# Inuri04/pgtg

Measured on AMD Instinct MI355X. Metric: env-steps/sec (batched random-action rollout) at 1/2/4/8 MI355X, higher is better.
Workload: dtype int32; 1 GPU; configs[4]: 1048576 envs of 5x5 procedural maps split over the GPUs, random actions, auto-reset, RCCL-reduced global step counter; envs_total=1048576, envs_per_gpu=1048576, map=5x5, autoreset=True, parallelism=dp1 (env shards, no data-path collective)

## Files before the change

### include/pgtg.h

```cpp
#ifndef PGTG_H_
#define PGTG_H_

#include <stdint.h>

#ifdef __cplusplus
extern "C" {
#endif

#define PGTG_ABI_VERSION 9

#define PGTG_OK 0
#define PGTG_E_INVALID -1
#define PGTG_E_DONE -2
#define PGTG_E_DEVICE -3
#define PGTG_E_UNSUPPORTED -4
#define PGTG_E_MAP -5

#define PGTG_MAX_TILES 256
#define PGTG_MAX_CHANNELS 128
#define PGTG_MAX_RULES 8
#define PGTG_MAX_WINDOW 31

enum {
  PGTG_CH_ZERO = 0,
  PGTG_CH_WALL = 1,
  PGTG_CH_GOALS = 2,
  PGTG_CH_TRAFFIC = 3,
  PGTG_CH_TL_GREEN = 4,
  PGTG_CH_TL_YELLOW = 5,
  PGTG_CH_TL_RED = 6,
  PGTG_CH_START = 7,
  PGTG_CH_SUBGOAL = 8,
  PGTG_CH_USED_SUBGOAL = 9,
  PGTG_CH_FINAL_GOAL = 10,
  PGTG_CH_ICE = 11,
  PGTG_CH_BROKEN = 12,
  PGTG_CH_SAND = 13,
  PGTG_CH_SPAWNER = 14,
  PGTG_CH_LANE0 = 32
};

typedef struct {
  int32_t tile_exits;
  int32_t speed_sq_min;
  int32_t speed_sq_max;
  int32_t min_traffic;
  int32_t min_matching_traffic;
  uint8_t weight[6][20];
} PgtgRule;

typedef struct {
  int32_t abi_version;
  int32_t width, height;
  double pct_connections;
  int32_t start_mode, goal_mode;
  int32_t start_x, start_y, start_dir;
  int32_t goal_x, goal_y, goal_dir;
  int32_t min_distance;
  double obstacle_probability;
  double w_ice, w_broken, w_sand, w_tl;
  int32_t n_channels;
  int32_t channels[PGTG_MAX_CHANNELS];
  int32_t sliding, sliding_size, next_subgoal;
  double sum_subgoals_reward, final_goal_bonus, crash_penalty, tl_violation_penalty;
  double standing_still_penalty, visited_penalty;
  double ice_probability, street_damage_probability, sand_probability, traffic_density;
  int32_t phase_dur[3];
  int32_t ignore_traffic_collisions;
  double profile_pct[5];
  int32_t separate_reward_cost;
  int32_t n_rules;
  PgtgRule rules[PGTG_MAX_RULES];
  int32_t fixed_map, fm_w, fm_h;
  uint8_t fm_exits[PGTG_MAX_TILES];
  int8_t fm_obst_type[PGTG_MAX_TILES];
  int8_t fm_obst_mask[PGTG_MAX_TILES];
  int32_t fm_start[3], fm_goal[3];
  int32_t autoreset;
  int32_t max_episode_steps;
  int32_t min_car_capacity;
  int32_t tune_envs_per_block;
  int32_t tune_obs_sub;
  int32_t tune_kt_grid, tune_kt_cap, tune_kt_wpc;
  int32_t tune_car_slots;
  int32_t tune_kt_serial;
  int32_t tune_queue_mode;
  int32_t tune_fault;
} PgtgConfig;

typedef struct {
  uint8_t* obs;
  int32_t* position;
  int32_t* velocity;
  int32_t* next_subgoal;
  double* reward;
  double* cost;
  uint8_t* terminated;
  uint8_t* truncated;
  uint8_t* final_obs;
  int32_t* final_position;
  int32_t* final_velocity;
  int32_t* final_next_subgoal;
  uint8_t* braking;
} PgtgOutputs;

typedef struct {
  int32_t x, y, vx, vy;
  int32_t terminated, flat_tire, phase, elapsed;
  int32_t n_cars, next_car_id, path_len, error;
  uint32_t spawn_counter;
  uint64_t seed;
  uint64_t used_subgoals[4];
  int32_t n_spawners, car_tail;
} PgtgEnvState;

typedef struct {
  int32_t id, x, y, route, profile, patience, delay;
} PgtgCar;

typedef struct {
  uint64_t episodes, truncated_only, length_sum;
  int32_t  length_min, length_max;
  double   return_sum;
  float    return_min, return_max;
} PgtgEpisodeSummary;

typedef struct pgtg_handle pgtg_handle;

int pgtg_create(const PgtgConfig* cfg, uint64_t n_envs, int32_t device, pgtg_handle** out);
int pgtg_destroy(pgtg_handle* h);
int pgtg_set_stream(pgtg_handle* h, void* stream);
int pgtg_set_outputs(pgtg_handle* h, const PgtgOutputs* out);
int pgtg_reset(pgtg_handle* h, const uint64_t* seeds_host, uint64_t seed_base, const uint8_t* mask_dev);
int pgtg_reset_unseeded(pgtg_handle* h, const uint8_t* mask_dev);
int pgtg_step(pgtg_handle* h, const uint8_t* actions_dev);
int pgtg_step_many(pgtg_handle* h, const uint8_t* actions_dev, uint64_t row_stride, uint64_t ticks);
int pgtg_random_actions(pgtg_handle* h, uint8_t* actions_dev, uint64_t seed, uint64_t t, uint64_t env_offset);
int pgtg_get_env_state(pgtg_handle* h, uint64_t env, PgtgEnvState* st);
int pgtg_get_cars(pgtg_handle* h, uint64_t env, PgtgCar* cars, int32_t cap, int32_t* n);
int pgtg_get_map_plan(pgtg_handle* h, uint64_t env, int32_t* w, int32_t* h_, uint8_t* exits, int8_t* otype,
                      int8_t* omask, int32_t* start3, int32_t* goal3);
#define PGTG_SQ_WALL (1ull << 32)
#define PGTG_SQ_SPAWNER (1ull << 37)
#define PGTG_SQ_START (1ull << 38)
#define PGTG_SQ_SUBGOAL (1ull << 39)
#define PGTG_SQ_USED_SUBGOAL (1ull << 40)
#define PGTG_SQ_FINAL_GOAL (1ull << 41)
#define PGTG_SQ_ICE (1ull << 42)
#define PGTG_SQ_BROKEN_ROAD (1ull << 43)
#define PGTG_SQ_SAND (1ull << 44)
#define PGTG_SQ_TRAFFIC_LIGHT (1ull << 45)
int pgtg_get_squares(pgtg_handle* h, uint64_t env, uint64_t* words, int32_t cap, int32_t* width, int32_t* height);
int pgtg_set_agent(pgtg_handle* h, uint64_t env, int32_t x, int32_t y, int32_t vx, int32_t vy);
int pgtg_add_car(pgtg_handle* h, uint64_t env, int32_t x, int32_t y, int32_t route, int32_t profile, int32_t car_id);
int pgtg_state_size(pgtg_handle* h, uint64_t* bytes);
int pgtg_dump_state(pgtg_handle* h, void* buf, uint64_t bytes);
int pgtg_load_state(pgtg_handle* h, const void* buf, uint64_t bytes);
typedef struct pgtg_snapshot pgtg_snapshot;
int pgtg_snapshot_create(pgtg_handle* h, uint64_t slots, pgtg_snapshot** out);
int pgtg_snapshot_destroy(pgtg_snapshot* s);
int pgtg_snapshot_bytes(const pgtg_snapshot* s, uint64_t* device_bytes, uint64_t* bytes_per_env);
int pgtg_snapshot_save(pgtg_handle* h, pgtg_snapshot* s, const uint32_t* env_idx_dev, const uint32_t* slot_idx_dev,
                       uint64_t count);
int pgtg_snapshot_load(pgtg_handle* h, const pgtg_snapshot* s, const uint32_t* slot_idx_dev, const uint32_t* env_idx_dev,
                       uint64_t count);
int pgtg_set_to_state(pgtg_handle* h, uint64_t env, int32_t x, int32_t y, int32_t vx, int32_t vy, int32_t flat_tire,
                      const PgtgCar* cars, int32_t n_cars);
int pgtg_set_rules(pgtg_handle* h, const PgtgRule* rules, int32_t n_rules);
int pgtg_set_flat_outputs(pgtg_handle* h, const int32_t* order, int32_t n_order, int32_t dtype, void* flat_dev,
                          void* final_flat_dev);
int pgtg_set_flat_scalars(pgtg_handle* h, float* reward_f32_dev, uint8_t* dones_dev, uint8_t* truncated_only_dev);
int pgtg_flatten(pgtg_handle* h, int32_t mode, int32_t grid);
int pgtg_set_episode_stats(pgtg_handle* h, float* ep_return_dev, int32_t* ep_length_dev);
int pgtg_episode_summary(pgtg_handle* h, PgtgEpisodeSummary* out, int32_t reset);
typedef struct {
  uint64_t n, steps;
  double gamma, gae_lambda;
  const float*   rewards;
  const float*   values;
  const uint8_t* dones;
  const uint8_t* truncated_only;
  const float*   terminal_values;
  const float*   last_values;
  float* advantages; float* returns;
} PgtgGae;
int pgtg_gae(pgtg_handle* h, const PgtgGae* a);
#define PGTG_POLICY_SAMPLE 0
#define PGTG_POLICY_ARGMAX 1
#define PGTG_POLICY_VALUE_ONLY 2
#define PGTG_POLICY_MAX_OBS_DIM 1048576
typedef struct {
  const float *w1p, *b1p, *w2p, *b2p, *wa, *ba;
  const float *w1v, *b1v, *w2v, *b2v, *wv, *bv;
  uint64_t obs_dim;
} PgtgPolicyWeights;
typedef struct { uint64_t n, obs_dim; const int8_t* obs; const void* packed;
                 int32_t mode; uint64_t seed, counter, env_offset;
                 const float* uniforms; uint8_t* actions; float* values; float* log_probs; } PgtgPolicy;
int pgtg_policy_packed_bytes(uint64_t obs_dim, uint64_t* bytes);
int pgtg_policy_pack(pgtg_handle* h, const PgtgPolicyWeights* raw, void* packed);
int pgtg_policy(pgtg_handle* h, const PgtgPolicy* a);
int pgtg_policy_chunk(void);
typedef struct {
  float *w1p, *b1p, *w2p, *b2p, *wa, *ba;
  float *w1v, *b1v, *w2v, *b2v, *wv, *bv;
} PgtgPpoGrads;
typedef struct {
  uint64_t batch, obs_dim, steps, n, obs_pitch;
  const int8_t* obs; const int64_t* indices;
  const uint8_t* actions;
  const float *log_probs, *advantages, *returns;
  const void* packed;
  const float* adv_stats;
  double clip_range, ent_coef, vf_coef;
  void* workspace;
  PgtgPpoGrads grads;
  float* stats;
} PgtgPpoGrad;
int pgtg_ppo_workspace_bytes(uint64_t obs_dim, uint64_t batch, uint64_t* bytes);
int pgtg_ppo_grad(pgtg_handle* h, const PgtgPpoGrad* a);
typedef struct {
  const float *w1p, *b1p, *w2p, *b2p, *wa, *ba;
  const float *w1v, *b1v, *w2v, *b2v, *wv, *bv;
} PgtgPpoConstGrads;
typedef struct {
  uint64_t obs_dim;
  PgtgPpoGrads params;
  PgtgPpoConstGrads grads;
  PgtgPpoGrads exp_avg, exp_avg_sq;
  void* packed;
  void* workspace;
  uint64_t step;
  float lr, beta1, beta2, eps, max_grad_norm;
  float* grad_norm;
} PgtgPpoStep;
int pgtg_ppo_step_workspace_bytes(uint64_t obs_dim, uint64_t* bytes);
int pgtg_ppo_step(pgtg_handle* h, const PgtgPpoStep* a);
int pgtg_ppo_adv_stats(pgtg_handle* h, const void* advantages, const void* indices, uint64_t batch, uint64_t steps,
                       uint64_t n, float* out);
typedef struct {
  uint64_t n, n_episodes;
  uint64_t step;
  double gamma;
  const double*  reward;
  const uint8_t* terminated;
  const uint8_t* truncated;
  double* ret; double* disc; double* g;
  int32_t* len; int32_t* cnt;
  double* rec_return; double* rec_discounted; int32_t* rec_length;
  double* rec_last_reward; int32_t* rec_end_step; uint8_t* rec_flags;
  int32_t* open_rows;
} PgtgEval;
typedef struct {
  uint64_t episodes, open_envs;
  uint64_t terminated, truncated_only;
  uint64_t last_reward_positive, last_reward_negative;
  uint64_t negative_discounted;
  uint64_t length_sum;
  int32_t  length_min, length_max;
  double   return_mean, return_std;
  double   return_min, return_max;
  double   discounted_mean, discounted_std;
} PgtgEvalSummary;
int pgtg_eval_step(pgtg_handle* h, const PgtgEval* a);
int pgtg_eval_summary(pgtg_handle* h, const PgtgEval* a, PgtgEvalSummary* out_dev, void* workspace);
int pgtg_eval_workspace_bytes(uint64_t n, uint64_t n_episodes, uint64_t* bytes);
int pgtg_observe(pgtg_handle* h);
int pgtg_car_digest(pgtg_handle* h, uint64_t* out_dev);
int pgtg_get_counters(pgtg_handle* h, uint64_t* env_steps, uint64_t* episodes);
int pgtg_get_queue_maps(pgtg_handle* h, uint64_t* maps);
int pgtg_get_queue_overflow(pgtg_handle* h, uint64_t* served);
int pgtg_error_count(pgtg_handle* h, uint64_t* n_errors, int32_t* first_code);
int pgtg_measure_hbm(int32_t device, uint64_t bytes, int32_t reps, double* copy_gbs);
int pgtg_window(const pgtg_handle* h);
uint64_t pgtg_num_envs(const pgtg_handle* h);
int pgtg_launch_info(const pgtg_handle* h, int32_t* envs_per_block, int32_t* lds_bytes);
int pgtg_occupancy(const pgtg_handle* h, int32_t* step_blocks_per_cu);
const char* pgtg_step_kernel(const pgtg_handle* h);
const char* pgtg_last_error(const pgtg_handle* h);
int pgtg_enable_timing(pgtg_handle* h, int32_t every);
int pgtg_timing_read(pgtg_handle* h, double* total_ms, uint64_t* launches, int32_t reset);

#ifdef __cplusplus
}
#endif
#endif
```

### pgtg_amd/_abi.py

```python
from __future__ import annotations

import ctypes as C
import os

from . import config as cfgmod

PKG = os.path.dirname(os.path.abspath(__file__))
LIB_PATH = os.environ.get("PGTG_LIB") or os.path.join(PKG, "libpgtg_hip.so")

PGTG_ABI_VERSION = 9
MAX_TILES = 256
MAX_CHANNELS = 128
MAX_RULES = 8

PGTG_OK = 0
PGTG_E_INVALID = -1
PGTG_E_DONE = -2
PGTG_E_DEVICE = -3
PGTG_E_UNSUPPORTED = -4
PGTG_E_MAP = -5

EXPORTED = [
    "pgtg_create", "pgtg_destroy", "pgtg_set_stream", "pgtg_set_outputs", "pgtg_reset",
    "pgtg_reset_unseeded", "pgtg_step", "pgtg_step_many", "pgtg_random_actions", "pgtg_get_env_state", "pgtg_get_cars",
    "pgtg_get_map_plan", "pgtg_get_squares", "pgtg_set_rules", "pgtg_set_agent", "pgtg_add_car", "pgtg_observe", "pgtg_get_counters",
    "pgtg_error_count", "pgtg_window", "pgtg_num_envs", "pgtg_launch_info", "pgtg_occupancy", "pgtg_step_kernel", "pgtg_last_error", "pgtg_enable_timing",
    "pgtg_timing_read", "pgtg_measure_hbm", "pgtg_state_size", "pgtg_dump_state", "pgtg_load_state",
    "pgtg_set_to_state", "pgtg_car_digest", "pgtg_get_queue_maps", "pgtg_get_queue_overflow", "pgtg_set_flat_outputs", "pgtg_set_flat_scalars",
    "pgtg_set_episode_stats", "pgtg_episode_summary", "pgtg_gae", "pgtg_flatten",
    "pgtg_eval_step", "pgtg_eval_summary", "pgtg_eval_workspace_bytes",
    "pgtg_policy", "pgtg_policy_pack", "pgtg_policy_packed_bytes", "pgtg_policy_chunk",
    "pgtg_ppo_workspace_bytes", "pgtg_ppo_grad",
    "pgtg_ppo_step_workspace_bytes", "pgtg_ppo_step", "pgtg_ppo_adv_stats",
    "pgtg_snapshot_create", "pgtg_snapshot_destroy", "pgtg_snapshot_bytes", "pgtg_snapshot_save", "pgtg_snapshot_load",
]


class PgtgRule(C.Structure):
    _fields_ = [("tile_exits", C.c_int32), ("speed_sq_min", C.c_int32), ("speed_sq_max", C.c_int32),
                ("min_traffic", C.c_int32), ("min_matching_traffic", C.c_int32),
                ("weight", (C.c_uint8 * 20) * 6)]


class PgtgConfig(C.Structure):
    _fields_ = [
        ("abi_version", C.c_int32), ("width", C.c_int32), ("height", C.c_int32),
        ("pct_connections", C.c_double), ("start_mode", C.c_int32), ("goal_mode", C.c_int32),
        ("start_x", C.c_int32), ("start_y", C.c_int32), ("start_dir", C.c_int32),
        ("goal_x", C.c_int32), ("goal_y", C.c_int32), ("goal_dir", C.c_int32),
        ("min_distance", C.c_int32), ("obstacle_probability", C.c_double),
        ("w_ice", C.c_double), ("w_broken", C.c_double), ("w_sand", C.c_double), ("w_tl", C.c_double),
        ("n_channels", C.c_int32), ("channels", C.c_int32 * MAX_CHANNELS),
        ("sliding", C.c_int32), ("sliding_size", C.c_int32), ("next_subgoal", C.c_int32),
        ("sum_subgoals_reward", C.c_double), ("final_goal_bonus", C.c_double),
        ("crash_penalty", C.c_double), ("tl_violation_penalty", C.c_double),
        ("standing_still_penalty", C.c_double), ("visited_penalty", C.c_double),
        ("ice_probability", C.c_double), ("street_damage_probability", C.c_double),
        ("sand_probability", C.c_double), ("traffic_density", C.c_double),
        ("phase_dur", C.c_int32 * 3), ("ignore_traffic_collisions", C.c_int32),
        ("profile_pct", C.c_double * 5), ("separate_reward_cost", C.c_int32),
        ("n_rules", C.c_int32), ("rules", PgtgRule * MAX_RULES),
        ("fixed_map", C.c_int32), ("fm_w", C.c_int32), ("fm_h", C.c_int32),
        ("fm_exits", C.c_uint8 * MAX_TILES), ("fm_obst_type", C.c_int8 * MAX_TILES),
        ("fm_obst_mask", C.c_int8 * MAX_TILES), ("fm_start", C.c_int32 * 3), ("fm_goal", C.c_int32 * 3),
        ("autoreset", C.c_int32), ("max_episode_steps", C.c_int32), ("min_car_capacity", C.c_int32),
        ("tune_envs_per_block", C.c_int32), ("tune_obs_sub", C.c_int32), ("tune_kt_grid", C.c_int32),
        ("tune_kt_cap", C.c_int32), ("tune_kt_wpc", C.c_int32), ("tune_car_slots", C.c_int32),
        ("tune_kt_serial", C.c_int32), ("tune_queue_mode", C.c_int32), ("tune_fault", C.c_int32),
    ]


class PgtgOutputs(C.Structure):
    _fields_ = [(n, C.c_void_p) for n in (
        "obs", "position", "velocity", "next_subgoal", "reward", "cost", "terminated", "truncated",
        "final_obs", "final_position", "final_velocity", "final_next_subgoal", "braking")]


class PgtgEnvState(C.Structure):
    _fields_ = [(n, C.c_int32) for n in ("x", "y", "vx", "vy", "terminated", "flat_tire", "phase", "elapsed",
                                         "n_cars", "next_car_id", "path_len", "error")] + [
        ("spawn_counter", C.c_uint32), ("seed", C.c_uint64), ("used_subgoals", C.c_uint64 * 4),
        ("n_spawners", C.c_int32), ("car_tail", C.c_int32)]


class PgtgCar(C.Structure):
    _fields_ = [(n, C.c_int32) for n in ("id", "x", "y", "route", "profile", "patience", "delay")]


class PgtgEpisodeSummary(C.Structure):
    _fields_ = [("episodes", C.c_uint64), ("truncated_only", C.c_uint64), ("length_sum", C.c_uint64),
                ("length_min", C.c_int32), ("length_max", C.c_int32), ("return_sum", C.c_double),
                ("return_min", C.c_float), ("return_max", C.c_float)]


class PgtgGae(C.Structure):
    _fields_ = [("n", C.c_uint64), ("steps", C.c_uint64), ("gamma", C.c_double), ("gae_lambda", C.c_double)] + [
        (n, C.c_void_p) for n in ("rewards", "values", "dones", "truncated_only", "terminal_values", "last_values",
                                  "advantages", "returns")]


EVAL_STATE_FIELDS = ("ret", "disc", "g", "len", "cnt")
EVAL_RECORD_FIELDS = ("rec_return", "rec_discounted", "rec_length", "rec_last_reward", "rec_end_step", "rec_flags")


class PgtgEval(C.Structure):
    _fields_ = [("n", C.c_uint64), ("n_episodes", C.c_uint64), ("step", C.c_uint64), ("gamma", C.c_double)] + [
        (n, C.c_void_p) for n in ("reward", "terminated", "truncated") + EVAL_STATE_FIELDS + EVAL_RECORD_FIELDS
        + ("open_rows",)]


class PgtgEvalSummary(C.Structure):
    _fields_ = [(n, C.c_uint64) for n in ("episodes", "open_envs", "terminated", "truncated_only",
                                          "last_reward_positive", "last_reward_negative", "negative_discounted",
                                          "length_sum")] + [
        ("length_min", C.c_int32), ("length_max", C.c_int32)] + [
        (n, C.c_double) for n in ("return_mean", "return_std", "return_min", "return_max", "discounted_mean",
                                  "discounted_std")]


PGTG_POLICY_SAMPLE, PGTG_POLICY_ARGMAX, PGTG_POLICY_VALUE_ONLY = 0, 1, 2
PGTG_POLICY_MAX_OBS_DIM = 1048576
POLICY_WEIGHT_FIELDS = ("w1p", "b1p", "w2p", "b2p", "wa", "ba", "w1v", "b1v", "w2v", "b2v", "wv", "bv")


class PgtgPolicyWeights(C.Structure):
    _fields_ = [(n, C.c_void_p) for n in POLICY_WEIGHT_FIELDS] + [("obs_dim", C.c_uint64)]


class PgtgPolicy(C.Structure):
    _fields_ = [("n", C.c_uint64), ("obs_dim", C.c_uint64), ("obs", C.c_void_p), ("packed", C.c_void_p),
                ("mode", C.c_int32), ("seed", C.c_uint64), ("counter", C.c_uint64), ("env_offset", C.c_uint64),
                ("uniforms", C.c_void_p), ("actions", C.c_void_p), ("values", C.c_void_p), ("log_probs", C.c_void_p)]


class PgtgPpoGrads(C.Structure):
    _fields_ = [(n, C.c_void_p) for n in POLICY_WEIGHT_FIELDS]


class PgtgPpoGrad(C.Structure):
    _fields_ = [(n, C.c_uint64) for n in ("batch", "obs_dim", "steps", "n", "obs_pitch")] + [
        (n, C.c_void_p) for n in ("obs", "indices", "actions", "log_probs", "advantages", "returns", "packed",
                                  "adv_stats")] + [
        ("clip_range", C.c_double), ("ent_coef", C.c_double), ("vf_coef", C.c_double), ("workspace", C.c_void_p),
        ("grads", PgtgPpoGrads), ("stats", C.c_void_p)]


class PgtgPpoStep(C.Structure):
    _fields_ = [("obs_dim", C.c_uint64), ("params", PgtgPpoGrads), ("grads", PgtgPpoGrads), ("exp_avg", PgtgPpoGrads),
                ("exp_avg_sq", PgtgPpoGrads), ("packed", C.c_void_p), ("workspace", C.c_void_p), ("step", C.c_uint64),
                ("lr", C.c_float), ("beta1", C.c_float), ("beta2", C.c_float), ("eps", C.c_float),
                ("max_grad_norm", C.c_float), ("grad_norm", C.c_void_p)]


_lib = None


def lib():
    global _lib
    if _lib is not None:
        return _lib
    if not os.path.exists(LIB_PATH):
        raise RuntimeError(f"{LIB_PATH} not built: run `python -m pgtg_amd.build` (HIP/gfx950); "
                           "there is no CPU fallback")
    import torch
    L = C.CDLL(LIB_PATH)
    vp, u64, i32 = C.c_void_p, C.c_uint64, C.c_int32
    sig = {
        "pgtg_create": ([C.POINTER(PgtgConfig), u64, i32, C.POINTER(vp)], C.c_int),
        "pgtg_destroy": ([vp], C.c_int),
        "pgtg_set_stream": ([vp, vp], C.c_int),
        "pgtg_set_outputs": ([vp, C.POINTER(PgtgOutputs)], C.c_int),
        "pgtg_reset": ([vp, vp, u64, vp], C.c_int),
        "pgtg_reset_unseeded": ([vp, vp], C.c_int),
        "pgtg_step": ([vp, vp], C.c_int),
        "pgtg_step_many": ([vp, vp, u64, u64], C.c_int),
        "pgtg_random_actions": ([vp, vp, u64, u64, u64], C.c_int),
        "pgtg_measure_hbm": ([i32, u64, i32, C.POINTER(C.c_double)], C.c_int),
        "pgtg_state_size": ([vp, C.POINTER(u64)], C.c_int),
        "pgtg_dump_state": ([vp, vp, u64], C.c_int),
        "pgtg_load_state": ([vp, vp, u64], C.c_int),
        "pgtg_set_to_state": ([vp, u64, i32, i32, i32, i32, i32, C.POINTER(PgtgCar), i32], C.c_int),
        "pgtg_get_env_state": ([vp, u64, C.POINTER(PgtgEnvState)], C.c_int),
        "pgtg_get_cars": ([vp, u64, C.POINTER(PgtgCar), i32, C.POINTER(i32)], C.c_int),
        "pgtg_get_map_plan": ([vp, u64] + [vp] * 7, C.c_int),
        "pgtg_get_squares": ([vp, u64, vp, i32, C.POINTER(i32), C.POINTER(i32)], C.c_int),
        "pgtg_set_rules": ([vp, vp, i32], C.c_int),
        "pgtg_set_agent": ([vp, u64, i32, i32, i32, i32], C.c_int),
        "pgtg_add_car": ([vp, u64, i32, i32, i32, i32, i32], C.c_int),
        "pgtg_observe": ([vp], C.c_int),
        "pgtg_get_counters": ([vp, C.POINTER(u64), C.POINTER(u64)], C.c_int),
        "pgtg_car_digest": ([vp, vp], C.c_int),
        "pgtg_get_queue_maps": ([vp, C.POINTER(u64)], C.c_int),
        "pgtg_get_queue_overflow": ([vp, C.POINTER(u64)], C.c_int),
        "pgtg_set_flat_outputs": ([vp, C.POINTER(C.c_int32), i32, i32, vp, vp], C.c_int),
        "pgtg_set_flat_scalars": ([vp, vp, vp, vp], C.c_int),
        "pgtg_flatten": ([vp, i32, i32], C.c_int),
        "pgtg_set_episode_stats": ([vp, vp, vp], C.c_int),
        "pgtg_episode_summary": ([vp, C.POINTER(PgtgEpisodeSummary), i32], C.c_int),
        "pgtg_gae": ([vp, C.POINTER(PgtgGae)], C.c_int),
        "pgtg_eval_step": ([vp, C.POINTER(PgtgEval)], C.c_int),
        "pgtg_eval_summary": ([vp, C.POINTER(PgtgEval), vp, vp], C.c_int),
        "pgtg_eval_workspace_bytes": ([u64, u64, C.POINTER(u64)], C.c_int),
        "pgtg_policy": ([vp, C.POINTER(PgtgPolicy)], C.c_int),
        "pgtg_policy_pack": ([vp, C.POINTER(PgtgPolicyWeights), vp], C.c_int),
        "pgtg_policy_packed_bytes": ([u64, C.POINTER(u64)], C.c_int),
        "pgtg_policy_chunk": ([], C.c_int),
        "pgtg_ppo_workspace_bytes": ([u64, u64, C.POINTER(u64)], C.c_int),
        "pgtg_ppo_grad": ([vp, C.POINTER(PgtgPpoGrad)], C.c_int),
        "pgtg_ppo_step_workspace_bytes": ([u64, C.POINTER(u64)], C.c_int),
        "pgtg_ppo_step": ([vp, C.POINTER(PgtgPpoStep)], C.c_int),
        "pgtg_ppo_adv_stats": ([vp, vp, vp, u64, u64, u64, vp], C.c_int),
        "pgtg_snapshot_create": ([vp, u64, C.POINTER(vp)], C.c_int),
        "pgtg_snapshot_destroy": ([vp], C.c_int),
        "pgtg_snapshot_bytes": ([vp, C.POINTER(u64), C.POINTER(u64)], C.c_int),
        "pgtg_snapshot_save": ([vp, vp, vp, vp, u64], C.c_int),
        "pgtg_snapshot_load": ([vp, vp, vp, vp, u64], C.c_int),
        "pgtg_error_count": ([vp, C.POINTER(u64), C.POINTER(i32)], C.c_int),
        "pgtg_window": ([vp], C.c_int),
        "pgtg_num_envs": ([vp], u64),
        "pgtg_launch_info": ([vp, C.POINTER(i32), C.POINTER(i32)], C.c_int),
        "pgtg_occupancy": ([vp, C.POINTER(i32)], C.c_int),
        "pgtg_step_kernel": ([vp], C.c_char_p),
        "pgtg_last_error": ([vp], C.c_char_p),
        "pgtg_timing_read": ([vp, C.POINTER(C.c_double), C.POINTER(u64), i32], C.c_int),
        "pgtg_enable_timing": ([vp, i32], C.c_int),
    }
    compat = os.environ.get("PGTG_ABI_COMPAT")
    for name, (args, res) in sig.items():
        if compat and not hasattr(L, name):
            continue
        f = getattr(L, name)
        f.argtypes = args
        f.restype = res
    _lib = L
    return L


def fill_rules(dst, rules) -> int:
    if len(rules) > MAX_RULES:
        raise ValueError(f"at most {MAX_RULES} traffic rules are supported")
    for i, r in enumerate(rules):
        o = dst[i]
        o.tile_exits, o.speed_sq_min, o.speed_sq_max = r.tile_exits, r.speed_sq_min, r.speed_sq_max
        o.min_traffic, o.min_matching_traffic = r.min_traffic, r.min_matching_traffic
        for d in range(6):
            for k in range(20):
                o.weight[d][k] = r.weight[d][k]
    return len(rules)


TUNE_KEYS = ("envs_per_block", "obs_sub", "kt_grid", "kt_cap", "kt_wpc", "car_slots", "kt_serial", "queue_mode", "fault")


def config_struct(spec: "cfgmod.EnvSpec", autoreset: bool, max_episode_steps: int | None,
                  min_car_capacity: int = 0, tune: dict | None = None) -> PgtgConfig:
    c = PgtgConfig()
    c.abi_version = int(os.environ.get("PGTG_ABI_COMPAT") or PGTG_ABI_VERSION)
    c.width, c.height = spec.width, spec.height
    c.pct_connections = spec.pct_connections
    c.start_mode, c.goal_mode = spec.start_mode, spec.goal_mode
    c.start_x, c.start_y, c.start_dir = spec.start_xyd
    c.goal_x, c.goal_y, c.goal_dir = spec.goal_xyd
    c.min_distance = spec.min_distance
    c.obstacle_probability = spec.obstacle_probability
    c.w_ice, c.w_broken, c.w_sand, c.w_tl = [float(w) for w in spec.weights]
    c.n_channels = len(spec.channels)
    for i, (_, code) in enumerate(spec.channels):
        c.channels[i] = code
    c.sliding, c.sliding_size, c.next_subgoal = int(spec.sliding), spec.sliding_size, int(spec.next_subgoal)
    c.sum_subgoals_reward = spec.sum_subgoals_reward
    c.final_goal_bonus = spec.final_goal_bonus
    c.crash_penalty = spec.crash_penalty
    c.tl_violation_penalty = spec.tl_violation_penalty
    c.standing_still_penalty = spec.standing_still_penalty
    c.visited_penalty = spec.visited_penalty
    c.ice_probability = spec.ice_probability
    c.street_damage_probability = spec.street_damage_probability
    c.sand_probability = spec.sand_probability
    c.traffic_density = spec.traffic_density
    for i in range(3):
        c.phase_dur[i] = spec.phase_dur[i]
    c.ignore_traffic_collisions = int(spec.ignore_traffic_collisions)
    for i in range(5):
        c.profile_pct[i] = float(spec.profile_pct[i])
    c.separate_reward_cost = int(spec.separate_reward_cost)
    c.n_rules = fill_rules(c.rules, spec.rules)
    fm = spec.fixed_map
    if fm is not None:
        if fm.width * fm.height > MAX_TILES:
            raise ValueError(f"this build supports maps of at most {MAX_TILES} tiles")
        c.fixed_map = 1
        c.fm_w, c.fm_h = fm.width, fm.height
        for i in range(fm.width * fm.height):
            c.fm_exits[i] = fm.exits[i]
            c.fm_obst_type[i] = fm.obstacle_type[i]
            c.fm_obst_mask[i] = fm.obstacle_mask[i]
        for i in range(3):
            c.fm_start[i] = fm.start[i]
            c.fm_goal[i] = fm.goal[i]
    c.autoreset = int(autoreset)
    c.max_episode_steps = int(max_episode_steps or 0)
    c.min_car_capacity = int(min_car_capacity)
    for k, v in (tune or {}).items():
        if k not in TUNE_KEYS:
            raise ValueError(f"unknown launch-shape override {k!r} (one of {TUNE_KEYS})")
        setattr(c, "tune_" + k, int(v))
    return c
```

### pgtg_amd/csrc/pgtg_env.hip

```cpp
#include <hip/hip_runtime.h>

#include <math.h>
#include <stdint.h>
#include <stdio.h>
#include <stdlib.h>
#include <string.h>

#include <algorithm>
#include <array>
#include <cstddef>
#include <string>
#include <vector>

#include "pgtg_device.h"
#include "pgtg_episode.h"
#include "pgtg_eval.h"
#include "pgtg_rollout.h"
#include "pgtg_policy.h"
#include "pgtg_ppo.h"
#include "pgtg_ppo_step.h"
#include "pgtg_snapshot.h"

namespace pgtg {
namespace dv {
#define PGTG_TBL_QUAL __constant__ static const
#include "pgtg_tables.h"
#undef PGTG_TBL_QUAL
}
namespace hs {
#define PGTG_TBL_QUAL static const
#include "pgtg_tables.h"
#undef PGTG_TBL_QUAL
}

__shared__ __attribute__((aligned(16))) TablesHead sT;
__shared__ __attribute__((aligned(16))) TablesTail sTX;

__device__ __forceinline__ void stage_bytes(const void* __restrict__ gsrc, void* ldst, int bytes) {
  const int n4 = bytes >> 4, tid = (int)threadIdx.x;
  const uint4* src = reinterpret_cast<const uint4*>(gsrc);
  uint4* dst = reinterpret_cast<uint4*>(ldst);
  uint4 r[4];
#pragma unroll
  for (int j = 0; j < 4; j++) r[j] = src[tid + j * kBlock < n4 ? tid + j * kBlock : 0];
#pragma unroll
  for (int j = 0; j < 4; j++)
    if (tid + j * kBlock < n4) dst[tid + j * kBlock] = r[j];
  for (int k = tid + 4 * kBlock; k < n4; k += kBlock) dst[k] = src[k];
  for (int k = n4 * 4 + tid; k < bytes / 4; k += kBlock)
    reinterpret_cast<uint32_t*>(ldst)[k] = reinterpret_cast<const uint32_t*>(gsrc)[k];
}
__device__ __forceinline__ void stage_tables(const Tables* __restrict__ gtab, bool tail) {
  stage_bytes(gtab, &sT, (int)sizeof(TablesHead));
  if (tail) stage_bytes(reinterpret_cast<const uint8_t*>(gtab) + kTabHead, &sTX, (int)sizeof(TablesTail));
}

__device__ __forceinline__ void lds_barrier() {
  __builtin_amdgcn_fence(__ATOMIC_RELEASE, "workgroup", "local");
  __builtin_amdgcn_s_barrier();
  __builtin_amdgcn_fence(__ATOMIC_ACQUIRE, "workgroup", "local");
}

template <bool BIG>
__device__ __forceinline__ void stage_plan(const uint16_t* __restrict__ plan, int nq, uint32_t* dst, int pdw) {
  const uint4* src = reinterpret_cast<const uint4*>(plan);
  for (int k0 = 0; k0 < (BIG ? nq : 1); k0 += 8) {
    uint4 q[8];
#pragma unroll
    for (int k = 0; k < 8; k++) q[k] = src[k0 + k < nq ? k0 + k : k0];
#pragma unroll
    for (int k = 0; k < 8; k++) {
      if (k0 + k < nq) {
        const uint32_t wv[4] = {q[k].x, q[k].y, q[k].z, q[k].w};
#pragma unroll
        for (int j = 0; j < 4; j++)
          if ((k0 + k) * 4 + j < pdw) dst[(k0 + k) * 4 + j] = wv[j];
      }
    }
  }
}

#ifdef PGTG_STAMPS
__device__ unsigned long long g_stamps[1 << 21];
#define STAMP(k)                                                                          \
  do {                                                                                    \
    if ((threadIdx.x & 63) == 0) {                                                        \
      unsigned long long t_ = __builtin_amdgcn_s_memtime();                               \
      g_stamps[((blockIdx.x * (kBlock / 64) + (threadIdx.x >> 6)) * 32 + (k)) & ((1 << 21) - 1)] = t_; \
    }                                                                                     \
  } while (0)
#define STAMPR(k)                                                                                     \
  do {                                                                                                \
    if ((threadIdx.x & 63) == 0)                                                                      \
      g_stamps[(1 << 20) | ((((blockIdx.x * (kBlock / 64) + (threadIdx.x >> 6)) * 8 + (k))) & ((1 << 20) - 1))] = \
          __builtin_amdgcn_s_memrealtime();                                                           \
  } while (0)
#else
#define STAMP(k) \
  do {           \
  } while (0)
#define STAMPR(k) \
  do {            \
  } while (0)
#endif

__device__ __forceinline__ uint32_t bit81(const uint32_t* m3, int sq) { return (m3[sq >> 5] >> (sq & 31)) & 1u; }

__device__ __forceinline__ int seg_dir(int lx, int ly) {
  bool mx = (unsigned)(lx - 3) <= 2u, my = (unsigned)(ly - 3) <= 2u;
  if (ly == 0 && mx) return 0;
  if (lx == 8 && my) return 1;
  if (ly == 8 && mx) return 2;
  if (lx == 0 && my) return 3;
  return -1;
}

struct EnvView {
  int px, py, vx, vy;
  uint32_t phase, flags, path_len, elapsed;
  uint32_t sg, spawn;
  uint64_t used;
};

__device__ __forceinline__ EnvView rec_view(const EnvRec& e) {
  EnvView v;
  v.px = (int)(int16_t)(e.a.x & 0xffffu);
  v.py = (int)(int16_t)(e.a.x >> 16);
  v.vx = (int)(int16_t)(e.a.y & 0xffffu);
  v.vy = (int)(int16_t)(e.a.y >> 16);
  v.phase = e.a.z & 0xffffu;
  v.flags = (e.a.z >> 16) & 0xfu;
  v.path_len = e.a.z >> 20;
  v.elapsed = e.a.w;
  v.sg = e.b.x;
  v.spawn = e.b.y;
  v.used = (uint64_t)e.b.z | ((uint64_t)e.b.w << 32);
  return v;
}
__device__ __forceinline__ EnvView rec_load(const EnvRec* r, uint64_t i) { return rec_view(r[i]); }
__device__ __forceinline__ void rec_store(EnvRec* r, uint64_t i, const EnvView& v) {
  EnvRec e;
  e.a.x = ((uint32_t)v.px & 0xffffu) | ((uint32_t)v.py << 16);
  e.a.y = ((uint32_t)v.vx & 0xffffu) | ((uint32_t)v.vy << 16);
  e.a.z = (v.phase & 0xffffu) | ((v.flags & 0xfu) << 16) | (v.path_len << 20);
  e.a.w = v.elapsed;
  e.b.x = v.sg;
  e.b.y = v.spawn;
  e.b.z = (uint32_t)v.used;
  e.b.w = (uint32_t)(v.used >> 32);
  r[i] = e;
}

__device__ __forceinline__ uint32_t plan_word_mask(const DevCfg& c, int word) {
  const int t0 = 2 * word;
  return t0 + 1 < c.nt ? ~0u : (t0 < c.nt ? 0xffffu : 0u);
}
constexpr int kQueueDepth = 3;
__host__ __device__ inline uint32_t queue_slot(uint32_t bits) { return (bits & 3u) < 2u ? (bits & 3u) : 2u; }
__host__ __device__ inline uint32_t queue_cur(uint32_t qs) { return queue_slot(qs); }
__host__ __device__ inline uint32_t queue_head(uint32_t qs) { return queue_slot(qs >> 2); }
__host__ __device__ inline uint32_t queue_spare(uint32_t qc, uint32_t qh) { return qc != qh ? 3u - qc - qh : (qc + 2u) % 3u; }
template <bool SLOT>
__device__ __forceinline__ uint16_t* plan_row(const DevCfg& c, const DevState& S, uint64_t i) {
  if (!SLOT) return S.plan + i * (uint64_t)c.plan_stride;
  return reinterpret_cast<uint16_t*>(S.qbuf + (i * kQueueDepth + queue_cur(S.qstate[i])) * (uint64_t)c.qrec_dw);
}
__device__ __forceinline__ void store_plan_quads(const DevCfg& c, uint4* dstp, int nq, const uint32_t* pw, int pdw) {
  for (int k = 0; k < nq; k++) {
    uint32_t wv[4];
#pragma unroll
    for (int j = 0; j < 4; j++) wv[j] = (k * 4 + j < pdw) ? pw[k * 4 + j] & plan_word_mask(c, k * 4 + j) : 0u;
    dstp[k] = make_uint4(wv[0], wv[1], wv[2], wv[3]);
  }
}
template <bool SLOT>
__device__ __forceinline__ void store_plan_row(const DevCfg& c, const DevState& S, uint64_t i, const uint32_t* pw, int pdw) {
  if (SLOT) {
    store_plan_quads(c, reinterpret_cast<uint4*>(plan_row<true>(c, S, i)), c.qrec_dw / 4, pw, pdw);
    return;
  }
  uint4* dstp = reinterpret_cast<uint4*>(S.plan + i * (uint64_t)c.plan_stride);
  for (int k = 0; k < c.plan_stride / 8; k++) {
    uint32_t wv[4];
#pragma unroll
    for (int j = 0; j < 4; j++) wv[j] = (k * 4 + j < pdw) ? pw[k * 4 + j] & plan_word_mask(c, k * 4 + j) : 0u;
    dstp[k] = make_uint4(wv[0], wv[1], wv[2], wv[3]);
  }
}

struct Plan {
  uint16_t* p;
  __device__ __forceinline__ uint32_t operator[](int t) const { return p[t]; }
};

template <bool BIG>
__device__ __forceinline__ bool used_bit(const EnvView& v, uint32_t p, int t) {
  return BIG ? (p & kPlanUsed) != 0u : ((v.used >> t) & 1ull) != 0ull;
}

template <bool BIG>
__device__ __forceinline__ uint32_t square_flags(const DevCfg& c, const Plan& pl, const EnvView& v, int x, int y) {
  int tx = x / kTile, ty = y / kTile;
  int lx = x - tx * kTile, ly = y - ty * kTile;
  int t = ty * c.tw + tx;
  uint32_t p = pl[t];
  uint32_t ex = plan_exits(p);
  int sq = lx * 9 + ly;
  uint32_t f = 0;
  uint32_t wall = bit81(sT.wall[ex], sq);
  if (wall) f |= SQ_WALL;
  int d = seg_dir(lx, ly);
  if (d >= 0 && ((ex >> d) & 1u)) {
    if (plan_sgdir(p) == d) f |= used_bit<BIG>(v, p, t) ? SQ_USED : SQ_SUBGOAL;
    if ((int)(v.sg & 0xffu) == t && (int)((v.sg >> 8) & 0xffu) == d) f |= SQ_START;
    if ((int)((v.sg >> 16) & 0xffu) == t && (int)(v.sg >> 24) == d) f |= SQ_FINAL;
  }
  const uint32_t ob = bit81(sT.obst[min(plan_omask(p), (uint32_t)PGTG_N_OBST_MASKS - 1u)], sq);
  uint32_t ot = plan_otype(p);
  if (ot && !wall && ob) f |= SQ_ICE << (ot - 1);
  return f;
}
__device__ __forceinline__ uint32_t square_lanes(const DevCfg& c, const Plan& pl, int x, int y) {
  int tx = x / kTile, ty = y / kTile;
  int lx = x - tx * kTile, ly = y - ty * kTile;
  uint32_t ex = plan_exits(pl[ty * c.tw + tx]);
  return ex ? sTX.lanes[ex][lx * 9 + ly] : 0u;
}
__device__ __forceinline__ bool square_spawner(const DevCfg& c, const Plan& pl, int x, int y) {
  int tx = x / kTile, ty = y / kTile;
  int lx = x - tx * kTile, ly = y - ty * kTile;
  uint32_t ex = plan_exits(pl[ty * c.tw + tx]);
  if (!ex) return false;
  int sq = lx * 9 + ly;
  if (bit81(sT.spawner[ex], sq)) return true;
  uint32_t l = sTX.lanes[ex][sq];
  return (tx == 0 && (l >> 31 & 1u)) || (tx == c.tw - 1 && (l >> 30 & 1u)) || (ty == 0 && (l >> 29 & 1u)) ||
         (ty == c.th - 1 && (l >> 28 & 1u));
}
__device__ __forceinline__ bool inside(const DevCfg& c, int x, int y) {
  return (unsigned)x < (unsigned)c.W && (unsigned)y < (unsigned)c.H;
}
__device__ __forceinline__ int phase_color(const DevCfg& c, uint32_t ph) {
  return (int)ph < c.phase_g ? 0 : ((int)ph < c.phase_gy ? 1 : 2);
}

__device__ __forceinline__ int lane_slot_tw(int tw, const Plan& pl, int x, int y) {
  int tx = x / kTile, ty = y / kTile;
  int lx = x - tx * kTile, ly = y - ty * kTile;
  int t = ty * tw + tx;
  uint32_t ex = plan_exits(pl[t]);
  const int li_raw = sTX.li[ex][lx * 9 + ly];
  const int li = ex ? li_raw : 255;
  return li == 255 ? -1 : t * 32 + li;
}
// ... 2085 lines not shown
      if (pcg_double(sand) < c.sand_p) {
        cx += pxp;
        cy += pyp;
        v.vx = v.vy = 0;
        break;
      }
    }
    cx += pxp;
    cy += pyp;
  }
  (void)gl_t;
  (void)gl_d;
  if (used_ice) stream_store_state(S.ice, i, ice);
  if (used_broken) stream_store_state(S.broken, i, broken);
  if (used_sand) stream_store_state(S.sand, i, sand);
  if (v.flags & kFlagFlatTire) v.vx = v.vy = 0;
  const bool accel = !(ax == 0 && ay == 0);
  if (S.visited) {
    uint32_t* vis = S.visited + i * (uint64_t)c.vis_words;
    int b = (cx + 2) * c.vis_pitch + (cy + 2);
    if (c.visited_penalty != 0.0 && accel && ((vis[b >> 5] >> (b & 31)) & 1u)) {
      if (c.separate_cost) cost += c.visited_penalty; else reward -= c.visited_penalty;
    }
    vis[b >> 5] |= 1u << (b & 31);
  }
  const int ox = v.px, oy = v.py;
  v.px = cx;
  v.py = cy;
  if (c.still_penalty != 0.0 && !accel && ox == cx && oy == cy) {
    if (c.separate_cost) cost += c.still_penalty; else reward -= c.still_penalty;
  }
  v.elapsed += 1u;
  if (c.max_steps > 0 && (int)v.elapsed >= c.max_steps) v.flags |= kFlagTruncated;
  res.reward = c.separate_cost ? perf : reward;
  res.cost = cost;
  return 0;
}

__device__ __forceinline__ uint32_t expand4(uint32_t x) { return ((x & 15u) * 0x00204081u) & 0x01010101u; }
__device__ __forceinline__ uint32_t udiv_f(uint32_t x, uint32_t d, float inv) {
  uint32_t q = (uint32_t)((float)x * inv);
  if (q * d > x) q--;
  if ((q + 1) * d <= x) q++;
  return q;
}

__device__ __forceinline__ void mark_lines(uint32_t* lm, const uint8_t* dst, uint32_t e, uint32_t OB) {
  const uintptr_t a0 = (uintptr_t)dst, base = a0 >> 7;
  uint32_t l = (uint32_t)(((a0 + (uintptr_t)e * OB) >> 7) - base);
  const uint32_t l1 = (uint32_t)(((a0 + (uintptr_t)(e + 1) * OB - 1) >> 7) - base);
  while (l <= l1) {
    const uint32_t hi = min(l1, l | 31u), n = hi - l + 1u;
    __hip_atomic_fetch_or(lm + (l >> 5), (n == 32u ? ~0u : ((1u << n) - 1u)) << (l & 31u), __ATOMIC_RELAXED,
                          __HIP_MEMORY_SCOPE_WORKGROUP);
    l = hi + 1u;
  }
}

__device__ __forceinline__ void write_obs(uint8_t* __restrict__ dst, uint32_t cnt, uint32_t OB, const uint32_t* st,
                                          const uint8_t* sel, int rank = -1, int nthr = kBlock,
                                          const uint32_t* lm = nullptr) {
  if (rank < 0) rank = (int)threadIdx.x;
  const uint32_t total = cnt * OB;
  const uintptr_t a0 = (uintptr_t)dst;
  const uintptr_t c0 = a0 & ~(uintptr_t)15;
  const uint32_t nchunks = (uint32_t)((a0 + total - c0 + 15) >> 4);
  const float invOB = 1.0f / (float)OB;
  for (uint32_t ch = (uint32_t)rank; ch < nchunks; ch += (uint32_t)nthr) {
    const int r = (int)((intptr_t)(c0 + ((uintptr_t)ch << 4)) - (intptr_t)a0);
    if (lm) {
      const uint32_t li = (uint32_t)(((c0 + ((uintptr_t)ch << 4)) >> 7) - (a0 >> 7));
      if (!((lm[li >> 5] >> (li & 31u)) & 1u)) continue;
    } else if (sel) {
      const intptr_t l0 = (intptr_t)((c0 + ((uintptr_t)ch << 4)) & ~(uintptr_t)127) - (intptr_t)a0;
      const uint32_t llo = l0 < 0 ? 0u : (uint32_t)l0;
      const uint32_t lhi = min((uint32_t)(l0 + 127), total - 1u);
      const uint32_t e0 = udiv_f(llo, OB, invOB), e1 = udiv_f(lhi, OB, invOB);
      bool any = false;
      for (uint32_t e = e0; e <= e1; e++) any = any || sel[e] == 1;
      if (!any) continue;
    }
    uint8_t* cp = dst + r;
    if (r >= 0 && (uint32_t)r + 16u <= total) {
      const uint32_t w = (uint32_t)r >> 5;
      const uint64_t two = (uint64_t)st[w] | ((uint64_t)st[w + 1] << 32);
      const uint32_t bits = (uint32_t)(two >> (r & 31));
#ifdef PGTG_NT_OBS
      typedef unsigned int v4u __attribute__((ext_vector_type(4)));
      v4u o = {expand4(bits), expand4(bits >> 4), expand4(bits >> 8), expand4(bits >> 12)};
      __builtin_nontemporal_store(o, reinterpret_cast<v4u*>(cp));
#else
      *reinterpret_cast<uint4*>(cp) = make_uint4(expand4(bits), expand4(bits >> 4), expand4(bits >> 8), expand4(bits >> 12));
#endif
    } else {
      for (int b = 0; b < 16; b++) {
        const int rb = r + b;
        if (rb >= 0 && (uint32_t)rb < total) cp[b] = (uint8_t)((st[rb >> 5] >> (rb & 31)) & 1u);
      }
    }
  }
}

__device__ __forceinline__ bool obs_key_ok(const DevCfg& c) { return !c.sliding && !c.generic_channels && !c.need_car; }
template <bool BIG>
__device__ __forceinline__ uint64_t obs_key(const DevCfg& c, const EnvView& v, const Plan& pl) {
  const int pix = min(max(0, v.px), c.W - 1), piy = min(max(0, v.py), c.H - 1);
  const int t = (piy / kTile) * c.tw + pix / kTile;
  const uint32_t p = pl[t];
  const uint32_t col = plan_otype(p) == 4u ? (uint32_t)phase_color(c, v.phase) : 0u;
  const uint32_t lo = p | (used_bit<BIG>(v, p, t) ? 1u << 16 : 0u) | col << 17 | (uint32_t)t << 19;
  return (uint64_t)v.sg << 32 | lo;
}

struct Lds {
  int envs;
  int plan_stride_dw;
  int scratch_dw;
  int traf_dw;
  int hist_dw;
  int seg_bits;
  int sub_envs;
  int stream_words;
  int spread;
  int compact;
  int queue;
  int gen_off;
  int lm_words;
  int stagger;
  int stagger_wgs;
  int ramp_pct;
  int img_in_traf;
  int prio;
  int abl;
};
constexpr int kQueueLanes = 64;
constexpr int kMaxQueueGrid = 4096;
constexpr int kQctrBlocks = 2 * kMaxQueueGrid;
constexpr int kQctrOvfLen = kQctrBlocks + 3;
constexpr int kQctrWords = kQctrOvfLen + 24;
__device__ __forceinline__ uint32_t wave_sum(uint32_t x) {
#pragma unroll
  for (int o = 32; o > 0; o >>= 1) x += (uint32_t)__shfl_xor((int)x, o);
  return x;
}
__host__ __device__ inline uint64_t queue_req_cap(uint64_t nblk, uint64_t grid, int envs) {
  const uint64_t c = 3 * ((nblk + grid - 1) / grid) * (uint64_t)envs;
  return c < (uint64_t)kQueueLanes ? (uint64_t)kQueueLanes : c;
}
constexpr uint64_t kStaggerMaxTicks = 20000;
constexpr int kBlockDepth = 3;
constexpr uint32_t kQueueStale = 0x80u;
constexpr int kViewDw = 8;
constexpr int kObsMasks = 2;
constexpr uint32_t kQselFull = 8u;

__host__ __device__ inline uint32_t queue_tag(uint32_t spawn) { return ~spawn; }
__host__ __device__ inline int odd_up(int x) { return x | 1; }
__host__ inline int img_words(int envs, int bits) { return ((int)(((int64_t)envs * bits + 31) / 32) + 2 + 3) & ~3; }

__host__ inline void lds_tail(Lds& l, const DevCfg& c);
__host__ inline Lds lds_layout(const DevCfg& c, int envs) {
  Lds l;
  l.envs = envs;
  l.plan_stride_dw = odd_up((c.nt + 1) / 2);
  l.scratch_dw = c.need_car ? 0 : 3;
  l.traf_dw = c.need_car ? odd_up(c.traf_bytes / 4) : 0;
  l.hist_dw = (c.n_rules > 0 || c.need_car) ? 5 : 0;
  l.seg_bits = c.n_channels * c.win * c.win;
  const int budget_words = 12 * 1024;
  int sub = l.seg_bits > 0 ? (int)(((int64_t)budget_words - 3) * 32 / l.seg_bits) : envs;
  l.sub_envs = sub > envs ? envs : (sub < 1 ? 1 : sub);
  l.stream_words = img_words(l.sub_envs, l.seg_bits);
  l.spread = c.need_car ? 1 : 0;
  l.compact = 1;
  l.queue = !c.need_car && c.n_rules == 0 && !c.fixed_map && !c.generic_channels && envs <= kBlock - 64 && l.sub_envs >= envs;
  l.stagger = 0;
  l.stagger_wgs = 0;
  l.ramp_pct = 25;
  l.img_in_traf = 0;
  l.abl = 0;
  l.prio = 0;
#ifdef PGTG_TUNING
  if (const char* e = getenv("PGTG_ABL")) l.abl = atoi(e);
  if (const char* e = getenv("PGTG_PRIO")) l.prio = atoi(e);
  if (const char* e = getenv("PGTG_RAMP")) l.ramp_pct = atoi(e);
  if (const char* e = getenv("PGTG_SPREAD")) l.spread = atoi(e);
  if (const char* e = getenv("PGTG_COMPACT")) l.compact = atoi(e);
  if (const char* e = getenv("PGTG_QUEUE")) l.queue = l.queue && atoi(e);
#endif
  lds_tail(l, c);
  return l;
}
__host__ inline int tail_bytes(const Lds& l) {
  return kBlock + (l.queue ? 128 : 32) + 4 * l.lm_words + (l.queue && l.envs <= 32 ? 4 * kViewDw * l.envs : 0);
}
__host__ inline void lds_tail(Lds& l, const DevCfg& c) {
  const int64_t total = (int64_t)l.envs * l.seg_bits;
  const int lines = (int)((127 + total) / 128) + 1;
  l.lm_words = (!c.need_car && l.sub_envs >= l.envs && lines <= 64 * 32) ? (lines + 31) / 32 : 0;
#ifdef PGTG_TUNING
  if (const char* e = getenv("PGTG_LINEMASK")) l.lm_words = atoi(e) ? l.lm_words : 0;
#endif
  l.gen_off = (int)(((size_t)l.envs * (l.plan_stride_dw + l.scratch_dw + l.traf_dw + l.hist_dw) + l.stream_words) +
                    tail_bytes(l) / 4);
}
__host__ inline size_t lds_bytes(const Lds& l) {
  return (size_t)4 * ((size_t)l.envs * (l.plan_stride_dw + l.scratch_dw + l.traf_dw + l.hist_dw) + l.stream_words) +
         tail_bytes(l) + (l.queue ? (size_t)4 * kQueueLanes * l.plan_stride_dw : 0);
}

__host__ inline void lds_img_in_traf(Lds& l, const DevCfg& c) {
  if (!c.need_car || !c.obs_fast || l.envs < 1) return;
  if ((int64_t)img_words(l.envs, l.seg_bits) > (int64_t)l.envs * l.traf_dw) return;
  l.img_in_traf = 1;
  l.sub_envs = l.envs;
  l.stream_words = 0;
  l.hist_dw = 7;
  lds_tail(l, c);
}

enum { MODE_STEP = 0, MODE_RESET_SEEDED = 1, MODE_RESET_UNSEEDED = 2, MODE_OBSERVE = 3 };

__device__ __forceinline__ void write_small_outputs(const DevCfg& c, const PgtgOutputs& o, uint64_t i, const EnvView& v,
                                                    const ObsInfo& oi, bool final) {
  if (!final) {
    if (o.position) reinterpret_cast<int2*>(o.position)[i] = make_int2(oi.posx, oi.posy);
    if (o.velocity) reinterpret_cast<int2*>(o.velocity)[i] = make_int2(v.vx, v.vy);
    if (o.next_subgoal) o.next_subgoal[i] = oi.nsd;
  } else {
    if (o.final_position) reinterpret_cast<int2*>(o.final_position)[i] = make_int2(oi.posx, oi.posy);
    if (o.final_velocity) reinterpret_cast<int2*>(o.final_velocity)[i] = make_int2(v.vx, v.vy);
    if (o.final_next_subgoal) o.final_next_subgoal[i] = oi.nsd;
  }
}

template <bool TR, bool BIG>
__device__ __forceinline__ void obs_pass(const DevCfg& c, const DevState& S, const Plan& pl, const EnvView& v,
                                         const PgtgOutputs& o, uint8_t* dst, uint64_t env0, int nb, bool want,
                                         bool final, const uint8_t* sel, uint32_t* st, const Lds& L,
                                         const uint8_t* occ, int slot) {
  for (int sb = 0; sb < nb; sb += L.sub_envs) {
    const int cnt = min(L.sub_envs, nb - sb);
    if (want && slot >= sb && slot < sb + cnt) {
      ObsInfo oi;
      build_obs<TR, BIG, true, !TR>(c, S, pl, v, st, (uint32_t)(slot - sb) * (uint32_t)c.obs_bytes, oi, occ);
      write_small_outputs(c, o, env0 + slot, v, oi, final);
    }
    lds_barrier();
    if (dst)
      write_obs(dst + (env0 + sb) * (uint64_t)c.obs_bytes, (uint32_t)cnt, (uint32_t)c.obs_bytes, st, sel ? sel + sb : nullptr);
    lds_barrier();
  }
}

__device__ __forceinline__ uint64_t stagger_start(const Lds& L, const DevState& S) {
  if (!L.stagger) return 0;
  const uint64_t t0 = wall_clock64();
  if (blockIdx.x == 0 || blockIdx.x >= (unsigned)L.stagger_wgs) return t0;
  const uint64_t span = min(S.wg_ticks[0] * (uint64_t)L.ramp_pct / 100ull, (unsigned long long)kStaggerMaxTicks);
  const uint64_t wait = span * blockIdx.x / (unsigned)L.stagger_wgs;
  while (wall_clock64() - t0 < wait) __builtin_amdgcn_s_sleep(16);
  return t0;
}
__device__ __forceinline__ void stagger_record(const Lds& L, const DevState& S, uint64_t t0) {
  if (L.stagger && blockIdx.x == 0 && threadIdx.x == 0) S.wg_ticks[0] = wall_clock64() - t0;
}

template <bool TR, bool BIG, bool SLOT = false>
__global__ void __launch_bounds__(kBlock, TR ? 3 : 4) k_env(const DevCfg* __restrict__ cfg, const Tables* __restrict__ gtab,
                                                 DevState S, const uint8_t* __restrict__ actions,
                                                 const uint8_t* __restrict__ mask, PgtgOutputs out, int mode, Lds L,
                                                 uint32_t tr_slot) {
  extern __shared__ uint32_t lds[];
  const DevCfg& c = *cfg;
  const int tid = threadIdx.x;
  const uint64_t t_start = TR ? 0 : stagger_start(L, S);
  STAMP(0);
  if ((TR && c.need_car) && mode != MODE_OBSERVE && blockIdx.x == 0 && tid == 0) S.tr_count[tr_slot ^ 1u] = 0u;
  stage_tables(gtab, c.generic_channels || (TR && c.need_car));
  const uint64_t env0 = (uint64_t)blockIdx.x * L.envs;
  const int nb = (int)min((uint64_t)L.envs, S.n - env0);
  const int per_wave = (!L.spread || L.envs >= kBlock) ? 64 : L.envs / 4;
  const bool has_slot = (tid & 63) < per_wave;
  const int slot = has_slot ? (tid >> 6) * per_wave + (tid & 63) : 0;
  const uint64_t i = env0 + slot;
  const bool live = has_slot && slot < nb;
  const int my_slot = slot;
  uint32_t* plan_w = lds + my_slot * L.plan_stride_dw;
  uint32_t* traf_w = lds + L.envs * (L.plan_stride_dw + L.scratch_dw) + my_slot * L.traf_dw;
  uint32_t* hist_w = lds + L.envs * (L.plan_stride_dw + L.scratch_dw + L.traf_dw) + my_slot * L.hist_dw;
  const int env_dw = L.plan_stride_dw + L.scratch_dw + L.traf_dw + L.hist_dw;
  uint32_t* st = (TR && L.img_in_traf) ? lds + L.envs * (L.plan_stride_dw + L.scratch_dw) : lds + L.envs * env_dw;
  uint8_t* sel = reinterpret_cast<uint8_t*>(lds + L.envs * env_dw + L.stream_words);
  uint64_t* wmask = reinterpret_cast<uint64_t*>(sel + kBlock);
  uint32_t* lm = L.lm_words ? reinterpret_cast<uint32_t*>(sel + kBlock + 32) : nullptr;
  const bool img_traf = TR && L.img_in_traf;
  const int xf_off = img_traf ? L.envs * (L.plan_stride_dw + L.scratch_dw + L.traf_dw) + 4
                   : L.envs * L.plan_stride_dw + ((TR && c.need_car) ? L.envs * L.scratch_dw : 0);
  const int xf_dw = img_traf ? L.hist_dw : (TR && c.need_car) ? L.traf_dw : L.scratch_dw;
  uint32_t* xf = lds + xf_off + my_slot * xf_dw;
  uint8_t* occ = reinterpret_cast<uint8_t*>(traf_w);
  uint16_t* sp_l = reinterpret_cast<uint16_t*>(occ + c.sp_cache_off);
  uint8_t* hist = reinterpret_cast<uint8_t*>(hist_w);
  Plan pl{reinterpret_cast<uint16_t*>(plan_w)};

  EnvView v{};
// ... 264 lines not shown
  __device__ __forceinline__ int err(uint32_t k0, bool ablate) const {
    return (tag != queue_tag(k0) && !ablate) ? PGTG_E_DEVICE : gen_err();
  }
};

template <bool BIG>
__device__ __forceinline__ void gen_queue_entry(const DevCfg& c, const DevState& S, uint64_t i, uint32_t k,
                                                uint16_t* plan, int pdw, uint32_t* __restrict__ dst,
                                                bool no_store = false, bool fold_ok = true) {
  SeedPool sp = ss_pool(S.seed[i]);
  Pcg map_rng = ss_child(sp, k);
  int st_t, st_d, gl_t, gl_d;
  uint64_t ix[4];
  generate_map<BIG>(c, BIG ? S.epk : sT.epk, map_rng, plan, st_t, st_d, gl_t, gl_d, ix);
  uint64_t dirs[4] = {0ull, 0ull, 0ull, 0ull};
  const bool fold = !BIG && c.dual && fold_ok;
  int len = compile_generated<BIG>(c, plan, st_t, gl_t, ix, fold ? dirs : nullptr);
  int px = 0, py = 0, err = 0;
  if (len <= 0 || !((plan_exits(plan[st_t]) >> st_d) & 1u)) {
    err = len < 0 ? PGTG_E_DEVICE : PGTG_E_MAP;
    len = 0;
  } else {
    const int j = (int)pcg_int(map_rng, 3);
    const int tx = st_t % c.tw, ty = st_t / c.tw;
    int lx, ly;
    switch (st_d) {
      case 0: lx = 3 + j; ly = 0; break;
      case 1: lx = 8; ly = 3 + j; break;
      case 2: lx = 3 + j; ly = 8; break;
      default: lx = 0; ly = 3 + j; break;
    }
    px = tx * kTile + lx;
    py = ty * kTile + ly;
  }
  const uint32_t* pw = reinterpret_cast<const uint32_t*>(plan);
  uint4* d4 = reinterpret_cast<uint4*>(dst);
  const int pwords = c.plan_dq * 4;
#ifdef PGTG_TUNING
  if (no_store) {
    if (len == 12345 && px == 7) d4[0] = make_uint4(0, 0, 0, 0);
    return;
  }
#endif
  for (int q = 0; q < pwords / 4; q++) {
    uint32_t wv[4];
#pragma unroll
    for (int j = 0; j < 4; j++) {
      wv[j] = (q * 4 + j < pdw) ? (pw[q * 4 + j] & plan_word_mask(c, q * 4 + j)) : 0u;
      if (fold) {
        const int t0 = 2 * (q * 4 + j);
        const uint32_t d0 = (uint32_t)((dirs[0] >> t0) & 1ull) + 2u * (uint32_t)((dirs[1] >> t0) & 1ull) +
                            3u * (uint32_t)((dirs[2] >> t0) & 1ull) + 4u * (uint32_t)((dirs[3] >> t0) & 1ull);
        const uint32_t d1 = t0 + 1 < 64 ? (uint32_t)((dirs[0] >> (t0 + 1)) & 1ull) + 2u * (uint32_t)((dirs[1] >> (t0 + 1)) & 1ull) +
                                          3u * (uint32_t)((dirs[2] >> (t0 + 1)) & 1ull) + 4u * (uint32_t)((dirs[3] >> (t0 + 1)) & 1ull)
                                        : 0u;
        wv[j] |= (d0 << 11 | d1 << 27) & plan_word_mask(c, q * 4 + j);
      }
    }
    d4[q] = make_uint4(wv[0], wv[1], wv[2], wv[3]);
  }
  d4[pwords / 4] = QueueMeta::pack(px, py, sg_word(st_t, st_d, gl_t, gl_d), (uint32_t)len, err, k);
  for (int q = pwords / 4 + 1; q < c.qrec_dw / 4; q++) d4[q] = make_uint4(0u, 0u, 0u, 0u);
}

#ifdef PGTG_TUNING
#define ABLATE(L, bit) (((L).abl & (bit)) != 0)
#else
#define ABLATE(L, bit) false
#endif

__device__ __forceinline__ void sub_barrier(uint32_t* ctr, uint32_t target) {
  __builtin_amdgcn_fence(__ATOMIC_RELEASE, "workgroup", "local");
  if ((threadIdx.x & 63) == 0) __hip_atomic_fetch_add(ctr, 1u, __ATOMIC_RELAXED, __HIP_MEMORY_SCOPE_WORKGROUP);
  while (__hip_atomic_load(ctr, __ATOMIC_RELAXED, __HIP_MEMORY_SCOPE_WORKGROUP) < target) __builtin_amdgcn_s_sleep(1);
  __builtin_amdgcn_fence(__ATOMIC_ACQUIRE, "workgroup", "local");
}

template <bool BIG>
__device__ __forceinline__ void group_obs(const DevCfg& c, const DevState& S, const EnvView& v, bool want,
                                          uint32_t* st, ObsInfo& oi, const Lds& L, int wave, int lane,
                                          uint32_t* ctr, uint32_t& bar, int np, int rank, uint32_t* vw,
                                          bool post = true) {
  const int vtid = wave * 64 + lane;
  const int E = L.envs;
  if (E <= 32) {
    if (wave == 0 && lane < E) {
      uint32_t* q = vw + lane * kViewDw;
      q[0] = (uint32_t)v.px;
      q[1] = (uint32_t)v.py;
      q[2] = v.sg;
      q[3] = v.phase;
      q[4] = (uint32_t)v.used;
      q[5] = (uint32_t)(v.used >> 32);
      q[6] = want ? 1u : 0u;
    }
    sub_barrier(ctr, bar += (uint32_t)np);
    STAMP(post ? 9 : 16);
    const int G = np * 64 / E, e = rank % E, sub = rank / E;
    if (sub >= G) return;
    const uint32_t* q = vw + e * kViewDw;
    if (!q[6]) return;
    const int C = c.n_channels, lo = sub * C / G, hi = (sub + 1) * C / G;
    if (lo == hi && sub != 0) return;
    EnvView ve{};
    ve.px = (int)q[0];
    ve.py = (int)q[1];
    ve.sg = q[2];
    ve.phase = q[3];
    ve.used = (uint64_t)q[4] | (uint64_t)q[5] << 32;
    STAMP(post ? 10 : 17);
    extern __shared__ uint32_t lds[];
    const Plan pl{reinterpret_cast<uint16_t*>(lds + e * L.plan_stride_dw)};
    build_obs<false, BIG, false, false>(c, S, pl, ve, st, (uint32_t)e * (uint32_t)c.obs_bytes, oi, nullptr, lo, hi, sub == 0,
                                 true);
    STAMP(post ? 11 : 18);
    return;
  }
  if (want) {
    extern __shared__ uint32_t lds[];
    const int slot = vtid;
    const Plan pl{reinterpret_cast<uint16_t*>(lds + slot * L.plan_stride_dw)};
    build_obs<false, BIG, false, false>(c, S, pl, v, st, (uint32_t)slot * (uint32_t)c.obs_bytes, oi, nullptr);
  }
}

template <bool BIG>
__device__ __forceinline__ QueueMeta ring_take(const DevCfg& c, const DevState& S, const Lds& L, uint64_t i, uint32_t qh,
                                           uint32_t k0, uint32_t* plan_w, int pdw, int depth) {
  const uint4* q4 = reinterpret_cast<const uint4*>(S.qbuf + (i * (uint64_t)depth + qh) * (uint64_t)c.qrec_dw);
  uint4* dstp = reinterpret_cast<uint4*>(S.plan + i * (uint64_t)c.plan_stride);
  const int nq = c.plan_dq;
  const uint4 meta = q4[nq];
  for (int k0q = 0; k0q < (BIG ? nq : 1); k0q += 8) {
    uint4 qw[8];
#pragma unroll
    for (int k = 0; k < 8; k++) qw[k] = q4[k0q + k < nq ? k0q + k : k0q];
#pragma unroll
    for (int k = 0; k < 8; k++) {
      if (k0q + k < nq) {
        if (!ABLATE(L, 32)) dstp[k0q + k] = qw[k];
        const uint32_t wv[4] = {qw[k].x, qw[k].y, qw[k].z, qw[k].w};
#pragma unroll
        for (int j = 0; j < 4; j++)
          if ((k0q + k) * 4 + j < pdw) plan_w[(k0q + k) * 4 + j] = wv[j];
      }
    }
  }
  if (!ABLATE(L, 32))
    for (int k = nq; k < c.plan_stride / 8; k++) dstp[k] = make_uint4(0u, 0u, 0u, 0u);
  episode_streams(c, S, i, k0);
  return QueueMeta(meta);
}

template <bool BIG>
__global__ void __launch_bounds__(kBlock, 4) k_envq(const DevCfg* __restrict__ cfg, const Tables* __restrict__ gtab,
                                                    DevState S, const uint8_t* __restrict__ actions, PgtgOutputs out,
                                                    Lds L, uint32_t qsel) {
  extern __shared__ uint32_t lds[];
  const DevCfg& c = *cfg;
  const int tid = threadIdx.x, wave = tid >> 6, lane = tid & 63;
  const uint64_t t_start = stagger_start(L, S);
  STAMP(0);
  STAMPR(2);
  const int env_waves = (L.envs + 63) / 64, gen_wave = env_waves;
  const bool env_wave = wave < env_waves;
  const uint32_t par = (qsel >> 2) & 1u;
  const uint64_t nblk = (S.n + (uint64_t)L.envs - 1) / (uint64_t)L.envs;
  const uint64_t cap = queue_req_cap(nblk, gridDim.x, L.envs);
  uint2* req_new = S.qreq + ((uint64_t)par * gridDim.x + blockIdx.x) * cap;
  const uint2* req_old = S.qreq + ((uint64_t)(par ^ 1u) * gridDim.x + blockIdx.x) * cap;
  const bool one_round = nblk <= gridDim.x;
  const uint32_t ox = blockIdx.x & 7u, set_new = qsel & 3u, set_old = (set_new + 2u) % 3u;
  const uint64_t ocap = ((gridDim.x + 7u) / 8u) * (uint64_t)L.envs;
  uint32_t cnt = 0;
  uint2 r0 = make_uint2(0u, 0u);
  if (wave == gen_wave) {
    cnt = S.qctr[(par ^ 1u) * gridDim.x + blockIdx.x];
    r0 = req_old[lane];
  }
  if (blockIdx.x == 0 && tid < 8) S.qctr[kQctrOvfLen + ((set_new + 1u) % 3u) * 8u + tid] = 0u;
  uint32_t qs_nx = 0;
  if (tid < L.envs && (uint64_t)blockIdx.x * L.envs + tid < S.n) qs_nx = S.qstate[(uint64_t)blockIdx.x * L.envs + tid];
  const int pdw = L.plan_stride_dw;
  stage_tables(gtab, false);
  uint32_t* st = lds + L.envs * (pdw + L.scratch_dw + L.traf_dw + L.hist_dw);
  uint8_t* sel = reinterpret_cast<uint8_t*>(st + L.stream_words);
  uint32_t* ctr = reinterpret_cast<uint32_t*>(sel + kBlock);
  uint32_t* lm = L.lm_words ? reinterpret_cast<uint32_t*>(sel + kBlock + 128) : nullptr;
  uint32_t* vw = reinterpret_cast<uint32_t*>(sel + kBlock + 128) + L.lm_words;
  const bool delta = lm && out.obs && obs_key_ok(c) && !(qsel & kQselFull) && kObsMasks * L.lm_words <= L.scratch_dw * L.envs;
  uint32_t* const om0 = lds + L.envs * pdw;
  uint32_t* om = delta ? om0 : nullptr;
  uint32_t* qn = ctr + 1;
  uint32_t* nxt = ctr + 2;
  uint32_t* bctr = S.qctr + kQctrBlocks;
  if (blockIdx.x == 0 && tid == 0) bctr[((qsel & 3u) + 1u) % 3u] = 0u;
  if (tid == 0) {
    *ctr = 0u;
    *qn = 0u;
  }
  lds_barrier();
  asm volatile("" : "+v"(qs_nx));

  if (wave == gen_wave) {
    STAMP(1);
    uint16_t* gplan = reinterpret_cast<uint16_t*>(lds + L.gen_off + lane * pdw);
    uint32_t made = 0, ovs = 0;
    if (!ABLATE(L, 1)) {
      const uint2* ovf = S.qovf + ((uint64_t)(par ^ 1u) * 8u + ox) * ocap;
      uint32_t ob = 0, on = 0, olen = 0, tot = 0;
      const uint32_t nj = (gridDim.x - ox + 7u) / 8u, jme = blockIdx.x / 8u;
      if (one_round) {
        olen = S.qctr[kQctrOvfLen + set_old * 8u + ox];
        if (olen > 0) {
          uint32_t pre = 0;
          for (uint32_t j0 = 0; j0 < nj; j0 += kQueueLanes) {
            const uint32_t j = j0 + (uint32_t)lane;
            const uint32_t sp = j < nj ? kQueueLanes - min(S.qctr[(par ^ 1u) * gridDim.x + ox + 8u * j], (uint32_t)kQueueLanes) : 0u;
            pre += wave_sum(j < jme ? sp : 0u);
            tot += wave_sum(sp);
          }
          on = olen > pre ? min(olen - pre, kQueueLanes - min(cnt, (uint32_t)kQueueLanes)) : 0u;
          ob = pre;
        }
      }
      for (uint32_t base = 0;; base += kQueueLanes) {
        const uint32_t own = base < cnt ? min((uint32_t)kQueueLanes, cnt - base) : 0u;
        const uint32_t oth = base == 0 ? on : 0u;
        if (own + oth == 0) break;
        made += own + oth;
        ovs += oth;
        if ((uint32_t)lane < own + oth) {
          const uint2 r = (uint32_t)lane >= own ? ovf[ob + (lane - own)] : base == 0 ? r0 : req_old[base + lane];
          const uint64_t ie = r.x >> 2;
          gen_queue_entry<BIG>(c, S, ie, r.y, gplan, pdw, S.qbuf + (ie * kQueueDepth + queue_slot(r.x)) * (uint64_t)c.qrec_dw,
                               ABLATE(L, 16), false);
        }
        if (base + kQueueLanes >= cnt) break;
      }
      for (uint64_t st0 = tot + (uint64_t)jme * kQueueLanes; st0 < olen; st0 += (uint64_t)nj * kQueueLanes) {
        const uint32_t m = (uint32_t)min((uint64_t)kQueueLanes, olen - st0);
        made += m;
        ovs += m;
        if ((uint32_t)lane < m) {
          const uint2 r = ovf[st0 + lane];
          const uint64_t ie = r.x >> 2;
          gen_queue_entry<BIG>(c, S, ie, r.y, gplan, pdw, S.qbuf + (ie * kQueueDepth + queue_slot(r.x)) * (uint64_t)c.qrec_dw,
                               ABLATE(L, 16), false);
        }
      }
    }
    if (lane == 0 && made) atomicAdd(&S.counters[2], (unsigned long long)made);
    if (lane == 0 && ovs) atomicAdd(&S.counters[3], (unsigned long long)ovs);
    STAMP(7);
    STAMPR(3);
    return;
  }

  const int np = kBlock / 64 - 1;
  const int nthr = np * 64;
  uint32_t bar = 0;
  for (uint64_t blk = blockIdx.x; blk < nblk;) {
    STAMP(0);
    uint32_t got = 0xffffffffu;
    if (tid == 0 && nblk > gridDim.x && *qn + 2u * (uint32_t)L.envs <= cap) got = atomicAdd(&bctr[qsel & 3u], 1u);
    int tid_o = tid;
    asm volatile("" : "+v"(tid_o));
    const int lane = tid_o & 63;
    const int rank = (wave < gen_wave ? wave : wave - 1) * 64 + lane;
    const int slot = tid_o;
    uint32_t* plan_w = lds + (env_wave ? slot : 0) * pdw;
    Plan pl{reinterpret_cast<uint16_t*>(plan_w)};
    const uint64_t env0 = blk * (uint64_t)L.envs;
    const int nb = (int)min((uint64_t)L.envs, S.n - env0);
    const uint64_t i = env0 + slot;
    const bool live = env_wave && slot < nb;
    EnvView v{};
    const uint32_t qs = qs_nx;
    const auto ring_slot = [&](uint32_t s) { return S.qbuf + (i * kQueueDepth + s) * (uint64_t)c.qrec_dw; };
    int act = 0;
    if (live) {
      v = rec_load(S.rec, i);
      act = actions[i];
      stage_plan<BIG>(reinterpret_cast<const uint16_t*>(ring_slot(queue_cur(qs))), c.plan_dq, plan_w, pdw);
    }
    for (int k = rank; k < L.lm_words; k += nthr) lm[k] = 0u;
    if (om)
      for (int k = rank; k < L.lm_words; k += nthr) om[k] = 0u;
    sub_barrier(ctr, bar += (uint32_t)np);
    STAMP(1);
    uint8_t my_sel = 0;
    int err = 0;
    if (live) {
      StepResult res{0.0, 0.0, 0u};
      bool occ_sat = false;
      TrafState ts{0, 0, 0, 0};
      const uint64_t key0 = om ? obs_key<BIG>(c, v, pl) : 0ull;
      err = env_step<false, BIG>(c, S, i, v, pl, act, res, nullptr, occ_sat, nullptr, ts, nullptr);
      STAMP(22);
      const bool done = (v.flags & (kFlagTerminated | kFlagTruncated)) != 0;
      if (out.reward) out.reward[i] = res.reward;
      if (out.cost) out.cost[i] = res.cost;
      if (out.terminated) out.terminated[i] = (v.flags & kFlagTerminated) ? 1 : 0;
      if (out.truncated) out.truncated[i] = (v.flags & kFlagTruncated) ? 1 : 0;
      if (out.braking) out.braking[i] = 0;
      my_sel = (done && c.autoreset && err == 0) ? 1 : 0;
      if (BIG && res.plan_dirty && !my_sel)
        store_plan_quads(c, reinterpret_cast<uint4*>(ring_slot(queue_cur(qs))), c.plan_dq, plan_w, pdw);
      if (lm && my_sel && out.final_obs) mark_lines(lm, out.final_obs + env0 * (uint64_t)c.obs_bytes, (uint32_t)slot, (uint32_t)c.obs_bytes);
      if (om && (my_sel || err != 0 || obs_key<BIG>(c, v, pl) != key0))
        mark_lines(om, out.obs + env0 * (uint64_t)c.obs_bytes, (uint32_t)slot, (uint32_t)c.obs_bytes);
      STAMP(23);
    }
    {
      ObsInfo oi;
      group_obs<BIG>(c, S, v, live, st, oi, L, wave, lane, ctr, bar, np, rank, vw);
      if (live) write_small_outputs(c, out, i, v, oi, my_sel == 1);
    }
    if (env_wave) sel[slot] = my_sel;
    const uint64_t rm = __ballot(my_sel == 1);
    if (env_wave && lane == 0 && rm) atomicAdd(&S.counters[1], (unsigned long long)__popcll(rm));
    if (tid == 0) *nxt = got;
    STAMP(2);
    STAMP(28);
    sub_barrier(ctr, bar += (uint32_t)np);
    STAMP(29);
    {
      const uint32_t g = *nxt;
      const uint64_t ni = ((uint64_t)gridDim.x + g) * (uint64_t)L.envs + (uint64_t)slot;
      qs_nx = 0;
      if (g != 0xffffffffu && slot < L.envs && ni < S.n) qs_nx = S.qstate[ni];
    }
    if (out.final_obs && !ABLATE(L, 2))
      write_obs(out.final_obs + env0 * (uint64_t)c.obs_bytes, (uint32_t)nb, (uint32_t)c.obs_bytes, st, sel, rank, nthr, lm);
    STAMP(3);
    sub_barrier(ctr, bar += (uint32_t)np);
    const bool reset_now = my_sel != 0;
    const uint32_t k0 = v.spawn;
    const uint32_t qc = queue_cur(qs), qh = queue_head(qs);
    if (reset_now) {
      const uint4* q4 = reinterpret_cast<const uint4*>(ring_slot(qh));
      const int nq = c.plan_dq;
      const uint4 meta = q4[nq];
      stage_plan<BIG>(reinterpret_cast<const uint16_t*>(q4), nq, plan_w, pdw);
      if (c.need_ice || c.need_broken || c.need_sand) {
        SeedPool sp = ss_pool(S.seed[i]);
        if (c.need_ice) stream_store_all(S.ice, i, ss_child(sp, k0 + 2u));
        if (c.need_broken) stream_store_all(S.broken, i, ss_child(sp, k0 + 3u));
        if (c.need_sand) stream_store_all(S.sand, i, ss_child(sp, k0 + 4u));
      }
      v.spawn = k0 + 5u;
      v.sg = meta.y;
      v.used = 0;
      v.path_len = meta.z & 0xffffu;
      v.flags = 0;
      v.phase = 0;
      v.elapsed = 0;
      v.vx = v.vy = 0;
      v.px = (int)(int16_t)(meta.x & 0xffffu);
      v.py = (int)(int16_t)(meta.x >> 16);
      const int e2 = (meta.w != queue_tag(k0) && !ABLATE(L, 1 | 16)) ? PGTG_E_DEVICE : -(int)(meta.z >> 16);
      if (e2) err = e2;
      if (S.visited && e2 == 0) {
        uint32_t* vis = S.visited + i * (uint64_t)c.vis_words;
        for (int q2 = 0; q2 < c.vis_words; q2++) vis[q2] = 0;
        int b = (v.px + 2) * c.vis_pitch + (v.py + 2);
        vis[b >> 5] |= 1u << (b & 31);
      }
    }
    asm volatile("" : "+v"(qs_nx));
    STAMP(4);
    const uint64_t rb = __ballot(reset_now);
    if (rb) {
      uint32_t base = 0;
      if (lane == 0) base = atomicAdd(qn, (uint32_t)__popcll(rb));
      base = __builtin_amdgcn_readfirstlane(base);
      const uint32_t k = (uint32_t)__popcll(rb);
      const uint32_t ovn = (one_round && base + k > (uint32_t)kQueueLanes) ? base + k - max(base, (uint32_t)kQueueLanes) : 0u;
      uint32_t obase = 0;
      if (ovn) {
        if (lane == 0) obase = atomicAdd(&S.qctr[kQctrOvfLen + set_new * 8u + ox], ovn);
        obase = __builtin_amdgcn_readfirstlane(obase);
      }
      if (reset_now) {
        const uint32_t p = base + (uint32_t)__popcll(rb & ((1ull << lane) - 1ull));
        const uint2 r = make_uint2((uint32_t)i << 2 | qc, k0 + 10u);
        if (one_round && p >= (uint32_t)kQueueLanes)
          S.qovf[((uint64_t)par * 8u + ox) * ocap + obase + (p - max(base, (uint32_t)kQueueLanes))] = r;
        else
          req_new[p] = r;
        S.qstate[i] = (uint8_t)(qh | queue_spare(qc, qh) << 2);
      }
    }
    if (live) {
      rec_store(S.rec, i, v);
      S.err[i] = (uint8_t)(-err);
    }
    STAMP(5);
    {
      ObsInfo oi;
      group_obs<BIG>(c, S, v, reset_now, st, oi, L, wave, lane, ctr, bar, np, rank, vw, false);
      if (reset_now) write_small_outputs(c, out, i, v, oi, false);
    }
    STAMP(30);
    sub_barrier(ctr, bar += (uint32_t)np);
    STAMP(31);
    if (tid == 0)
      S.qctr[par * gridDim.x + blockIdx.x] = one_round ? min(*qn, (uint32_t)kQueueLanes) : *qn;
    const uint32_t g = *nxt;
    if (out.obs && !ABLATE(L, 4))
      write_obs(out.obs + env0 * (uint64_t)c.obs_bytes, (uint32_t)nb, (uint32_t)c.obs_bytes, st, nullptr, rank, nthr, om);
    if (om) om = om == om0 ? om0 + L.lm_words : om0;
    if (tid == 0) atomicAdd(&S.counters[0], (unsigned long long)nb);
    if (blk == blockIdx.x) stagger_record(L, S, t_start);
    STAMP(6);
    blk = g == 0xffffffffu ? nblk : (uint64_t)gridDim.x + g;
  }  STAMPR(3);
}

template <bool BIG>
__global__ void __launch_bounds__(kBlock, 4) k_envb(const DevCfg* __restrict__ cfg, const Tables* __restrict__ gtab,
                                                    DevState S, const uint8_t* __restrict__ actions, PgtgOutputs out,
                                                    Lds L) {
  extern __shared__ uint32_t lds[];
  const DevCfg& c = *cfg;
  const int tid = threadIdx.x, wave = tid >> 6, lane = tid & 63;
  const uint64_t t_start = stagger_start(L, S);
  STAMP(0);
  STAMPR(2);
  stage_tables(gtab, false);
  const uint64_t env0 = (uint64_t)blockIdx.x * L.envs;
  const int nb = (int)min((uint64_t)L.envs, S.n - env0);
  const int env_waves = (L.envs + 63) / 64, gen_wave = env_waves;
#ifdef PGTG_TUNING
  if (wave != gen_wave) {
    if (L.prio == 1) __builtin_amdgcn_s_setprio(1);
    else if (L.prio == 2) __builtin_amdgcn_s_setprio(2);
    else if (L.prio == 3) __builtin_amdgcn_s_setprio(3);
  }
#endif
  const int qcap = env_waves > 2 ? 2 * kQueueLanes : kQueueLanes;
  const bool env_wave = wave < env_waves;
  const int slot = tid;
  const uint64_t i = env0 + slot;
  const bool live = env_wave && slot < nb;
  const int pdw = L.plan_stride_dw;
  uint32_t* plan_w = lds + (env_wave ? slot : 0) * pdw;
  uint32_t* xf = lds + L.envs * pdw;
  uint32_t* st = lds + L.envs * (pdw + L.scratch_dw + L.traf_dw + L.hist_dw);
  uint8_t* sel = reinterpret_cast<uint8_t*>(st + L.stream_words);
  uint64_t* fm = reinterpret_cast<uint64_t*>(sel + kBlock);
  uint32_t* ctr = reinterpret_cast<uint32_t*>(fm + 3 * kBlockDepth);
  uint32_t* lm = L.lm_words ? reinterpret_cast<uint32_t*>(sel + kBlock + 128) : nullptr;
  uint32_t* vw = reinterpret_cast<uint32_t*>(sel + kBlock + 128) + L.lm_words;
  Plan pl{reinterpret_cast<uint16_t*>(plan_w)};

  EnvView v{};
  uint32_t qs = 0;
  int act = 0;
  if (live) {
    v = rec_load(S.rec, i);
    qs = S.qstate[i];
    act = actions[i];
    stage_plan<BIG>(S.plan + i * (uint64_t)c.plan_stride, c.plan_dq, plan_w, pdw);
    xf[slot * L.scratch_dw] = v.spawn;
    xf[slot * L.scratch_dw + 1] = qs;
  }
  const uint32_t qn = qs & 3u, qh = (qs >> 2) & 3u;
  if (env_wave) {
#pragma unroll
    for (int l = 0; l < kBlockDepth; l++) {
      const uint64_t m = __ballot(live && qn <= (uint32_t)l);
      if (lane == 0) fm[l * 3 + wave] = m;
    }
  }
  if (tid == 0) *ctr = 0u;
  for (int k = tid; k < L.lm_words; k += kBlock) lm[k] = 0u;
  lds_barrier();
  STAMP(1);
  int F[kBlockDepth];
#pragma unroll
  for (int l = 0; l < kBlockDepth; l++) {
    F[l] = 0;
    for (int w = 0; w < env_waves; w++) F[l] += __popcll(fm[l * 3 + w]);
  }
  const bool any_empty = F[0] != 0;
#ifdef PGTG_STAMPS
  if ((threadIdx.x & 63) == 0)
    g_stamps[((blockIdx.x * (kBlock / 64) + (threadIdx.x >> 6)) * 32 + 12) & ((1 << 21) - 1)] =
        (unsigned long long)F[0] | (unsigned long long)F[1] << 16 | (unsigned long long)F[2] << 32;
#endif

  if (wave == gen_wave) {
    uint16_t* gplan = reinterpret_cast<uint16_t*>(lds + L.gen_off + lane * pdw);
    auto refill = [&](int k, int l) {
      int e = 0, pre = 0;
      for (int w = 0; w < env_waves; w++) {
        const uint64_t m = fm[l * 3 + w];
        const int cw = __popcll(m);
        if (k >= pre && k < pre + cw) e = w * 64 + select64(m, k - pre);
        pre += cw;
      }
      const uint64_t ie = env0 + e;
      const uint32_t qe = xf[e * L.scratch_dw + 1];
      const uint32_t rslot = (((qe >> 2) & 3u) + (uint32_t)l) % (uint32_t)kBlockDepth;
      gen_queue_entry<BIG>(c, S, ie, xf[e * L.scratch_dw] + 5u * (uint32_t)l, gplan, pdw,
                      S.qbuf + (ie * kBlockDepth + rslot) * (uint64_t)c.qrec_dw, ABLATE(L, 16), !ABLATE(L, 512));
    };
    if (ABLATE(L, 1)) {
      if (any_empty) __syncthreads();
      return;
    }
    for (int k = lane; k < F[0]; k += kQueueLanes) refill(k, 0);
    if (any_empty) __syncthreads();
    for (int k0 = lane; k0 < qcap; k0 += kQueueLanes) {
      int k = k0, l = 1;
      while (l < kBlockDepth && k >= F[l]) {
        k -= F[l];
        l++;
      }
      if (l < kBlockDepth) refill(k, l);
    }
    if (lane == 0) {
      int rest = 0;
      for (int l = 1; l < kBlockDepth; l++) rest += F[l];
      atomicAdd(&S.counters[2], (unsigned long long)(F[0] + min(rest, qcap)));
    }
    STAMP(7);
    STAMPR(3);
    return;
  }

  const int np = kBlock / 64 - 1;
  const int rank = (wave < gen_wave ? wave : wave - 1) * 64 + lane, nthr = np * 64;
  uint32_t bar = 0;
  uint8_t my_sel = 0;
  int err = 0;
  if (live) {
    StepResult res{0.0, 0.0, 0u};
    bool occ_sat = false;
    TrafState ts{0, 0, 0, 0};
    err = env_step<false, BIG>(c, S, i, v, pl, act, res, nullptr, occ_sat, nullptr, ts, nullptr);
    STAMP(22);
    const bool done = (v.flags & (kFlagTerminated | kFlagTruncated)) != 0;
    if (out.reward) out.reward[i] = res.reward;
    if (out.cost) out.cost[i] = res.cost;
    if (out.terminated) out.terminated[i] = (v.flags & kFlagTerminated) ? 1 : 0;
    if (out.truncated) out.truncated[i] = (v.flags & kFlagTruncated) ? 1 : 0;
    if (out.braking) out.braking[i] = 0;
    my_sel = (done && c.autoreset && err == 0) ? 1 : 0;
    if (BIG && res.plan_dirty && !my_sel) store_plan_row<false>(c, S, i, plan_w, pdw);
    if (lm && my_sel && out.final_obs) mark_lines(lm, out.final_obs + env0 * (uint64_t)c.obs_bytes, (uint32_t)slot, (uint32_t)c.obs_bytes);
    STAMP(23);
  }
  {
    ObsInfo oi;
    group_obs<BIG>(c, S, v, live, st, oi, L, wave, lane, ctr, bar, np, rank, vw);
    if (live) write_small_outputs(c, out, i, v, oi, my_sel == 1);
  }
  if (env_wave) sel[slot] = my_sel;
  const uint64_t rm = __ballot(my_sel == 1);
  if (env_wave && lane == 0 && rm) atomicAdd(&S.counters[1], (unsigned long long)__popcll(rm));
  STAMP(2);
  STAMP(28);
  sub_barrier(ctr, bar += (uint32_t)np);
  STAMP(29);
  if (out.final_obs && !ABLATE(L, 2))
    write_obs(out.final_obs + env0 * (uint64_t)c.obs_bytes, (uint32_t)nb, (uint32_t)c.obs_bytes, st,
              ABLATE(L, 128) ? nullptr : sel, rank, nthr, ABLATE(L, 128) ? nullptr : lm);
  STAMP(3);
// ... 442 lines not shown
#pragma unroll
    for (int u = 0; u <= NC; u++)
#pragma unroll
      for (int h = 0; h < V; h++) {
        const uint32_t j = (uint32_t)(V * ln + h) + (u == NC ? pb : (uint32_t)u) * CH;
        offv[u][h] = j < cw2 ? offs[j] : 0u;
      }
    auto load_row = [&](uint32_t r, Row& m) {
      const uint32_t ent = __builtin_amdgcn_readfirstlane(rows[r]);
      const bool fr = ent >= 256u;
      const uint64_t er = (uint64_t)blockIdx.x * K + (ent & 255u);
      const uint8_t* orow = (fr ? a.fobs : a.obs) + er * (uint64_t)OB;
      T* row = reinterpret_cast<T*>(fr ? a.fdst : a.dst) + er * (uint64_t)D;
      const auto src = __builtin_amdgcn_make_buffer_rsrc(uniform_ptr(orow), 0, (int)OB, 0x00020000);
      m.dst = __builtin_amdgcn_make_buffer_rsrc(uniform_ptr(row), 0,
                                                __builtin_amdgcn_readfirstlane((int)(D * sizeof(T))), 0x00020000);
      m.dsto = __builtin_amdgcn_make_buffer_rsrc(uniform_ptr(row), 0,
                                                 __builtin_amdgcn_readfirstlane((int)(pb * CH * sizeof(T))), 0x00020000);
      const auto dpos = __builtin_amdgcn_make_buffer_rsrc(uniform_ptr((fr ? a.fpos : a.pos) + 2 * er), 0, 8, 0x00020000);
      const auto dvel = __builtin_amdgcn_make_buffer_rsrc(uniform_ptr((fr ? a.fvel : a.vel) + 2 * er), 0, 8, 0x00020000);
      const auto dnsd = __builtin_amdgcn_make_buffer_rsrc(
          uniform_ptr(a.nsd_on ? (fr ? a.fnsd : a.nsd) + er : (fr ? a.fpos : a.pos)), 0, a.nsd_on ? 4 : 0, 0x00020000);
      m.mv[0] = (int)__builtin_amdgcn_raw_buffer_load_b32(dpos, lo4, 0, 0);
      m.mv[1] = (int)__builtin_amdgcn_raw_buffer_load_b32(dvel, ovel, 0, 0);
      m.mv[2] = (int)__builtin_amdgcn_raw_buffer_load_b32(dnsd, onsd, 0, 0);
      m.q0 = __builtin_amdgcn_raw_buffer_load_b128(src, lo4 * 4u, 0, 0);
      m.q1 = __builtin_amdgcn_raw_buffer_load_b128(src, 1024u + lo4 * 4u, 0, 0);
      m.tb = __builtin_amdgcn_raw_buffer_load_b8(src, obt + (uint32_t)ln, 0, 0);
    };
    auto store_row = [&](const Row& m) {
      win[wv][ln] = m.q0;
      win[wv][64 + ln] = m.q1;
      if ((uint32_t)ln < OB - obt) wb[obt + (uint32_t)ln] = (uint8_t)m.tb;
      const int mv = m.mv[0] + m.mv[1] + m.mv[2];
      const int px = __builtin_amdgcn_readlane(mv, 0), py = __builtin_amdgcn_readlane(mv, 1);
      const int vx = __builtin_amdgcn_readlane(mv, 2), vy = __builtin_amdgcn_readlane(mv, 3);
      const int nsdv = __builtin_amdgcn_readlane(mv, 4) + 1;
#pragma unroll
      for (int p = 0; p < NC; p++) {
        T f[V];
#pragma unroll
        for (int h = 0; h < V; h++) f[h] = (T)wb[offv[p][h]];
        flat_store_v<T, V>(m.dsto, lo + (uint32_t)p * CH * (uint32_t)sizeof(T), f);
      }
      uint32_t obb[V];
#pragma unroll
      for (int h = 0; h < V; h++) obb[h] = wb[offv[NC][h]];
#pragma unroll
      for (int s = 0; s < 2; s++) {
        const uint32_t pc = pb + (uint32_t)s;
        T f[V];
#pragma unroll
        for (int h = 0; h < V; h++) {
          const int k = V * ln + h + (int)(pc * CH) - (int)cw2;
          const int k2 = a.nsd_on ? k - 9 : k;
          int tv = (int)(k2 == px);
          tv = k2 < 9 ? tv : (int)(k2 - 9 == py);
          tv = k2 < 18 ? tv : (k2 == 18 ? vx : vy);
          tv = (a.nsd_on && k < 9) ? (int)(k == nsdv) : tv;
          f[h] = k < 0 ? (T)obb[h] : (T)tv;
        }
        if (pc * CH < D) flat_store_v<T, V>(m.dst, lo + pc * CH * (uint32_t)sizeof(T), f);
      }
    };
    Row mA{}, mB{};
    uint32_t r = wv;
    if (r < nr) {
      load_row(r, mA);
      load_row(min(r + 4u, nr - 1u), mB);
      store_row(mA);
      r += 4u;
      while (r < nr) {
        load_row(min(r + 4u, nr - 1u), mA);
        store_row(mB);
        r += 4u;
        if (r >= nr) break;
        load_row(min(r + 4u, nr - 1u), mB);
        store_row(mA);
        r += 4u;
      }
    }
  } else {
    for (uint32_t r = wv; r < nr; r += 4u) {
      const uint32_t ent = rows[r];
      const bool fr = ent >= 256u;
      const uint64_t er = (uint64_t)blockIdx.x * K + (ent & 255u);
      const uint8_t* __restrict__ orow = (fr ? a.fobs : a.obs) + er * (uint64_t)a.OB;
      T* __restrict__ row = reinterpret_cast<T*>(fr ? a.fdst : a.dst) + er * (uint64_t)D;
      const int32_t* pos = fr ? a.fpos : a.pos;
      const int32_t* vel = fr ? a.fvel : a.vel;
      const int nsdv = a.nsd_on ? (fr ? a.fnsd : a.nsd)[er] + 1 : -1;
      const int px = pos[2 * er], py = pos[2 * er + 1], vx = vel[2 * er], vy = vel[2 * er + 1];
      for (uint32_t j0 = 0; j0 < D; j0 += kFlatU * 64u) {
        uint32_t ob[kFlatU];
#pragma unroll
        for (int u = 0; u < kFlatU; u++) {
          const uint32_t j = j0 + (uint32_t)ln + (uint32_t)u * 64u;
          const uint32_t off = j0 == 0 ? offs[j - j0] : (j < cw2 ? (uint32_t)a.order[j / w2] * w2 + j % w2 : 0u);
          ob[u] = orow[j < cw2 ? off : 0u];
        }
#pragma unroll
        for (int p = 0; p < kFlatU; p++) {
          const uint32_t j = j0 + (uint32_t)ln + (uint32_t)p * 64u;
          const T f = j < cw2 ? (T)ob[p] : flat_tail<T>(a, (int)(j - cw2), nsdv, px, py, vx, vy);
          if (j < D) row[j] = f;
        }
      }
    }
  }
}

__global__ void k_fill_seeds(uint64_t* seed, uint64_t n, uint64_t base, const uint64_t* src, const uint8_t* mask) {
  uint64_t i = (uint64_t)blockIdx.x * blockDim.x + threadIdx.x;
  if (i < n && (mask == nullptr || mask[i] != 0)) seed[i] = src ? src[i] : base + i;
}

}

using namespace pgtg;

struct pgtg_handle {
  int device = 0;
  uint64_t n = 0;
  hipStream_t stream = nullptr;
  DevCfg hcfg{};
  DevCfg* dcfg = nullptr;
  Tables* dtab = nullptr;
  DevState S{};
  PgtgOutputs out{};
  Lds L{};
  size_t lds = 0;
  std::vector<void*> allocs;
  std::string err;
  uint64_t seed_offset = 0;
  uint64_t* seed_stage = nullptr;
  int tune_epb = 0, tune_obs_sub = 0, tune_kt_grid = 0, tune_kt_cap = 0, tune_kt_wpc = 0;
  int timing = 0;
  uint64_t step_launches = 0;
  std::vector<hipEvent_t> evpool;
  size_t ev_used = 0;
  double acc_ms = 0.0;
  uint64_t acc_n = 0;
  std::vector<uint32_t> epk;
  std::vector<uint16_t> ewl;
  uint32_t tr_slot = 0;
  int kt_grid = 0, kt_cap = 16;
  int kt_plan_dw = 0, kt_rs_dw = 0;
  size_t kt_lds = 0;
  uint64_t q_launch = 0;
  uint64_t q_grid = 0;
  int q_block = -1;
  bool slot_plan = false;
  int tune_queue_mode = 0;
  bool obs_current = false;
  FlatArgs flat{};
  const void* flat_fn = nullptr;
  uint64_t flat_wgs = 1536;
  void* flat_dst = nullptr;
  void* final_flat_dst = nullptr;
  float* flat_rew32 = nullptr;
  uint8_t* flat_dones = nullptr;
  uint8_t* flat_tonly = nullptr;
  int flat_dtype = 0;
  EpisodeArgs ep{};
  uint64_t ep_rows = 0;
};


enum StepArgs { ARGS_ENV, ARGS_ENVB, ARGS_ENVQ };
enum StepFamily { ENV_TR_SLOT, ENV_SLOT, ENV_TR, ENVB, ENVQ, ENV, kStepFamilies };
struct StepKernel {
  const void* fn;
  StepArgs args;
  const char *name, *name_traffic;
};
#define STEP_ROW(fn, args, name) {(const void*)fn, args, name, name " + pgtg::k_traffic"}
static const StepKernel kStepKernels[2 * kStepFamilies] = {
    STEP_ROW((k_env<true, true, true>), ARGS_ENV, "pgtg::k_env<true, true>"),
    STEP_ROW((k_env<true, false, true>), ARGS_ENV, "pgtg::k_env<true, false>"),
    STEP_ROW((k_env<false, true, true>), ARGS_ENV, "pgtg::k_env<false, true>"),
    STEP_ROW((k_env<false, false, true>), ARGS_ENV, "pgtg::k_env<false, false>"),
    STEP_ROW((k_env<true, true>), ARGS_ENV, "pgtg::k_env<true, true>"),
    STEP_ROW((k_env<true, false>), ARGS_ENV, "pgtg::k_env<true, false>"),
    STEP_ROW((k_envb<true>), ARGS_ENVB, "pgtg::k_envb<true>"),
    STEP_ROW((k_envb<false>), ARGS_ENVB, "pgtg::k_envb<false>"),
    STEP_ROW((k_envq<true>), ARGS_ENVQ, "pgtg::k_envq<true>"),
    STEP_ROW((k_envq<false>), ARGS_ENVQ, "pgtg::k_envq<false>"),
    STEP_ROW((k_env<false, true>), ARGS_ENV, "pgtg::k_env<false, true>"),
    STEP_ROW((k_env<false, false>), ARGS_ENV, "pgtg::k_env<false, false>"),
};
#undef STEP_ROW

static const StepKernel& step_fn(const pgtg_handle* h, int mode) {
  StepFamily f = ENV;
  if (h->slot_plan && h->hcfg.n_rules > 0) f = ENV_TR_SLOT;
  else if (h->slot_plan && (mode != MODE_STEP || !h->L.queue)) f = ENV_SLOT;
  else if (h->hcfg.need_car || h->hcfg.n_rules > 0) f = ENV_TR;
  else if (mode == MODE_STEP && h->L.queue) f = h->q_block == 1 ? ENVB : ENVQ;
  return kStepKernels[2 * f + (h->hcfg.nt > kSmallTiles ? 0 : 1)];
}

static int queue_depth(const pgtg_handle* h) { return h->q_block == 1 ? kBlockDepth : kQueueDepth; }

static thread_local std::string g_create_err;

#define HIPCHK(h, x)                                                                 \
  do {                                                                               \
    hipError_t e_ = (x);                                                             \
    if (e_ != hipSuccess) {                                                          \
      (h)->err = std::string(#x) + ": " + hipGetErrorString(e_);                     \
      return PGTG_E_DEVICE;                                                          \
    }                                                                                \
  } while (0)

static int timing_flush(pgtg_handle* h) {
  for (size_t k = 0; k + 1 < h->ev_used; k += 2) {
    float ms = 0.f;
    HIPCHK(h, hipEventSynchronize(h->evpool[k + 1]));
    HIPCHK(h, hipEventElapsedTime(&ms, h->evpool[k], h->evpool[k + 1]));
    h->acc_ms += ms;
    h->acc_n++;
  }
  h->ev_used = 0;
  return 0;
}

template <typename T>
static int dalloc(pgtg_handle* h, T** p, size_t count) {
  void* q = nullptr;
  if (count == 0) count = 1;
  HIPCHK(h, hipMalloc(&q, count * sizeof(T)));
  HIPCHK(h, hipMemset(q, 0, count * sizeof(T)));
  h->allocs.push_back(q);
  *p = reinterpret_cast<T*>(q);
  return 0;
}

static int fail(pgtg_handle* h, int code, const std::string& m) {
  h->err = m;
  return code;
}

static int cu_count(int device) {
  int ncu = 0;
  if (hipDeviceGetAttribute(&ncu, hipDeviceAttributeMultiprocessorCount, device) != hipSuccess || ncu < 1) ncu = 256;
  return ncu;
}

static int host_sync(pgtg_handle* h) {
  HIPCHK(h, hipSetDevice(h->device));
  HIPCHK(h, hipStreamSynchronize(h->stream));
  return 0;
}

static int8_t nsd_dir(int dx, int dy) {
  double angle = atan2(-(double)dy, (double)dx);
  double q = (angle + M_PI) / (M_PI / 4);
  double mq = fmod(q, 8.0);
  if (mq < 0) mq += 8.0;
  static const int remap[8] = {2, 1, 0, 7, 6, 5, 4, 3};
  return (int8_t)remap[(int)mq];
}
static int8_t compass_dir(int dx, int dy, int s) {
  if (abs(dx) <= s && abs(dy) <= s) return -1;
  double angle = atan2((double)dy, (double)dx);
  double P8 = M_PI / 8;
  if (-P8 <= angle && angle < P8) return 2;
  if (P8 <= angle && angle < 3 * P8) return 3;
  if (3 * P8 <= angle && angle < 5 * P8) return 4;
  if (5 * P8 <= angle && angle < 7 * P8) return 5;
  if (angle >= 7 * P8 || angle < -7 * P8) return 6;
  if (-7 * P8 <= angle && angle < -5 * P8) return 7;
  if (-5 * P8 <= angle && angle < -3 * P8) return 0;
  if (-3 * P8 <= angle && angle < -P8) return 1;
  return -1;
}

static uint64_t u53_threshold(double p) {
  if (!(p > 0.0)) return 0;
  if (p >= 1.0) return 1ull << 53;
  return (uint64_t)ceil(ldexp(p, 53));
}

static int derive_cfg(pgtg_handle* h, const PgtgConfig& in, DevCfg& c) {
  memset(&c, 0, sizeof c);
  if (in.abi_version != PGTG_ABI_VERSION) return fail(h, PGTG_E_INVALID, "ABI version mismatch");
  int tw = in.fixed_map ? in.fm_w : in.width, th = in.fixed_map ? in.fm_h : in.height;
  if (tw < 1 || th < 1) return fail(h, PGTG_E_INVALID, "map width and height must be >= 1");
  if (tw * th > PGTG_MAX_TILES) return fail(h, PGTG_E_UNSUPPORTED, "this build supports width*height <= 256 tiles");
  c.tw = tw;
  c.th = th;
  c.nt = tw * th;
  c.W = tw * kTile;
  c.H = th * kTile;
  c.fixed_map = in.fixed_map;
  c.tune_fault = in.tune_fault;
  if (in.fixed_map) {
    for (int t = 0; t < c.nt; t++) {
      uint32_t p = in.fm_exits[t] & 15u;
      if (in.fm_obst_type[t] >= 0) p |= (uint32_t)(in.fm_obst_type[t] + 1) << 4 | (uint32_t)in.fm_obst_mask[t] << 7;
      c.fixed_plan[t] = (uint16_t)p;
    }
    int st = in.fm_start[1] * tw + in.fm_start[0], gl = in.fm_goal[1] * tw + in.fm_goal[0];
    if (in.fm_start[0] < 0 || in.fm_start[0] >= tw || in.fm_start[1] < 0 || in.fm_start[1] >= th || in.fm_goal[0] < 0 ||
        in.fm_goal[0] >= tw || in.fm_goal[1] < 0 || in.fm_goal[1] >= th)
      return fail(h, PGTG_E_INVALID, "fixed map start/goal outside the map");
    c.fixed_sg = (uint32_t)st | (uint32_t)in.fm_start[2] << 8 | (uint32_t)gl << 16 | (uint32_t)in.fm_goal[2] << 24;
  }
  c.start_mode = in.start_mode;
  c.goal_mode = in.goal_mode;
  c.sx = in.start_x;
  c.sy = in.start_y;
  c.sdir = in.start_dir;
  c.gx = in.goal_x;
  c.gy = in.goal_y;
  c.gdir = in.goal_dir;
  c.min_distance = in.min_distance;
  {
    std::vector<int> keys;
    std::vector<std::vector<std::array<int, 2>>> dst(c.nt);
    std::vector<int> seen(c.nt, 0);
    auto add1 = [&](int a, int b, int d) {
      if (!seen[a]) {
        seen[a] = 1;
        keys.push_back(a);
      }
      dst[a].push_back({b, d});
    };
    for (int x = 0; x < tw; x++)
      for (int y = 0; y < th; y++) {
        int t = y * tw + x;
        if (x < tw - 1) {
          add1(t, t + 1, 1);
          add1(t + 1, t, 3);
        }
        if (y < th - 1) {
          add1(t, t + tw, 2);
          add1(t + tw, t, 0);
        }
      }
    std::vector<int> ea, eb, ed;
    for (int a : keys)
// ... 152 lines not shown
    c.car_slots = 3 * cap + kCompactSlack;
    if (in.tune_car_slots > 0) {
      if (in.tune_car_slots < c.car_slots) return fail(h, PGTG_E_INVALID, "tune_car_slots < 3 x car capacity + 4");
      c.car_slots = in.tune_car_slots;
    }
    c.max_spawners = c.nt * 5;
    c.sp_cache_off = c.nt * 16;
    c.traf_bytes = c.sp_cache_off + 2 * kSpCache;
    c.rs_jj_off = ((2 * cap + 3) / 4) * 4;
    c.rs_seen_off = c.rs_jj_off + ((2 * cap + 3) / 4) * 4;
    c.rs_pre_off = c.rs_seen_off + 4 * c.nt;
    c.rs_bytes = (c.rs_pre_off + 2 * (c.W + 1) + 3) / 4 * 4;
    c.rs_bytes = std::max(c.rs_bytes, c.rs_jj_off + 16 * c.nt);
    c.rs_cm_off = 0;
    if (c.th <= 7) {
      c.rs_cm_off = c.rs_bytes;
      c.rs_bytes += 8 * c.W;
    }
  }
  {
    const double ys[5] = {0.95, 0.75, 0.3, 0.98, 0.1}, rv[5] = {0.01, 0.05, 0.15, 0.001, 0.3};
    const int mf[5] = {2, 1, 0, 3, 0};
    const double pl[5] = {0.9, 0.7, 0.3, 0.95, 0.1}, sm[5] = {0.8, 1.0, 1.3, 0.6, 1.5}, rd[5] = {0.1, 0.15, 0.05, 0.3, 0.1};
    for (int k = 0; k < 5; k++) {
      c.beh_t[BEH_YELLOW][k] = u53_threshold(ys[k]);
      c.beh_t[BEH_RED][k] = u53_threshold(rv[k]);
      c.beh_min_follow[k] = mf[k];
      c.beh_patience_thr[k] = (int)floor(pl[k] * 10);
      c.beh_t[BEH_GO][k] = u53_threshold(1.0 - pl[k]);
      c.beh_t[BEH_SPEED][k] = u53_threshold(sm[k]);
      c.beh_t[BEH_DELAY][k] = u53_threshold(rd[k]);
    }
  }
  {
    double tot = 0.0, p[5];
    for (int k = 0; k < 5; k++) tot += in.profile_pct[k];
    for (int k = 0; k < 5; k++) p[k] = tot > 0 ? in.profile_pct[k] / tot : (k == 1 ? 1.0 : 0.0);
    double acc = 0.0, cdf[5];
    for (int k = 0; k < 5; k++) {
      acc += p[k];
      cdf[k] = acc;
    }
    for (int k = 0; k < 5; k++) c.profile_t[k] = u53_threshold(cdf[k] / cdf[4]);
  }
  c.n_rules = in.n_rules;
  if (in.n_rules < 0 || in.n_rules > PGTG_MAX_RULES) return fail(h, PGTG_E_INVALID, "bad rule count");
  for (int k = 0; k < in.n_rules; k++) c.rules[k] = in.rules[k];
  {
    bool possible = c.need_car;
    for (int k = 0; k < in.n_rules; k++) possible = possible || in.rules[k].min_traffic <= 0;
    if (!possible) c.n_rules = 0;
  }
  c.nsd_off = c.W > c.H ? c.W : c.H;
  c.nsd_pitch = 2 * c.nsd_off + 1;
  c.cmp_off = c.nsd_off + 2;
  c.cmp_pitch = 2 * c.cmp_off + 1;
  c.vis_pitch = c.H + 4;
  c.vis_words = ((c.W + 4) * (c.H + 4) + 31) / 32;
  c.plan_dq = (c.nt + 7) / 8;
  c.plan_stride = (!c.need_car && !c.fixed_map && c.nt >= 16) ? ((c.nt + 63) / 64) * 64 : c.plan_dq * 8;
  c.qrec_dw = (c.plan_dq * 4 + 4 + 31) & ~31;
#ifdef PGTG_TUNING
  if (const char* e = getenv("PGTG_QPAD"))
    if (!atoi(e)) c.qrec_dw = c.plan_dq * 4 + 4;
  if (const char* e = getenv("PGTG_PPAD"))
    if (!atoi(e)) c.plan_stride = c.plan_dq * 8;
#endif
  return 0;
}

static void set_sub_envs(Lds& l, int sub) {
  l.sub_envs = sub;
  l.stream_words = img_words(sub, l.seg_bits);
}

extern "C" {

static int choose_launch(pgtg_handle* h, bool allow_queue) {
  const DevCfg& c = h->hcfg;
  h->obs_current = false;
  const uint64_t n_envs = h->n;
  const bool queue_able = allow_queue && !c.need_car && c.n_rules == 0 && !c.fixed_map && !c.generic_channels && c.nt >= 16;
  int envs = c.need_car ? 128
           : n_envs <= (uint64_t)8 * 1024 ? 16
           : n_envs <= (uint64_t)16 * 1024 ? 32
           : n_envs <= (uint64_t)64 * 1024 ? 64
           : (n_envs <= (uint64_t)128 * 1024 || queue_able) ? 128 : kBlock;
  if (h->tune_epb) envs = h->tune_epb;
  if (envs != 16 && envs != 32 && envs != 64 && envs != 128 && envs != 192 && envs != kBlock) envs = kBlock;
  if (envs == 192 && !queue_able) envs = kBlock;
  while (envs > 16 && lds_bytes(lds_layout(c, envs)) + sizeof(Tables) > 150 * 1024) envs /= 2;
  h->L = lds_layout(c, envs);
  if (c.need_car) {
    auto shrink = [&](Lds l) {
      while (l.sub_envs > 8 && lds_bytes(l) + sizeof(Tables) > 80 * 1024) set_sub_envs(l, l.sub_envs / 2);
      return l;
    };
    Lds best = shrink(lds_layout(c, envs));
    while (best.envs > 16 && lds_bytes(best) + sizeof(Tables) > 80 * 1024) best = shrink(lds_layout(c, best.envs / 2));
    if (lds_bytes(best) + sizeof(Tables) > 80 * 1024) best = shrink(lds_layout(c, envs));
    if ((h->tune_epb == 0 && n_envs >= (uint64_t)256 * kBlock) || h->tune_epb == kBlock) {
      Lds l = lds_layout(c, kBlock);
      while (l.sub_envs > 8 && lds_bytes(l) + sizeof(Tables) > 160 * 1024) set_sub_envs(l, l.sub_envs / 2);
      if (lds_bytes(l) + sizeof(Tables) <= 160 * 1024) best = l;
    }
    h->L = best;
  }
  if (!c.need_car && h->L.envs == kBlock) {
    const uint64_t blocks = (n_envs + kBlock - 1) / kBlock;
    const int want = (int)std::min<uint64_t>(4, (blocks + 255) / 256);
    auto fit = [&](const Lds& l) { return (int)((160 * 1024) / (lds_bytes(l) + sizeof(Tables))); };
    while (fit(h->L) < want && h->L.sub_envs > 64) set_sub_envs(h->L, h->L.sub_envs / 2);
  }
  if (h->tune_obs_sub >= 1 && h->tune_obs_sub < h->L.sub_envs) set_sub_envs(h->L, h->tune_obs_sub);
  else lds_img_in_traf(h->L, c);
  if (c.need_car) {
    h->kt_plan_dw = odd_up((c.nt + 1) / 2);
    h->kt_rs_dw = odd_up(c.rs_bytes / 4);
    const size_t per_env = (size_t)4 * (h->kt_plan_dw + h->kt_rs_dw);
    int wpc = h->tune_kt_wpc ? std::max(1, std::min(4, h->tune_kt_wpc)) : 2;
    for (;; wpc--) {
      h->kt_cap = 32;
      while (h->kt_cap > 1 && wpc * (4 * h->kt_cap * per_env + sizeof(Tables) + 256) > 160 * 1024) h->kt_cap--;
      if (wpc == 1 || wpc * (4 * h->kt_cap * per_env + sizeof(Tables) + 256) <= 160 * 1024) break;
    }
    if (h->tune_kt_cap >= 1 && h->tune_kt_cap <= h->kt_cap) h->kt_cap = h->tune_kt_cap;
    h->kt_lds = 4 * h->kt_cap * per_env;
    h->kt_grid = (int)std::min<uint64_t>((uint64_t)cu_count(h->device) * wpc, (h->n + 3) / 4);
    if (h->tune_kt_grid > 0) h->kt_grid = h->tune_kt_grid;
    if (h->kt_lds + sizeof(Tables) > 160 * 1024) return fail(h, PGTG_E_UNSUPPORTED, "LDS budget exceeded (traffic reset scratch)");
    if (h->kt_lds > 64 * 1024)
      (void)hipFuncSetAttribute((const void*)k_traffic, hipFuncAttributeMaxDynamicSharedMemorySize, (int)h->kt_lds);
  }
  h->L.queue = h->L.queue && allow_queue && h->L.sub_envs >= h->L.envs && h->L.envs <= kBlock - 64;
  lds_tail(h->L, c);
  if (h->L.queue && lds_bytes(h->L) + kTabHead > 40 * 1024) {
    h->L.queue = 0;
    lds_tail(h->L, c);
  }
  h->lds = lds_bytes(h->L);
  if (h->lds + sizeof(Tables) > 160 * 1024) return fail(h, PGTG_E_UNSUPPORTED, "LDS budget exceeded");
  if (h->lds > 64 * 1024) {
    for (const StepKernel& k : kStepKernels)
      (void)hipFuncSetAttribute(k.fn, hipFuncAttributeMaxDynamicSharedMemorySize, (int)h->lds);
  }
  if (!c.need_car && c.n_rules == 0) {
    int per_cu = 0;
    const void* fn = step_fn(h, MODE_STEP).fn;
    if (hipOccupancyMaxActiveBlocksPerMultiprocessor(&per_cu, fn, kBlock, h->lds) != hipSuccess || per_cu < 1) per_cu = 1;
    h->L.stagger_wgs = cu_count(h->device) * per_cu;
    const uint64_t blocks = (h->n + h->L.envs - 1) / h->L.envs;
    h->L.stagger = blocks >= (uint64_t)2 * h->L.stagger_wgs ? 1 : 0;
    h->q_grid = std::max<uint64_t>(1, std::min(std::min(blocks, (uint64_t)h->L.stagger_wgs), (uint64_t)kMaxQueueGrid));
    if (h->q_block < 0 && h->L.queue)
      h->q_block = h->tune_queue_mode ? (h->tune_queue_mode == 2 ? 1 : 0)
                                      : (blocks <= (uint64_t)2 * h->L.stagger_wgs ? 1 : 0);
#ifdef PGTG_TUNING
    if (const char* e = getenv("PGTG_STAGGER")) h->L.stagger = atoi(e);
#endif
  }
  return PGTG_OK;
}

static int create(pgtg_handle* h, const PgtgConfig* cfg) {
  h->tune_epb = cfg->tune_envs_per_block;
  h->tune_obs_sub = cfg->tune_obs_sub;
  h->tune_kt_grid = cfg->tune_kt_grid;
  h->tune_kt_cap = cfg->tune_kt_cap;
  h->tune_kt_wpc = cfg->tune_kt_wpc;
  h->tune_queue_mode = cfg->tune_queue_mode;
  if (h->n == 0) return fail(h, PGTG_E_INVALID, "n_envs must be > 0");
  if (int rc = derive_cfg(h, *cfg, h->hcfg)) return rc;
  if (hipSetDevice(h->device) != hipSuccess) return fail(h, PGTG_E_DEVICE, "hipSetDevice failed");
  const DevCfg& c = h->hcfg;
  DevState& S = h->S;
  const uint64_t n = S.n = h->n;
  if (int rc = dalloc(h, &h->dcfg, 1)) return rc;
  if (int rc = dalloc(h, &S.rec, n)) return rc;
  if (int rc = dalloc(h, &S.seed, n)) return rc;
  if (int rc = dalloc(h, &S.err, n)) return rc;
  if (int rc = dalloc(h, &S.counters, 4)) return rc;
  if (int rc = dalloc(h, &S.wg_ticks, 1)) return rc;
  DevStream* streams[4] = {&S.car, &S.ice, &S.broken, &S.sand};
  int needs[4] = {c.need_car, c.need_ice, c.need_broken, c.need_sand};
  for (int k = 0; k < 4; k++)
    if (needs[k])
      for (uint64_t** p : {&streams[k]->shi, &streams[k]->slo, &streams[k]->ihi, &streams[k]->ilo, &streams[k]->buf})
        if (int rc = dalloc(h, p, n)) return rc;
  if (c.visited_penalty != 0.0)
    if (int rc = dalloc(h, &S.visited, n * (uint64_t)c.vis_words)) return rc;
  if (c.nt > kSmallTiles) {
    uint32_t* e = nullptr;
    if (int rc = dalloc(h, &e, h->epk.size())) return rc;
    if (hipMemcpy(e, h->epk.data(), h->epk.size() * sizeof(uint32_t), hipMemcpyHostToDevice) != hipSuccess)
      return fail(h, PGTG_E_DEVICE, "edge table upload failed");
    S.epk = e;
  }
  if (c.need_car) {
    S.sp_pitch = (uint32_t)((c.max_spawners + 7) & ~7);
    S.fresh_occ = (uint32_t)((c.car_cap + 3) & ~3);
    S.fresh_dw = S.fresh_occ + (uint32_t)c.nt * 4u;
    if (int rc = dalloc(h, &S.car_w0, (uint64_t)c.car_slots * n)) return rc;
    if (int rc = dalloc(h, &S.car_w1, (uint64_t)c.car_slots * n)) return rc;
    if (int rc = dalloc(h, &S.car_id, (uint64_t)c.car_slots * n)) return rc;
    if (int rc = dalloc(h, &S.traf, n)) return rc;
    if (int rc = dalloc(h, &S.occ, (uint64_t)c.nt * 4 * n)) return rc;
    if (int rc = dalloc(h, &S.fresh, (uint64_t)S.fresh_dw * n)) return rc;
    if (int rc = dalloc(h, &S.spawners, (uint64_t)S.sp_pitch * n)) return rc;
    if (int rc = dalloc(h, &S.tr_list, n)) return rc;
    if (int rc = dalloc(h, &S.tr_count, 2)) return rc;
  }
  {
    std::vector<int8_t> nsd((size_t)c.nsd_pitch * c.nsd_pitch), cmp((size_t)c.cmp_pitch * c.cmp_pitch);
    for (int a = 0; a < c.nsd_pitch; a++)
      for (int b = 0; b < c.nsd_pitch; b++) nsd[(size_t)a * c.nsd_pitch + b] = nsd_dir(a - c.nsd_off, b - c.nsd_off);
    for (int a = 0; a < c.cmp_pitch; a++)
      for (int b = 0; b < c.cmp_pitch; b++)
        cmp[(size_t)a * c.cmp_pitch + b] = compass_dir(a - c.cmp_off, b - c.cmp_off, cfg->sliding_size);
    int8_t *dn = nullptr, *dc = nullptr;
    if (int rc = dalloc(h, &dn, nsd.size())) return rc;
    if (int rc = dalloc(h, &dc, cmp.size())) return rc;
    if (hipMemcpy(dn, nsd.data(), nsd.size(), hipMemcpyHostToDevice) != hipSuccess ||
        hipMemcpy(dc, cmp.data(), cmp.size(), hipMemcpyHostToDevice) != hipSuccess)
      return fail(h, PGTG_E_DEVICE, "table upload failed");
    S.nsd_tab = dn;
    S.cmp_tab = dc;
  }
  {
    Tables t;
    memset(&t, 0, sizeof t);
    memcpy(t.wall, hs::kTileWall, sizeof t.wall);
    memcpy(t.seg, hs::kExitSeg, sizeof t.seg);
    memcpy(t.obst, hs::kObstMask, sizeof t.obst);
    memcpy(t.spawner, hs::kLaneSpawner, sizeof t.spawner);
    memcpy(t.lanes, hs::kLanes, sizeof t.lanes);
    memcpy(t.ind, c.ind_reward, sizeof t.ind);
    if (c.n_edges <= kSmallEdges) memcpy(t.epk, h->epk.data(), h->epk.size() * sizeof(uint32_t));
    if (c.n_edges <= kSmallEdges) memcpy(t.ewl, h->ewl.data(), h->ewl.size() * sizeof(uint16_t));
    memcpy(t.bt, c.bt, sizeof t.bt);
    memcpy(t.bd, c.bd, sizeof t.bd);
    for (int k = 0; k < PGTG_MAX_CHANNELS; k++) t.chan[k] = (uint8_t)c.channels[k];
    memset(t.li, 255, sizeof t.li);
    memset(t.slot_sq, 255, sizeof t.slot_sq);
    for (int ex = 0; ex < 16; ex++) {
      int n = 0;
      for (int lx = 0; lx < 9; lx++)
        for (int ly = 0; ly < 9; ly++) {
          int sq = lx * 9 + ly;
          uint32_t ln = hs::kLanes[ex][sq];
          if (ln) {
            t.li[ex][sq] = (uint8_t)n;
            t.slot_sq[ex][n] = (uint8_t)sq;
            n++;
            t.lanecol[ex][lx] |= (uint16_t)(1u << ly);
          }
          if ((hs::kLaneSpawner[ex][sq >> 5] >> (sq & 31)) & 1u) t.spcol[ex][lx] |= (uint16_t)(1u << ly);
          for (int ty = 0; ty < 4; ty++)
            if ((ln >> (28 + ty)) & 1u) t.allcol[ex][ty][lx] |= (uint16_t)(1u << ly);
        }
    }
    memcpy(t.lane_route, hs::kLaneRoute, sizeof t.lane_route);
    memcpy(t.route_type_lane, hs::kRouteTypeLane, sizeof t.route_type_lane);
    for (int r = 0; r < cfg->n_rules && r < PGTG_MAX_RULES; r++) memcpy(t.rule_w[r], cfg->rules[r].weight, sizeof t.rule_w[r]);
    memcpy(t.beh_t, h->hcfg.beh_t, sizeof t.beh_t);
    memcpy(t.beh_mf, h->hcfg.beh_min_follow, sizeof t.beh_mf);
    memcpy(t.beh_pt, h->hcfg.beh_patience_thr, sizeof t.beh_pt);
    if (dalloc(h, &h->dtab, 1) || hipMemcpy(h->dtab, &t, sizeof t, hipMemcpyHostToDevice) != hipSuccess)
      return fail(h, PGTG_E_DEVICE, "table upload failed");
  }
  if (hipMemcpy(h->dcfg, &h->hcfg, sizeof(DevCfg), hipMemcpyHostToDevice) != hipSuccess)
    return fail(h, PGTG_E_DEVICE, "config upload failed");
  if (int rc = choose_launch(h, true)) return rc;
  h->slot_plan = h->L.queue && h->q_block == 0;
  if (h->slot_plan && n > (1ull << 30))
    return fail(h, PGTG_E_UNSUPPORTED, "more than 2^30 envs with the persistent map-queue step kernel");
  if (!h->slot_plan)
    if (int rc = dalloc(h, &S.plan, n * (uint64_t)c.plan_stride)) return rc;
  if (h->L.queue) {
    if (int rc = dalloc(h, &S.qbuf, n * (uint64_t)queue_depth(h) * (uint64_t)c.qrec_dw)) return rc;
    if (int rc = dalloc(h, &S.qstate, n)) return rc;
    if (h->slot_plan && hipMemset(S.qstate, 0x04, n) != hipSuccess) return fail(h, PGTG_E_DEVICE, "hipMemset failed");
  }
  if (h->L.queue && !h->q_block) {
    const uint64_t blocks = (n + h->L.envs - 1) / h->L.envs;
    if (int rc = dalloc(h, &S.qreq, 2 * h->q_grid * queue_req_cap(blocks, h->q_grid, h->L.envs))) return rc;
    if (int rc = dalloc(h, &S.qovf, 2 * 8 * ((h->q_grid + 7) / 8) * (uint64_t)h->L.envs)) return rc;
    if (int rc = dalloc(h, &S.qctr, kQctrWords)) return rc;
  }
  return PGTG_OK;
}

int pgtg_create(const PgtgConfig* cfg, uint64_t n_envs, int32_t device, pgtg_handle** out) {
  if (!cfg || !out) return PGTG_E_INVALID;
  *out = nullptr;
  pgtg_handle* h = new pgtg_handle();
  h->device = device;
  h->n = n_envs;
  if (int rc = create(h, cfg)) {
    g_create_err = h->err;
    pgtg_destroy(h);
    return rc;
  }
  *out = h;
  return PGTG_OK;
}

int pgtg_destroy(pgtg_handle* h) {
  if (!h) return PGTG_OK;
  for (void* p : h->allocs) (void)hipFree(p);
  for (auto e : h->evpool) (void)hipEventDestroy(e);
  delete h;
  return PGTG_OK;
}

int pgtg_set_stream(pgtg_handle* h, void* stream) {
  if (!h) return PGTG_E_INVALID;
  h->stream = reinterpret_cast<hipStream_t>(stream);
  return PGTG_OK;
}

int pgtg_set_outputs(pgtg_handle* h, const PgtgOutputs* o) {
  if (!h || !o) return PGTG_E_INVALID;
  if (h->ep.out_ret && (!o->reward || !o->terminated || !o->truncated))
    return fail(h, PGTG_E_INVALID, "episode statistics are bound: the reward, terminated and truncated outputs must stay");
  h->out = *o;
  h->obs_current = false;
  return PGTG_OK;
}

static int launch_episode(pgtg_handle* h) {
  EpisodeArgs a = h->ep;
  a.rew = h->out.reward;
  a.term = h->out.terminated;
  a.trunc = h->out.truncated;
  hipLaunchKernelGGL(k_episode, dim3((unsigned)h->ep_rows), dim3(kEpisodeBlock), 0, h->stream, a);
  HIPCHK(h, hipGetLastError());
  return PGTG_OK;
}

static int episode_zero(pgtg_handle* h, const uint8_t* mask) {
  if (!h->ep.ret) return PGTG_OK;
  hipLaunchKernelGGL(k_episode_zero, dim3((unsigned)h->ep_rows), dim3(kEpisodeBlock), 0, h->stream, h->ep.ret, h->ep.len,
                     mask, h->n);
  HIPCHK(h, hipGetLastError());
  return PGTG_OK;
}

static int launch_flatten(pgtg_handle* h, int mode, uint64_t grid) {
  FlatArgs a = h->flat;
  const PgtgOutputs& o = h->out;
  const bool final = mode == 1;
  a.obs = final ? o.final_obs : o.obs;
  a.pos = final ? o.final_position : o.position;
  a.vel = final ? o.final_velocity : o.velocity;
  a.nsd = final ? o.final_next_subgoal : o.next_subgoal;
  a.term = o.terminated;
  a.trunc = o.truncated;
  a.dst = final ? h->final_flat_dst : h->flat_dst;
  a.fobs = o.final_obs;
  a.fpos = o.final_position;
  a.fvel = o.final_velocity;
  a.fnsd = o.final_next_subgoal;
  a.fdst = h->final_flat_dst;
  a.final = mode;
  a.rew = o.reward;
  a.rew32 = final ? nullptr : h->flat_rew32;
  a.dones = final ? nullptr : h->flat_dones;
  a.tonly = final ? nullptr : h->flat_tonly;
  const bool one = a.D <= kFlatU * 64 && a.OB <= 2048;
  const bool pair = one && !h->flat_dtype && a.D % 2 == 0;
  const void* fn = h->flat_dtype ? (one ? (const void*)k_flatten<int8_t, true, 1> : (const void*)k_flatten<int8_t, false, 1>)
                                 : (pair ? (const void*)k_flatten<float, true, 2>
                                         : (one ? (const void*)k_flatten<float, true, 1> : (const void*)k_flatten<float, false, 1>));
  if (h->flat_fn != fn) {
    int per_cu = 0;
    if (hipOccupancyMaxActiveBlocksPerMultiprocessor(&per_cu, fn, 256, 0) != hipSuccess || per_cu < 1) per_cu = 1;
    h->flat_fn = fn;
    h->flat_wgs = (uint64_t)cu_count(h->device) * (uint64_t)per_cu;
  }
  const uint64_t G = grid ? grid : std::max<uint64_t>(std::min<uint64_t>(h->n, h->flat_wgs), (h->n + 255) / 256);
  void* args[] = {&a};
  HIPCHK(h, hipLaunchKernel(fn, dim3((unsigned)G), dim3(256), args, 0, h->stream));
  HIPCHK(h, hipGetLastError());
  return PGTG_OK;
}

static int launch(pgtg_handle* h, const uint8_t* actions, const uint8_t* mask, int mode) {
  HIPCHK(h, hipSetDevice(h->device));
  uint64_t blocks = (h->n + h->L.envs - 1) / h->L.envs;
  const bool timed = h->timing > 0 && mode == MODE_STEP && (h->step_launches++ % (uint64_t)h->timing) == 0;
  if (timed) {
    if (h->evpool.empty()) {
      h->evpool.resize(2048);
      for (auto& e : h->evpool) HIPCHK(h, hipEventCreate(&e));
    }
    if (h->ev_used + 2 > h->evpool.size()) {
      int rc = timing_flush(h);
      if (rc) return rc;
    }
    HIPCHK(h, hipEventRecord(h->evpool[h->ev_used], h->stream));
  }
  const StepKernel& k = step_fn(h, mode);
  const bool full = !h->obs_current;
  h->obs_current = false;
  uint32_t qsel = (uint32_t)(h->q_launch % 3) | (uint32_t)(h->q_launch & 1) << 2 | (full ? kQselFull : 0u);
  void* args[] = {&h->dcfg, &h->dtab, &h->S, &actions, &mask, &h->out, &mode, &h->L, &h->tr_slot};
  void* bargs[] = {&h->dcfg, &h->dtab, &h->S, &actions, &h->out, &h->L};
  void* qargs[] = {&h->dcfg, &h->dtab, &h->S, &actions, &h->out, &h->L, &qsel};
  void** kargs = args;
  switch (k.args) {
    case ARGS_ENV: break;
    case ARGS_ENVB: kargs = bargs; break;
    case ARGS_ENVQ:
      kargs = qargs;
      h->q_launch++;
      blocks = std::min(blocks, h->q_grid);
      break;
  }
  HIPCHK(h, hipLaunchKernel(k.fn, dim3((unsigned)blocks), dim3(kBlock), kargs, h->lds, h->stream));
  HIPCHK(h, hipGetLastError());
  if (h->hcfg.need_car && mode != MODE_OBSERVE) {
    hipLaunchKernelGGL(k_traffic, dim3((unsigned)h->kt_grid), dim3(kBlock), h->kt_lds, h->stream, h->dcfg, h->dtab,
                       h->S, h->out, h->tr_slot, h->kt_plan_dw, h->kt_rs_dw, h->kt_cap);
    HIPCHK(h, hipGetLastError());
    h->tr_slot ^= 1u;
  }
  {
    const bool fl = h->flat_dst != nullptr, ff = h->final_flat_dst != nullptr && mode == MODE_STEP;
    if (fl || ff)
      if (int rc = launch_flatten(h, fl && ff ? 2 : (ff ? 1 : 0), 0)) return rc;
  }
  if (timed) {
    HIPCHK(h, hipEventRecord(h->evpool[h->ev_used + 1], h->stream));
    h->ev_used += 2;
  }
  if (h->ep.out_ret && mode == MODE_STEP)
    if (int rc = launch_episode(h)) return rc;
  h->obs_current = h->out.obs != nullptr && (mode == MODE_STEP || mode == MODE_OBSERVE || !mask);
  return PGTG_OK;
}

static int queue_fill(pgtg_handle* h) {
  if (!h->L.queue || !h->S.qbuf) return PGTG_OK;
  if (h->S.qctr) HIPCHK(h, hipMemsetAsync(h->S.qctr, 0, kQctrWords * sizeof(uint32_t), h->stream));
#ifdef PGTG_TUNING
  if (const char* e = getenv("PGTG_QFILL"))
    if (!atoi(e)) return PGTG_OK;
#endif
  const int pdw = h->L.plan_stride_dw;
  const size_t lds = (size_t)4 * kBlock * pdw;
  const bool big = h->hcfg.nt > kSmallTiles;
  const void* fn = h->q_block == 1 ? (big ? (const void*)k_qfill_b<true> : (const void*)k_qfill_b<false>)
                                   : (big ? (const void*)k_qfill<true> : (const void*)k_qfill<false>);
  if (lds > 64 * 1024) HIPCHK(h, hipFuncSetAttribute(fn, hipFuncAttributeMaxDynamicSharedMemorySize, (int)lds));
  const uint64_t blocks = (h->n + kBlock - 1) / kBlock;
  void* args[] = {&h->dcfg, &h->dtab, &h->S, (void*)&pdw};
  HIPCHK(h, hipLaunchKernel(fn, dim3((unsigned)blocks), dim3(kBlock), args, lds, h->stream));
  HIPCHK(h, hipGetLastError());
  return PGTG_OK;
}

int pgtg_reset(pgtg_handle* h, const uint64_t* seeds_host, uint64_t seed_base, const uint8_t* mask_dev) {
  if (!h) return PGTG_E_INVALID;
  HIPCHK(h, hipSetDevice(h->device));
  if (seeds_host && !mask_dev) {
    HIPCHK(h, hipMemcpyAsync(h->S.seed, seeds_host, h->n * sizeof(uint64_t), hipMemcpyHostToDevice, h->stream));
  } else {
    const uint64_t* src = nullptr;
    if (seeds_host) {
      if (!h->seed_stage)
        if (int rc = dalloc(h, &h->seed_stage, h->n)) return rc;
      HIPCHK(h, hipMemcpyAsync(h->seed_stage, seeds_host, h->n * sizeof(uint64_t), hipMemcpyHostToDevice, h->stream));
      src = h->seed_stage;
    }
    hipLaunchKernelGGL(k_fill_seeds, dim3((unsigned)((h->n + 255) / 256)), dim3(256), 0, h->stream, h->S.seed, h->n,
                       seed_base, src, mask_dev);
    HIPCHK(h, hipGetLastError());
  }
  if (int rc = launch(h, nullptr, mask_dev, MODE_RESET_SEEDED)) return rc;
  if (int rc = episode_zero(h, mask_dev)) return rc;
  return queue_fill(h);
}

int pgtg_reset_unseeded(pgtg_handle* h, const uint8_t* mask_dev) {
  if (!h) return PGTG_E_INVALID;
  if (int rc = launch(h, nullptr, mask_dev, MODE_RESET_UNSEEDED)) return rc;
  if (int rc = episode_zero(h, mask_dev)) return rc;
  return queue_fill(h);
}

int pgtg_step(pgtg_handle* h, const uint8_t* actions_dev) {
  if (!h || !actions_dev) return PGTG_E_INVALID;
  return launch(h, actions_dev, nullptr, MODE_STEP);
}

int pgtg_step_many(pgtg_handle* h, const uint8_t* actions_dev, uint64_t row_stride, uint64_t ticks) {
  if (!h || !actions_dev || row_stride < h->n) return PGTG_E_INVALID;
  for (uint64_t k = 0; k < ticks; k++)
    if (int rc = launch(h, actions_dev + k * row_stride, nullptr, MODE_STEP)) return rc;
  return PGTG_OK;
}

int pgtg_observe(pgtg_handle* h) {
  if (!h) return PGTG_E_INVALID;
  return launch(h, nullptr, nullptr, MODE_OBSERVE);
}

int pgtg_random_actions(pgtg_handle* h, uint8_t* actions_dev, uint64_t seed, uint64_t t, uint64_t env_offset) {
  if (!h || !actions_dev) return PGTG_E_INVALID;
  HIPCHK(h, hipSetDevice(h->device));
  hipLaunchKernelGGL(k_random_actions, dim3((unsigned)((h->n + 255) / 256)), dim3(256), 0, h->stream, actions_dev, h->n,
                     seed, t, env_offset);
  HIPCHK(h, hipGetLastError());
  return PGTG_OK;
}

static int read_traf(pgtg_handle* h, uint64_t env, uint4* t) {
  HIPCHK(h, hipMemcpy(t, h->S.traf + env, sizeof *t, hipMemcpyDeviceToHost));
  return 0;
}

static int read_plan_row(pgtg_handle* h, uint64_t env, std::vector<uint16_t>& p) {
  const DevCfg& c = h->hcfg;
  p.assign((size_t)c.plan_stride, 0);
  if (h->S.plan) {
    HIPCHK(h, hipMemcpy(p.data(), h->S.plan + env * (uint64_t)c.plan_stride, p.size() * 2, hipMemcpyDeviceToHost));
    return 0;
  }
  uint8_t qs = 0;
  HIPCHK(h, hipMemcpy(&qs, h->S.qstate + env, 1, hipMemcpyDeviceToHost));
  const uint32_t* slot = h->S.qbuf + (env * kQueueDepth + queue_cur(qs)) * (uint64_t)c.qrec_dw;
  HIPCHK(h, hipMemcpy(p.data(), slot, std::min(p.size() * 2, (size_t)c.plan_dq * 16), hipMemcpyDeviceToHost));
  return 0;
}

int pgtg_get_env_state(pgtg_handle* h, uint64_t env, PgtgEnvState* st) {
  if (!h || !st || env >= h->n) return PGTG_E_INVALID;
  if (int rc = host_sync(h)) return rc;
  EnvRec r;
  uint64_t seed;
  uint8_t e;
  HIPCHK(h, hipMemcpy(&r, h->S.rec + env, sizeof r, hipMemcpyDeviceToHost));
  HIPCHK(h, hipMemcpy(&seed, h->S.seed + env, sizeof seed, hipMemcpyDeviceToHost));
  HIPCHK(h, hipMemcpy(&e, h->S.err + env, 1, hipMemcpyDeviceToHost));
  memset(st, 0, sizeof *st);
  st->x = (int16_t)(r.a.x & 0xffffu);
  st->y = (int16_t)(r.a.x >> 16);
  st->vx = (int16_t)(r.a.y & 0xffffu);
  st->vy = (int16_t)(r.a.y >> 16);
  st->phase = (int)(r.a.z & 0xffffu);
  uint32_t fl = (r.a.z >> 16) & 0xfu;
  st->terminated = (fl & kFlagTerminated) ? 1 : 0;
  st->flat_tire = (fl & kFlagFlatTire) ? 1 : 0;
  st->path_len = (int)(r.a.z >> 20);
  st->elapsed = (int)r.a.w;
  st->spawn_counter = r.b.y;
  st->used_subgoals[0] = (uint64_t)r.b.z | ((uint64_t)r.b.w << 32);
  if (h->hcfg.nt > kSmallTiles) {
    std::vector<uint16_t> p;
    if (int rc = read_plan_row(h, env, p)) return rc;
    st->used_subgoals[0] = 0;
    for (int t = 0; t < h->hcfg.nt; t++) st->used_subgoals[t >> 6] |= (uint64_t)((p[t] & kPlanUsed) != 0) << (t & 63);
  }
  st->seed = seed;
  st->error = -(int)e;
  if (h->hcfg.need_car) {
    uint4 t;
    if (int rc = read_traf(h, env, &t)) return rc;
    st->n_cars = (int)(t.x & 0xffffu);
    st->n_spawners = (int)(t.x >> 16);
    st->next_car_id = (int)t.y;
    st->car_tail = (int)t.z;
  }
  return PGTG_OK;
}


static int host_read_cars(pgtg_handle* h, uint64_t env, const uint4& t, std::vector<PgtgCar>& cars) {
  cars.clear();
  const int tail = (int)t.z;
  if (tail == 0) return 0;
  const uint64_t N = h->n;
  std::vector<uint32_t> w0(tail), w1(tail, 0u), id(tail);
  if (t.w & kTrafFresh) {
    HIPCHK(h, hipMemcpy(w0.data(), h->S.fresh + env * (uint64_t)h->S.fresh_dw, 4 * (size_t)tail, hipMemcpyDeviceToHost));
    for (int k = 0; k < tail; k++) id[k] = (uint32_t)k;
  } else {
    HIPCHK(h, hipMemcpy2D(w0.data(), 4, h->S.car_w0 + env, N * 4, 4, tail, hipMemcpyDeviceToHost));
    HIPCHK(h, hipMemcpy2D(w1.data(), 4, h->S.car_w1 + env, N * 4, 4, tail, hipMemcpyDeviceToHost));
    HIPCHK(h, hipMemcpy2D(id.data(), 4, h->S.car_id + env, N * 4, 4, tail, hipMemcpyDeviceToHost));
  }
  for (int k = 0; k < tail; k++) {
    if (w0[k] & kCarEmpty) continue;
    cars.push_back(PgtgCar{(int32_t)id[k], (int32_t)(w0[k] & 255u), (int32_t)((w0[k] >> 8) & 255u),
                           (int32_t)((w0[k] >> 16) & 31u), (int32_t)((w0[k] >> 21) & 7u), (int32_t)w1[k],
                           (int32_t)((w0[k] >> 24) & 3u)});
  }
  if ((int)cars.size() != (int)(t.x & 0xffffu)) return fail(h, PGTG_E_DEVICE, "car slots disagree with the car count");
  return 0;
}

static int host_write_cars(pgtg_handle* h, uint64_t env, uint4 t, const std::vector<PgtgCar>& cars, uint32_t next_id) {
  const int n = (int)cars.size();
  if (n > h->hcfg.car_cap) return fail(h, PGTG_E_UNSUPPORTED, "more cars than the handle's car capacity");
  const uint64_t N = h->n;
  std::vector<uint32_t> w0(n), w1(n), id(n);
  for (int k = 0; k < n; k++) {
    const PgtgCar& q = cars[k];
    w0[k] = (uint32_t)q.x | (uint32_t)q.y << 8 | (uint32_t)q.route << 16 | (uint32_t)q.profile << 21 |
            (uint32_t)q.delay << 24;
    w1[k] = (uint32_t)q.patience;
    id[k] = (uint32_t)q.id;
  }
  if (n > 0) {
    HIPCHK(h, hipMemcpy2D(h->S.car_w0 + env, N * 4, w0.data(), 4, 4, n, hipMemcpyHostToDevice));
    HIPCHK(h, hipMemcpy2D(h->S.car_w1 + env, N * 4, w1.data(), 4, 4, n, hipMemcpyHostToDevice));
    HIPCHK(h, hipMemcpy2D(h->S.car_id + env, N * 4, id.data(), 4, 4, n, hipMemcpyHostToDevice));
  }
  t.x = (t.x & 0xffff0000u) | (uint32_t)n;
  t.y = next_id;
  t.z = (uint32_t)n;
  t.w = 0u;
  HIPCHK(h, hipMemcpy(h->S.traf + env, &t, sizeof t, hipMemcpyHostToDevice));
  return 0;
}

int pgtg_get_cars(pgtg_handle* h, uint64_t env, PgtgCar* cars, int32_t cap, int32_t* n) {
  if (!h || env >= h->n || !n) return PGTG_E_INVALID;
  *n = 0;
  if (!h->hcfg.need_car) return PGTG_OK;
  if (int rc = host_sync(h)) return rc;
  uint4 t;
  if (int rc = read_traf(h, env, &t)) return rc;
  *n = (int)(t.x & 0xffffu);
  if (cars && cap > 0 && *n > 0) {
    std::vector<PgtgCar> v;
    if (int rc = host_read_cars(h, env, t, v)) return rc;
    for (int k = 0; k < (int)v.size() && k < cap; k++) cars[k] = v[k];
  }
  return PGTG_OK;
}

int pgtg_get_map_plan(pgtg_handle* h, uint64_t env, int32_t* w, int32_t* h_, uint8_t* exits, int8_t* otype,
                      int8_t* omask, int32_t* start3, int32_t* goal3) {
  if (!h || env >= h->n) return PGTG_E_INVALID;
  if (int rc = host_sync(h)) return rc;
  const DevCfg& c = h->hcfg;
  std::vector<uint16_t> p;
  EnvRec r;
  if (int rc = read_plan_row(h, env, p)) return rc;
  HIPCHK(h, hipMemcpy(&r, h->S.rec + env, sizeof r, hipMemcpyDeviceToHost));
  *w = c.tw;
// ... 294 lines not shown
    if (rc == hipSuccess) rc = hipMemsetAsync(e.ptr, 0, e.bytes, h->stream);
    if (rc != hipSuccess) {
      if (e.ptr) (void)hipFree(e.ptr);
      pgtg_snapshot_destroy(s);
      return fail(h, PGTG_E_DEVICE, std::string("pgtg_snapshot_create: ") + hipGetErrorString(rc));
    }
    s->sec.push_back(e);
    s->device_bytes += e.bytes;
    s->bytes_per_env += section_bytes(hs, 1);
  }
  if (s->sec.size() > (size_t)kMaxCopySections) {
    pgtg_snapshot_destroy(s);
    return fail(h, PGTG_E_UNSUPPORTED, "pgtg_snapshot_create: more state sections than the copy table holds");
  }
  *out = s;
  return PGTG_OK;
}

int pgtg_snapshot_destroy(pgtg_snapshot* s) {
  if (!s) return PGTG_OK;
  (void)hipSetDevice(s->device);
  for (auto& e : s->sec) (void)hipFree(e.ptr);
  delete s;
  return PGTG_OK;
}

int pgtg_snapshot_bytes(const pgtg_snapshot* s, uint64_t* device_bytes, uint64_t* bytes_per_env) {
  if (!s) return PGTG_E_INVALID;
  if (device_bytes) *device_bytes = s->device_bytes;
  if (bytes_per_env) *bytes_per_env = s->bytes_per_env;
  return PGTG_OK;
}

static int snapshot_table(pgtg_handle* h, const pgtg_snapshot* s, bool to_snapshot, const char* who, CopyTable* T) {
  PgtgStateHeader hd{};
  int depth = 0;
  snapshot_shape(h, &hd, &depth);
  if (h->device != s->device) return fail(h, PGTG_E_INVALID, std::string(who) + ": the snapshot lives on another device");
  if (const char* other = shape_differs(hd, s->shape))
    return fail(h, PGTG_E_INVALID, std::string(who) + ": the snapshot was created from a handle of " + other);
  if (depth != s->depth)
    return fail(h, PGTG_E_INVALID, std::string(who) + ": the snapshot was created from a handle with another map-queue step "
                                                      "kernel (its map rings have another layout)");
  memset(T, 0, sizeof *T);
  uint32_t k = 0;
  for (const auto& hs : state_sections(h)) {
    if (hs.kind == kSecBatch) continue;
    if (k >= s->sec.size() || s->sec[k].id != hs.id || s->sec[k].kind != hs.kind || s->sec[k].row != hs.row)
      return fail(h, PGTG_E_INVALID, std::string(who) + ": section list mismatch");
    CopySection& e = T->sec[k];
    e.src = to_snapshot ? hs.ptr : s->sec[k].ptr;
    e.dst = to_snapshot ? s->sec[k].ptr : hs.ptr;
    e.src_n = to_snapshot ? h->n : s->slots;
    e.dst_n = to_snapshot ? s->slots : h->n;
    e.kind = hs.kind;
    e.row = (uint32_t)hs.row;
    e.unit = 4;
    if (hs.kind == kSecRows) {
      const uint64_t bits = (uint64_t)(uintptr_t)e.src | (uint64_t)(uintptr_t)e.dst | hs.row;
      e.unit = 16;
      while (bits & (e.unit - 1)) e.unit >>= 1;
    }
    k++;
  }
  if (k != s->sec.size()) return fail(h, PGTG_E_INVALID, std::string(who) + ": section list mismatch");
  T->n_sections = k;
  return PGTG_OK;
}

static int snapshot_copy(pgtg_handle* h, const pgtg_snapshot* s, bool to_snapshot, const char* who, const uint32_t* src_idx,
                         const uint32_t* dst_idx, uint64_t count) {
  if (!h || !s) return PGTG_E_INVALID;
  CopyTable T;
  if (int rc = snapshot_table(h, s, to_snapshot, who, &T)) return rc;
  if (count > 0xffffffffull) return fail(h, PGTG_E_INVALID, std::string(who) + ": more than 2^32 - 1 pairs");
  if (count == 0) return PGTG_OK;
  HIPCHK(h, hipSetDevice(h->device));
  if (int rc = queue_fill(h)) return rc;
  if (!to_snapshot) h->obs_current = false;
  T.src_idx = src_idx;
  T.dst_idx = dst_idx;
  T.count = count;
  if (!to_snapshot && h->ep.ret) {
    T.ep_ret = h->ep.ret;
    T.ep_len = h->ep.len;
  }
  hipLaunchKernelGGL(k_state_copy, dim3((unsigned)((count + kCopyBlock - 1) / kCopyBlock)), dim3(kCopyBlock), 0, h->stream, T);
  HIPCHK(h, hipGetLastError());
  return PGTG_OK;
}

int pgtg_snapshot_save(pgtg_handle* h, pgtg_snapshot* s, const uint32_t* env_idx_dev, const uint32_t* slot_idx_dev,
                       uint64_t count) {
  return snapshot_copy(h, s, true, "pgtg_snapshot_save", env_idx_dev, slot_idx_dev, count);
}

int pgtg_snapshot_load(pgtg_handle* h, const pgtg_snapshot* s, const uint32_t* slot_idx_dev, const uint32_t* env_idx_dev,
                       uint64_t count) {
  return snapshot_copy(h, s, false, "pgtg_snapshot_load", slot_idx_dev, env_idx_dev, count);
}

int pgtg_set_to_state(pgtg_handle* h, uint64_t env, int32_t x, int32_t y, int32_t vx, int32_t vy, int32_t flat_tire,
                      const PgtgCar* cars, int32_t n_cars) {
  if (!h || env >= h->n || (n_cars > 0 && !cars)) return PGTG_E_INVALID;
  if (abs(vx) > 30000 || abs(vy) > 30000 || abs(x) > 30000 || abs(y) > 30000)
    return fail(h, PGTG_E_UNSUPPORTED, "position/velocity outside the 16-bit state range");
  const DevCfg& c = h->hcfg;
  if (n_cars > 0 && !c.need_car) return fail(h, PGTG_E_UNSUPPORTED, "create the handle with min_car_capacity > 0 or traffic");
  if (n_cars > c.car_cap) return fail(h, PGTG_E_UNSUPPORTED, "more cars than the handle's car capacity");
  for (int k = 0; k < n_cars; k++)
    if (!car_ok(c, cars[k].x, cars[k].y, cars[k].route, cars[k].profile))
      return fail(h, PGTG_E_INVALID, "car outside the map or bad route/profile");
  if (int rc = host_sync(h)) return rc;
  h->obs_current = false;
  EnvRec r;
  HIPCHK(h, hipMemcpy(&r, h->S.rec + env, sizeof r, hipMemcpyDeviceToHost));
  r.a.x = ((uint32_t)x & 0xffffu) | ((uint32_t)y << 16);
  r.a.y = ((uint32_t)vx & 0xffffu) | ((uint32_t)vy << 16);
  uint32_t flags = (r.a.z >> 16) & 0xfu;
  flags = flat_tire ? (flags | kFlagFlatTire) : (flags & ~kFlagFlatTire);
  r.a.z = (r.a.z & 0xfff0ffffu) | (flags << 16);
  HIPCHK(h, hipMemcpy(h->S.rec + env, &r, sizeof r, hipMemcpyHostToDevice));
  if (c.need_car) {
    uint4 t;
    if (int rc = read_traf(h, env, &t)) return rc;
    std::vector<PgtgCar> v;
    for (int k = 0; k < n_cars; k++) v.push_back(PgtgCar{cars[k].id, cars[k].x, cars[k].y, cars[k].route, cars[k].profile, 0, 0});
    if (int rc = host_write_cars(h, env, t, v, n_cars > 0 ? (uint32_t)cars[n_cars - 1].id + 1u : t.y)) return rc;
  }
  return PGTG_OK;
}

int pgtg_car_digest(pgtg_handle* h, uint64_t* out_dev) {
  if (!h || !out_dev) return PGTG_E_INVALID;
  if (!h->hcfg.need_car) return fail(h, PGTG_E_UNSUPPORTED, "pgtg_car_digest: the handle has no traffic");
  HIPCHK(h, hipSetDevice(h->device));
  hipLaunchKernelGGL(k_car_digest, dim3((unsigned)((h->n + 255) / 256)), dim3(256), 0, h->stream, h->S, out_dev);
  HIPCHK(h, hipGetLastError());
  return PGTG_OK;
}

static int read_counters(pgtg_handle* h, unsigned long long (&c)[4]) {
  if (int rc = host_sync(h)) return rc;
  HIPCHK(h, hipMemcpy(c, h->S.counters, sizeof c, hipMemcpyDeviceToHost));
  return PGTG_OK;
}

int pgtg_get_counters(pgtg_handle* h, uint64_t* env_steps, uint64_t* episodes) {
  if (!h) return PGTG_E_INVALID;
  unsigned long long c[4];
  if (int rc = read_counters(h, c)) return rc;
  if (env_steps) *env_steps = c[0];
  if (episodes) *episodes = c[1];
  return PGTG_OK;
}

int pgtg_get_queue_maps(pgtg_handle* h, uint64_t* maps) {
  if (!h || !maps) return PGTG_E_INVALID;
  unsigned long long c[4];
  if (int rc = read_counters(h, c)) return rc;
  *maps = c[2];
  return PGTG_OK;
}

int pgtg_get_queue_overflow(pgtg_handle* h, uint64_t* served) {
  if (!h || !served) return PGTG_E_INVALID;
  unsigned long long c[4];
  if (int rc = read_counters(h, c)) return rc;
  *served = c[3];
  return PGTG_OK;
}

int pgtg_set_flat_outputs(pgtg_handle* h, const int32_t* order, int32_t n_order, int32_t dtype, void* flat_dev,
                          void* final_flat_dev) {
  if (!h) return PGTG_E_INVALID;
  h->flat_dst = h->final_flat_dst = nullptr;
  if (!flat_dev && !final_flat_dev) return PGTG_OK;
  const DevCfg& c = h->hcfg;
  const PgtgOutputs& o = h->out;
  if (dtype != 0 && dtype != 1) return fail(h, PGTG_E_INVALID, "flat dtype: 0 float32, 1 int8");
  if (!order || n_order != c.n_channels) return fail(h, PGTG_E_INVALID, "flat order: one entry per channel");
  uint64_t seen[2] = {0, 0};
  for (int k = 0; k < n_order; k++) {
    if (order[k] < 0 || order[k] >= n_order || ((seen[order[k] >> 6] >> (order[k] & 63)) & 1u))
      return fail(h, PGTG_E_INVALID, "flat order: not a permutation of the channels");
    seen[order[k] >> 6] |= 1ull << (order[k] & 63);
  }
  if (c.sliding && c.ss >= 9)
    return fail(h, PGTG_E_UNSUPPORTED, "position (s, s) of a sliding window of size >= 9 is outside MultiDiscrete([9, 9])");
  if (flat_dev && (!o.obs || !o.position || !o.velocity || (c.next_subgoal && !o.next_subgoal)))
    return fail(h, PGTG_E_INVALID, "flat rows need the obs, position, velocity (and next_subgoal) outputs");
  if (final_flat_dev && (!o.final_obs || !o.final_position || !o.final_velocity || !o.terminated || !o.truncated ||
                         (c.next_subgoal && !o.final_next_subgoal)))
    return fail(h, PGTG_E_INVALID, "terminal flat rows need the final_* and terminated/truncated outputs");
  if (((uintptr_t)flat_dev | (uintptr_t)final_flat_dev) & 15u) return fail(h, PGTG_E_INVALID, "flat rows: 16-byte aligned buffers");
  FlatArgs& a = h->flat;
  a.n = h->n;
  a.w2 = c.win * c.win;
  a.OB = c.obs_bytes;
  a.cw2 = c.n_channels * a.w2;
  a.nsd_on = c.next_subgoal ? 1 : 0;
  a.D = a.cw2 + (a.nsd_on ? 9 : 0) + 20;
  for (int k = 0; k < n_order; k++) a.order[k] = (uint8_t)order[k];
  h->flat_dtype = dtype;
  h->flat_dst = flat_dev;
  h->final_flat_dst = final_flat_dev;
  return PGTG_OK;
}

int pgtg_set_flat_scalars(pgtg_handle* h, float* reward_f32_dev, uint8_t* dones_dev, uint8_t* truncated_only_dev) {
  if (!h) return PGTG_E_INVALID;
  h->flat_rew32 = nullptr;
  h->flat_dones = h->flat_tonly = nullptr;
  if (!reward_f32_dev && !dones_dev && !truncated_only_dev) return PGTG_OK;
  if (!reward_f32_dev || !dones_dev || !truncated_only_dev)
    return fail(h, PGTG_E_INVALID, "flat scalars: all three buffers or none");
  if (!h->out.reward || !h->out.terminated || !h->out.truncated)
    return fail(h, PGTG_E_INVALID, "flat scalars need the reward, terminated and truncated outputs");
  h->flat_rew32 = reward_f32_dev;
  h->flat_dones = dones_dev;
  h->flat_tonly = truncated_only_dev;
  return PGTG_OK;
}

int pgtg_flatten(pgtg_handle* h, int32_t mode, int32_t grid) {
  if (!h) return PGTG_E_INVALID;
  if (mode < 0 || mode > 2) return fail(h, PGTG_E_INVALID, "pgtg_flatten: mode 0 observation rows, 1 terminal rows, 2 both");
  if (mode != 1 && !h->flat_dst) return fail(h, PGTG_E_INVALID, "pgtg_flatten: no observation rows bound (pgtg_set_flat_outputs)");
  if (mode != 0 && !h->final_flat_dst) return fail(h, PGTG_E_INVALID, "pgtg_flatten: no terminal rows bound (pgtg_set_flat_outputs)");
  if (grid < 0 || (grid > 0 && ((uint64_t)grid < (h->n + 255) / 256 || (uint64_t)grid > h->n)))
    return fail(h, PGTG_E_INVALID, "pgtg_flatten: grid must be 0 or between ceil(n / 256) and n workgroups");
  HIPCHK(h, hipSetDevice(h->device));
  return launch_flatten(h, mode, (uint64_t)grid);
}

int pgtg_set_episode_stats(pgtg_handle* h, float* ep_return_dev, int32_t* ep_length_dev) {
  if (!h) return PGTG_E_INVALID;
  if (!ep_return_dev && !ep_length_dev) {
    h->ep.out_ret = nullptr;
    h->ep.out_len = nullptr;
    return PGTG_OK;
  }
  if (!ep_return_dev || !ep_length_dev) return fail(h, PGTG_E_INVALID, "episode statistics: both buffers or none");
  if (!h->out.reward || !h->out.terminated || !h->out.truncated)
    return fail(h, PGTG_E_INVALID, "episode statistics need the reward, terminated and truncated outputs");
  if (!h->ep.rows) {
    HIPCHK(h, hipSetDevice(h->device));
    h->ep_rows = (h->n + kEpisodeBlock - 1) / kEpisodeBlock;
    if (int rc = dalloc(h, &h->ep.ret, h->n)) return rc;
    if (int rc = dalloc(h, &h->ep.len, h->n)) return rc;
    PgtgEpisodeSummary* rows = nullptr;
    if (int rc = dalloc(h, &rows, h->ep_rows)) return rc;
    HIPCHK(h, hipDeviceSynchronize());
    h->ep.rows = rows;
    h->ep.n = h->n;
  }
  h->ep.out_ret = ep_return_dev;
  h->ep.out_len = ep_length_dev;
  return PGTG_OK;
}

int pgtg_episode_summary(pgtg_handle* h, PgtgEpisodeSummary* out, int32_t reset) {
  if (!h || !out) return PGTG_E_INVALID;
  if (!h->ep.rows) return fail(h, PGTG_E_INVALID, "pgtg_episode_summary: episode statistics were never bound");
  if (int rc = host_sync(h)) return rc;
  std::vector<PgtgEpisodeSummary> rows(h->ep_rows);
  HIPCHK(h, hipMemcpy(rows.data(), h->ep.rows, rows.size() * sizeof(PgtgEpisodeSummary), hipMemcpyDeviceToHost));
  PgtgEpisodeSummary s{};
  s.length_min = INT32_MAX;
  s.return_min = INFINITY;
  s.return_max = -INFINITY;
  for (const auto& r : rows) {
    if (!r.episodes) continue;
    s.episodes += r.episodes;
    s.truncated_only += r.truncated_only;
    s.length_sum += r.length_sum;
    s.length_min = std::min(s.length_min, r.length_min);
    s.length_max = std::max(s.length_max, r.length_max);
    s.return_sum = s.return_sum + r.return_sum;
    s.return_min = std::min(s.return_min, r.return_min);
    s.return_max = std::max(s.return_max, r.return_max);
  }
  *out = s;
  if (reset) {
    HIPCHK(h, hipMemsetAsync(h->ep.rows, 0, rows.size() * sizeof(PgtgEpisodeSummary), h->stream));
    HIPCHK(h, hipStreamSynchronize(h->stream));
  }
  return PGTG_OK;
}

int pgtg_gae(pgtg_handle* h, const PgtgGae* a) {
  if (!h) return PGTG_E_INVALID;
  if (!a) return fail(h, PGTG_E_INVALID, "pgtg_gae: no arguments");
  if (a->steps == 0) return fail(h, PGTG_E_INVALID, "pgtg_gae: steps must be at least 1");
  if (!a->rewards || !a->values || !a->dones || !a->last_values || !a->advantages || !a->returns)
    return fail(h, PGTG_E_INVALID, "pgtg_gae: rewards, values, dones, last_values, advantages and returns are required");
  if ((a->truncated_only == nullptr) != (a->terminal_values == nullptr))
    return fail(h, PGTG_E_INVALID, "pgtg_gae: truncated_only and terminal_values: both or neither");
  if (!std::isfinite(a->gamma) || !std::isfinite(a->gae_lambda))
    return fail(h, PGTG_E_INVALID, "pgtg_gae: gamma and gae_lambda must be finite");
  if (a->n == 0) return PGTG_OK;
  const uint64_t grid = (a->n + kGaeBlock - 1) / kGaeBlock;
  if (grid > 0x7fffffffull || a->steps > 0x7fffffffull || a->steps + 1 > UINT64_MAX / 4 / a->n)
    return fail(h, PGTG_E_UNSUPPORTED, "pgtg_gae: the rollout is too large for one launch");
  GaeArgs g;
  g.rew = a->rewards;
// ... 432 lines not shown
```

### pgtg_amd/vector.py

```python
from __future__ import annotations

import ctypes as C
import os
from typing import Any

from . import _abi
from .config import EnvSpec, make_spec

_EXC = {
    _abi.PGTG_E_INVALID: ValueError,
    _abi.PGTG_E_DONE: RuntimeError,
    _abi.PGTG_E_DEVICE: RuntimeError,
    _abi.PGTG_E_UNSUPPORTED: ValueError,
    _abi.PGTG_E_MAP: ValueError,
}


def _check(rc: int, handle=None) -> None:
    if rc != _abi.PGTG_OK:
        msg = _abi.lib().pgtg_last_error(handle)
        raise _EXC.get(rc, RuntimeError)((msg or b"").decode() or f"pgtg error {rc}")


def fork_indices(roots, copies: int):
# ... 395 lines not shown
                "start": tuple(s3), "goal": tuple(g3)}

    def squares(self, i: int):
        import numpy as np
        w, h = C.c_int32(), C.c_int32()
        _check(self._lib.pgtg_get_squares(self._h, i, None, 0, C.byref(w), C.byref(h)), self._h)
        out = np.zeros(w.value * h.value, np.uint64)
        _check(self._lib.pgtg_get_squares(self._h, i, C.c_void_p(out.ctypes.data), out.size, C.byref(w),
                                          C.byref(h)), self._h)
        return out.reshape(w.value, h.value)

    def _push_rules(self):
        arr = (_abi.PgtgRule * _abi.MAX_RULES)()
        n = _abi.fill_rules(arr, self.spec.rules)
        _check(self._lib.pgtg_set_rules(self._h, arr, n), self._h)

    def add_traffic_rule(self, rule_dict: dict):
        from .config import add_rule
        add_rule(self.spec, rule_dict)
        self._push_rules()

    def remove_traffic_rule(self, rule_name: str) -> bool:
        from .config import remove_rule
        removed = remove_rule(self.spec, rule_name)
        if removed:
            self._push_rules()
        return removed

    def rule_names(self) -> list[str]:
        return [r.name for r in self.spec.rules]

    def dump_state(self):
        import numpy as np
        n = C.c_uint64()
        _check(self._lib.pgtg_state_size(self._h, C.byref(n)), self._h)
        buf = np.empty(n.value, dtype=np.uint8)
        _check(self._lib.pgtg_dump_state(self._h, C.c_void_p(buf.ctypes.data), n.value), self._h)
        return buf

    def load_state(self, blob, observe: bool = True):
        import numpy as np
        b = np.ascontiguousarray(blob, dtype=np.uint8)
        _check(self._lib.pgtg_load_state(self._h, C.c_void_p(b.ctypes.data), b.size), self._h)
        self._seeded = True
        if observe:
            self.observe()

    def snapshot(self, slots: int | None = None) -> Snapshot:
        return Snapshot(self, slots)

    def _scratch_snapshot(self, slots: int) -> Snapshot:
        s = getattr(self, "_scratch", None)
        if s is None or s.slots < slots:
            if s is not None:
                s.close()
            s = self._scratch = Snapshot(self, slots)
        return s

    def copy_envs(self, src, dst, observe: bool = True, check: bool = True) -> None:
        import torch
        src = torch.as_tensor(src, device=self.device).reshape(-1)
        if check and src.numel() and bool(((src < 0) | (src >= self.num_envs)).any()):
            raise ValueError(f"source index outside the batch of {self.num_envs} envs")
        snap = self._scratch_snapshot(max(1, src.numel()))
        snap.save(self, src, None)
        snap.load(self, torch.arange(src.numel(), device=self.device), dst, observe=observe, check=check)

    def rollout(self, n_steps: int, gamma: float = 0.99, gae_lambda: float = 0.95, obs_dtype=None):
        from .rollout import Rollout
        return Rollout(self, n_steps, gamma, gae_lambda, obs_dtype)

    def evaluation(self, n_episodes: int, gamma: float = 0.99):
        from .evaluate import Evaluation
        return Evaluation(self, n_episodes, gamma)

    def _bound_tensors(self) -> list:
        ts = [self.obs_map, self.position, self.velocity, self.reward, self.terminated, self.truncated, self.braking,
              self.cost, self.nsd, self.final_map, self.final_position, self.final_velocity, self.final_nsd]
        for refs in ("_flat_refs", "_flat_scalar_refs", "_episode_refs"):
            ts += list(getattr(self, refs, ()) or ())
        return [t for t in ts if t is not None]

    def light_step(self, actions) -> tuple[dict, Any, Any, Any]:
        snap = self._scratch_snapshot(self.num_envs)
        snap.save(self)
        bound = self._bound_tensors()
        kept = [t.clone() for t in bound]
        stats = self._episode_refs
        if stats:
            self.disable_episode_stats()
        try:
            self.step_launch(actions)
            m, pos, vel = self.obs_map.clone(), self.position.clone(), self.velocity.clone()
            obs = {"position": pos, "velocity": vel, "map": {k: m[:, i] for i, k in enumerate(self.keys)}}
            if self.nsd is not None:
                obs["next_subgoal_direction"] = self.nsd.clone()
            out = (obs, self.reward.clone(), self.terminated.clone(), self.truncated.clone())
        finally:
            snap.load(self, observe=False, check=False)
            for t, k in zip(bound, kept):
                t.copy_(k)
            if stats:
                self._bind_episode_ptrs(*stats)
        return out

    def set_to_state(self, i: int, x: int, y: int, vx: int, vy: int, flat_tire: bool, cars=()):
        cars = list(cars)
        arr = (_abi.PgtgCar * max(1, len(cars)))()
        for k, (cid, cx, cy, route, prof) in enumerate(cars):
            arr[k].id, arr[k].x, arr[k].y, arr[k].route, arr[k].profile = int(cid), int(cx), int(cy), int(route), int(prof)
        _check(self._lib.pgtg_set_to_state(self._h, i, int(x), int(y), int(vx), int(vy), int(bool(flat_tire)), arr,
                                           len(cars)), self._h)

    def set_agent(self, i: int, x: int, y: int, vx: int, vy: int):
        _check(self._lib.pgtg_set_agent(self._h, i, x, y, vx, vy), self._h)

    def add_car(self, i: int, x: int, y: int, route: int, profile: int, car_id: int = -1):
        _check(self._lib.pgtg_add_car(self._h, i, x, y, route, profile, car_id), self._h)

    def mean_cars(self, sample: int = 64) -> float:
        idx = range(0, self.num_envs, max(1, self.num_envs // sample))
        return sum(self.env_state(i)["n_cars"] for i in idx) / len(idx)

    def launch_info(self) -> tuple[int, int]:
        e, b = C.c_int32(), C.c_int32()
        _check(self._lib.pgtg_launch_info(self._h, C.byref(e), C.byref(b)), self._h)
        return e.value, b.value

    def occupancy(self) -> int:
        n = C.c_int32()
        _check(self._lib.pgtg_occupancy(self._h, C.byref(n)), self._h)
        return n.value

    def step_kernel(self) -> str:
        return self._lib.pgtg_step_kernel(self._h).decode()

    def car_digest(self):
        import torch
        out = torch.empty(self.num_envs, dtype=torch.int64, device=self.device)
        self._bind_stream()
        _check(self._lib.pgtg_car_digest(self._h, C.c_void_p(out.data_ptr())), self._h)
        return out

    def counters(self) -> tuple[int, int]:
        a, b = C.c_uint64(), C.c_uint64()
        _check(self._lib.pgtg_get_counters(self._h, C.byref(a), C.byref(b)), self._h)
        return a.value, b.value

    def queue_maps(self) -> int:
        m = C.c_uint64()
        _check(self._lib.pgtg_get_queue_maps(self._h, C.byref(m)), self._h)
        return m.value

    def queue_overflow(self) -> int:
        m = C.c_uint64()
        if not hasattr(self._lib, "pgtg_get_queue_overflow"):
            return -1
        _check(self._lib.pgtg_get_queue_overflow(self._h, C.byref(m)), self._h)
        return m.value

    def enable_timing(self, every: int = 1):
        self._lib.pgtg_enable_timing(self._h, int(every))

    def timing_read(self, reset: bool = True) -> tuple[float, int]:
        ms, n = C.c_double(), C.c_uint64()
        _check(self._lib.pgtg_timing_read(self._h, C.byref(ms), C.byref(n), int(reset)), self._h)
        return ms.value, n.value
```

Measured before the change: 2.750 billion env-steps/s.

## Fuse multiple env ticks into one persistent queue-kernel launch in step_many

Adds a FUSED variant of the queued step kernel that loops over up to step_ticks (default 64) ticks inside a single launch. Blocks walk their env blocks statically instead of using atomic work stealing. The generator wave and the env waves hand off each tick through workgroup-scope counters and spin-waits. pgtg_step_many uses this path when the handle qualifies, which removes per-tick launch overhead and inter-kernel gaps. The cost is in-kernel spin synchronisation, loss of dynamic load balancing, and possible generator stalls that delay the env waves.

Result: faster. 2.938 billion env-steps/s, median of 6 (+6.8%).

```diff
diff --git a/include/pgtg.h b/include/pgtg.h
--- a/include/pgtg.h
+++ b/include/pgtg.h
@@ -86,6 +86,8 @@
   int32_t tune_kt_serial;
   int32_t tune_queue_mode;
   int32_t tune_fault;
+  int32_t tune_step_ticks;
+  int32_t tune_queue_grid;
 } PgtgConfig;
 
 typedef struct {
@@ -269,6 +271,7 @@
 int pgtg_car_digest(pgtg_handle* h, uint64_t* out_dev);
 int pgtg_get_counters(pgtg_handle* h, uint64_t* env_steps, uint64_t* episodes);
 int pgtg_get_queue_maps(pgtg_handle* h, uint64_t* maps);
+int pgtg_get_step_launches(pgtg_handle* h, uint64_t* launches);
 int pgtg_get_queue_overflow(pgtg_handle* h, uint64_t* served);
 int pgtg_error_count(pgtg_handle* h, uint64_t* n_errors, int32_t* first_code);
 int pgtg_measure_hbm(int32_t device, uint64_t bytes, int32_t reps, double* copy_gbs);
diff --git a/pgtg_amd/_abi.py b/pgtg_amd/_abi.py
--- a/pgtg_amd/_abi.py
+++ b/pgtg_amd/_abi.py
@@ -26,7 +26,7 @@
     "pgtg_get_map_plan", "pgtg_get_squares", "pgtg_set_rules", "pgtg_set_agent", "pgtg_add_car", "pgtg_observe", "pgtg_get_counters",
     "pgtg_error_count", "pgtg_window", "pgtg_num_envs", "pgtg_launch_info", "pgtg_occupancy", "pgtg_step_kernel", "pgtg_last_error", "pgtg_enable_timing",
     "pgtg_timing_read", "pgtg_measure_hbm", "pgtg_state_size", "pgtg_dump_state", "pgtg_load_state",
-    "pgtg_set_to_state", "pgtg_car_digest", "pgtg_get_queue_maps", "pgtg_get_queue_overflow", "pgtg_set_flat_outputs", "pgtg_set_flat_scalars",
+    "pgtg_set_to_state", "pgtg_car_digest", "pgtg_get_queue_maps", "pgtg_get_step_launches", "pgtg_get_queue_overflow", "pgtg_set_flat_outputs", "pgtg_set_flat_scalars",
     "pgtg_set_episode_stats", "pgtg_episode_summary", "pgtg_gae", "pgtg_flatten",
     "pgtg_eval_step", "pgtg_eval_summary", "pgtg_eval_workspace_bytes",
     "pgtg_policy", "pgtg_policy_pack", "pgtg_policy_packed_bytes", "pgtg_policy_chunk",
@@ -67,6 +67,7 @@
         ("tune_envs_per_block", C.c_int32), ("tune_obs_sub", C.c_int32), ("tune_kt_grid", C.c_int32),
         ("tune_kt_cap", C.c_int32), ("tune_kt_wpc", C.c_int32), ("tune_car_slots", C.c_int32),
         ("tune_kt_serial", C.c_int32), ("tune_queue_mode", C.c_int32), ("tune_fault", C.c_int32),
+        ("tune_step_ticks", C.c_int32), ("tune_queue_grid", C.c_int32),
     ]
 
 
@@ -192,6 +193,7 @@
         "pgtg_car_digest": ([vp, vp], C.c_int),
         "pgtg_get_queue_maps": ([vp, C.POINTER(u64)], C.c_int),
         "pgtg_get_queue_overflow": ([vp, C.POINTER(u64)], C.c_int),
+        "pgtg_get_step_launches": ([vp, C.POINTER(u64)], C.c_int),
         "pgtg_set_flat_outputs": ([vp, C.POINTER(C.c_int32), i32, i32, vp, vp], C.c_int),
         "pgtg_set_flat_scalars": ([vp, vp, vp, vp], C.c_int),
         "pgtg_flatten": ([vp, i32, i32], C.c_int),
@@ -249,7 +251,8 @@
     return len(rules)
 
 
-TUNE_KEYS = ("envs_per_block", "obs_sub", "kt_grid", "kt_cap", "kt_wpc", "car_slots", "kt_serial", "queue_mode", "fault")
+TUNE_KEYS = ("envs_per_block", "obs_sub", "kt_grid", "kt_cap", "kt_wpc", "car_slots", "kt_serial", "queue_mode", "fault",
+             "step_ticks", "queue_grid")
 
 
 def config_struct(spec: "cfgmod.EnvSpec", autoreset: bool, max_episode_steps: int | None,
diff --git a/pgtg_amd/csrc/pgtg_env.hip b/pgtg_amd/csrc/pgtg_env.hip
--- a/pgtg_amd/csrc/pgtg_env.hip
+++ b/pgtg_amd/csrc/pgtg_env.hip
@@ -95,11 +95,19 @@
       g_stamps[(1 << 20) | ((((blockIdx.x * (kBlock / 64) + (threadIdx.x >> 6)) * 8 + (k))) & ((1 << 20) - 1))] = \
           __builtin_amdgcn_s_memrealtime();                                                           \
   } while (0)
+#define STAMPT(t)                                                                                              \
+  do {                                                                                                         \
+    if (threadIdx.x == 0 && blockIdx.x < 2048u && (t) < 256u)                                                  \
+      g_stamps[(1 << 19) + blockIdx.x * 256u + (t)] = __builtin_amdgcn_s_memrealtime();                        \
+  } while (0)
 #else
 #define STAMP(k) \
   do {           \
   } while (0)
 #define STAMPR(k) \
+  do {            \
+  } while (0)
+#define STAMPT(t) \
   do {            \
   } while (0)
 #endif
@@ -2491,6 +2499,7 @@
 constexpr uint32_t kQueueStale = 0x80u;
 constexpr int kViewDw = 8;
 constexpr int kObsMasks = 2;
+constexpr uint32_t kStepTicks = 64;
 constexpr uint32_t kQselFull = 8u;
 
 __host__ __device__ inline uint32_t queue_tag(uint32_t spawn) { return ~spawn; }
@@ -3061,10 +3070,10 @@
   return QueueMeta(meta);
 }
 
-template <bool BIG>
+template <bool BIG, bool FUSED = false>
 __global__ void __launch_bounds__(kBlock, 4) k_envq(const DevCfg* __restrict__ cfg, const Tables* __restrict__ gtab,
                                                     DevState S, const uint8_t* __restrict__ actions, PgtgOutputs out,
-                                                    Lds L, uint32_t qsel) {
+                                                    Lds L, uint32_t qsel, uint32_t ticks, uint64_t act_stride) {
   extern __shared__ uint32_t lds[];
   const DevCfg& c = *cfg;
   const int tid = threadIdx.x, wave = tid >> 6, lane = tid & 63;
@@ -3073,12 +3082,12 @@
   STAMPR(2);
   const int env_waves = (L.envs + 63) / 64, gen_wave = env_waves;
   const bool env_wave = wave < env_waves;
-  const uint32_t par = (qsel >> 2) & 1u;
+  uint32_t par = (qsel >> 2) & 1u;
   const uint64_t nblk = (S.n + (uint64_t)L.envs - 1) / (uint64_t)L.envs;
   const uint64_t cap = queue_req_cap(nblk, gridDim.x, L.envs);
   uint2* req_new = S.qreq + ((uint64_t)par * gridDim.x + blockIdx.x) * cap;
   const uint2* req_old = S.qreq + ((uint64_t)(par ^ 1u) * gridDim.x + blockIdx.x) * cap;
-  const bool one_round = nblk <= gridDim.x;
+  const bool one_round = !FUSED && nblk <= gridDim.x;
   const uint32_t ox = blockIdx.x & 7u, set_new = qsel & 3u, set_old = (set_new + 2u) % 3u;
   const uint64_t ocap = ((gridDim.x + 7u) / 8u) * (uint64_t)L.envs;
   uint32_t cnt = 0;
@@ -3102,11 +3111,18 @@
   uint32_t* om = delta ? om0 : nullptr;
   uint32_t* qn = ctr + 1;
   uint32_t* nxt = ctr + 2;
+  uint32_t* rdone = ctr + 3;
+  uint32_t* fdone = ctr + 4;
   uint32_t* bctr = S.qctr + kQctrBlocks;
-  if (blockIdx.x == 0 && tid == 0) bctr[((qsel & 3u) + 1u) % 3u] = 0u;
+  if (FUSED) {
+    if (blockIdx.x == 0 && tid < 3) bctr[tid] = 0u;
+  } else if (blockIdx.x == 0 && tid == 0) {
+    bctr[((qsel & 3u) + 1u) % 3u] = 0u;
+  }
   if (tid == 0) {
     *ctr = 0u;
     *qn = 0u;
+    if (FUSED) *rdone = *fdone = 0u;
   }
   lds_barrier();
   asm volatile("" : "+v"(qs_nx));
@@ -3114,53 +3130,65 @@
   if (wave == gen_wave) {
     STAMP(1);
     uint16_t* gplan = reinterpret_cast<uint16_t*>(lds + L.gen_off + lane * pdw);
-    uint32_t made = 0, ovs = 0;
-    if (!ABLATE(L, 1)) {
-      const uint2* ovf = S.qovf + ((uint64_t)(par ^ 1u) * 8u + ox) * ocap;
-      uint32_t ob = 0, on = 0, olen = 0, tot = 0;
-      const uint32_t nj = (gridDim.x - ox + 7u) / 8u, jme = blockIdx.x / 8u;
-      if (one_round) {
-        olen = S.qctr[kQctrOvfLen + set_old * 8u + ox];
-        if (olen > 0) {
-          uint32_t pre = 0;
-          for (uint32_t j0 = 0; j0 < nj; j0 += kQueueLanes) {
-            const uint32_t j = j0 + (uint32_t)lane;
-            const uint32_t sp = j < nj ? kQueueLanes - min(S.qctr[(par ^ 1u) * gridDim.x + ox + 8u * j], (uint32_t)kQueueLanes) : 0u;
-            pre += wave_sum(j < jme ? sp : 0u);
-            tot += wave_sum(sp);
+    for (uint32_t tick = 0;;) {
+      uint32_t made = 0, ovs = 0;
+      if (!ABLATE(L, 1)) {
+        const uint2* ovf = S.qovf + ((uint64_t)(par ^ 1u) * 8u + ox) * ocap;
+        uint32_t ob = 0, on = 0, olen = 0, tot = 0;
+        const uint32_t nj = (gridDim.x - ox + 7u) / 8u, jme = blockIdx.x / 8u;
+        if (one_round) {
+          olen = S.qctr[kQctrOvfLen + set_old * 8u + ox];
+          if (olen > 0) {
+            uint32_t pre = 0;
+            for (uint32_t j0 = 0; j0 < nj; j0 += kQueueLanes) {
+              const uint32_t j = j0 + (uint32_t)lane;
+              const uint32_t sp = j < nj ? kQueueLanes - min(S.qctr[(par ^ 1u) * gridDim.x + ox + 8u * j], (uint32_t)kQueueLanes) : 0u;
+              pre += wave_sum(j < jme ? sp : 0u);
+              tot += wave_sum(sp);
+            }
+            on = olen > pre ? min(olen - pre, kQueueLanes - min(cnt, (uint32_t)kQueueLanes)) : 0u;
+            ob = pre;
           }
-          on = olen > pre ? min(olen - pre, kQueueLanes - min(cnt, (uint32_t)kQueueLanes)) : 0u;
-          ob = pre;
         }
-      }
-      for (uint32_t base = 0;; base += kQueueLanes) {
-        const uint32_t own = base < cnt ? min((uint32_t)kQueueLanes, cnt - base) : 0u;
-        const uint32_t oth = base == 0 ? on : 0u;
-        if (own + oth == 0) break;
-        made += own + oth;
-        ovs += oth;
-        if ((uint32_t)lane < own + oth) {
-          const uint2 r = (uint32_t)lane >= own ? ovf[ob + (lane - own)] : base == 0 ? r0 : req_old[base + lane];
-          const uint64_t ie = r.x >> 2;
-          gen_queue_entry<BIG>(c, S, ie, r.y, gplan, pdw, S.qbuf + (ie * kQueueDepth + queue_slot(r.x)) * (uint64_t)c.qrec_dw,
-                               ABLATE(L, 16), false);
+        for (uint32_t base = 0;; base += kQueueLanes) {
+          const uint32_t own = base < cnt ? min((uint32_t)kQueueLanes, cnt - base) : 0u;
+          const uint32_t oth = base == 0 ? on : 0u;
+          if (own + oth == 0) break;
+          made += own + oth;
+          ovs += oth;
+          if ((uint32_t)lane < own + oth) {
+            const uint2 r = (uint32_t)lane >= own ? ovf[ob + (lane - own)] : base == 0 ? r0 : req_old[base + lane];
+            const uint64_t ie = r.x >> 2;
+            gen_queue_entry<BIG>(c, S, ie, r.y, gplan, pdw, S.qbuf + (ie * kQueueDepth + queue_slot(r.x)) * (uint64_t)c.qrec_dw,
+                                 ABLATE(L, 16), false);
+          }
+          if (base + kQueueLanes >= cnt) break;
         }
-        if (base + kQueueLanes >= cnt) break;
-      }
-      for (uint64_t st0 = tot + (uint64_t)jme * kQueueLanes; st0 < olen; st0 += (uint64_t)nj * kQueueLanes) {
-        const uint32_t m = (uint32_t)min((uint64_t)kQueueLanes, olen - st0);
-        made += m;
-        ovs += m;
-        if ((uint32_t)lane < m) {
-          const uint2 r = ovf[st0 + lane];
-          const uint64_t ie = r.x >> 2;
-          gen_queue_entry<BIG>(c, S, ie, r.y, gplan, pdw, S.qbuf + (ie * kQueueDepth + queue_slot(r.x)) * (uint64_t)c.qrec_dw,
-                               ABLATE(L, 16), false);
+        for (uint64_t st0 = tot + (uint64_t)jme * kQueueLanes; st0 < olen; st0 += (uint64_t)nj * kQueueLanes) {
+          const uint32_t m = (uint32_t)min((uint64_t)kQueueLanes, olen - st0);
+          made += m;
+          ovs += m;
+          if ((uint32_t)lane < m) {
+            const uint2 r = ovf[st0 + lane];
+            const uint64_t ie = r.x >> 2;
+            gen_queue_entry<BIG>(c, S, ie, r.y, gplan, pdw, S.qbuf + (ie * kQueueDepth + queue_slot(r.x)) * (uint64_t)c.qrec_dw,
+                                 ABLATE(L, 16), false);
+          }
         }
       }
-    }
-    if (lane == 0 && made) atomicAdd(&S.counters[2], (unsigned long long)made);
-    if (lane == 0 && ovs) atomicAdd(&S.counters[3], (unsigned long long)ovs);
+      if (lane == 0 && made) atomicAdd(&S.counters[2], (unsigned long long)made);
+      if (lane == 0 && ovs) atomicAdd(&S.counters[3], (unsigned long long)ovs);
+      if (!FUSED || ++tick == ticks) break;
+      __builtin_amdgcn_fence(__ATOMIC_RELEASE, "workgroup");
+      if (lane == 0) __hip_atomic_store(fdone, tick, __ATOMIC_RELAXED, __HIP_MEMORY_SCOPE_WORKGROUP);
+      while (__hip_atomic_load(rdone, __ATOMIC_RELAXED, __HIP_MEMORY_SCOPE_WORKGROUP) < tick * (uint32_t)(kBlock / 64 - 1))
+        __builtin_amdgcn_s_sleep(4);
+      __builtin_amdgcn_fence(__ATOMIC_ACQUIRE, "workgroup");
+      par ^= 1u;
+      req_old = S.qreq + ((uint64_t)(par ^ 1u) * gridDim.x + blockIdx.x) * cap;
+      cnt = S.qctr[(par ^ 1u) * gridDim.x + blockIdx.x];
+      r0 = req_old[lane];
+    }
     STAMP(7);
     STAMPR(3);
     return;
@@ -3169,10 +3197,15 @@
   const int np = kBlock / 64 - 1;
   const int nthr = np * 64;
   uint32_t bar = 0;
+  uint32_t tick = 0;
   for (uint64_t blk = blockIdx.x; blk < nblk;) {
     STAMP(0);
     uint32_t got = 0xffffffffu;
-    if (tid == 0 && nblk > gridDim.x && *qn + 2u * (uint32_t)L.envs <= cap) got = atomicAdd(&bctr[qsel & 3u], 1u);
+    if (!FUSED && tid == 0 && nblk > gridDim.x && *qn + 2u * (uint32_t)L.envs <= cap) got = atomicAdd(&bctr[qsel & 3u], 1u);
+    const auto next_block = [&]() -> uint64_t {
+      const uint64_t b = blk + gridDim.x;
+      return b < nblk ? b : (tick + 1u < ticks ? (uint64_t)blockIdx.x : nblk);
+    };
     int tid_o = tid;
     asm volatile("" : "+v"(tid_o));
     const int lane = tid_o & 63;
@@ -3234,7 +3267,12 @@
     STAMP(28);
     sub_barrier(ctr, bar += (uint32_t)np);
     STAMP(29);
-    {
+    if (FUSED) {
+      const uint64_t bn = next_block();
+      const uint64_t ni = bn * (uint64_t)L.envs + (uint64_t)slot;
+      qs_nx = 0;
+      if (bn != blk && bn < nblk && slot < L.envs && ni < S.n) qs_nx = S.qstate[ni];
+    } else {
       const uint32_t g = *nxt;
       const uint64_t ni = ((uint64_t)gridDim.x + g) * (uint64_t)L.envs + (uint64_t)slot;
       qs_nx = 0;
@@ -3244,6 +3282,10 @@
       write_obs(out.final_obs + env0 * (uint64_t)c.obs_bytes, (uint32_t)nb, (uint32_t)c.obs_bytes, st, sel, rank, nthr, lm);
     STAMP(3);
     sub_barrier(ctr, bar += (uint32_t)np);
+    if (FUSED && tick > 0 && blk == blockIdx.x) {
+      while (__hip_atomic_load(fdone, __ATOMIC_RELAXED, __HIP_MEMORY_SCOPE_WORKGROUP) < tick) __builtin_amdgcn_s_sleep(1);
+      __builtin_amdgcn_fence(__ATOMIC_ACQUIRE, "workgroup");
+    }
     const bool reset_now = my_sel != 0;
     const uint32_t k0 = v.spawn;
     const uint32_t qc = queue_cur(qs), qh = queue_head(qs);
@@ -3301,6 +3343,7 @@
         S.qstate[i] = (uint8_t)(qh | queue_spare(qc, qh) << 2);
       }
     }
+    if (FUSED && blk == blockIdx.x && blk + gridDim.x >= nblk && live) qs_nx = S.qstate[i];
     if (live) {
       rec_store(S.rec, i, v);
       S.err[i] = (uint8_t)(-err);
@@ -3321,10 +3364,29 @@
       write_obs(out.obs + env0 * (uint64_t)c.obs_bytes, (uint32_t)nb, (uint32_t)c.obs_bytes, st, nullptr, rank, nthr, om);
     if (om) om = om == om0 ? om0 + L.lm_words : om0;
     if (tid == 0) atomicAdd(&S.counters[0], (unsigned long long)nb);
-    if (blk == blockIdx.x) stagger_record(L, S, t_start);
+    if (blk == blockIdx.x && (!FUSED || tick == 0)) stagger_record(L, S, t_start);
     STAMP(6);
-    blk = g == 0xffffffffu ? nblk : (uint64_t)gridDim.x + g;
-  }  STAMPR(3);
+    if (!FUSED) {
+      blk = g == 0xffffffffu ? nblk : (uint64_t)gridDim.x + g;
+      continue;
+    }
+    const uint64_t blk_nx = next_block();
+    if (blk + gridDim.x >= nblk) STAMPT(tick);
+    if (blk_nx > blk) {
+      blk = blk_nx;
+      continue;
+    }
+    __builtin_amdgcn_fence(__ATOMIC_RELEASE, "workgroup");
+    if (lane == 0) __hip_atomic_fetch_add(rdone, 1u, __ATOMIC_RELAXED, __HIP_MEMORY_SCOPE_WORKGROUP);
+    if (tid == 0) *qn = 0u;
+    tick++;
+    par ^= 1u;
+    actions += act_stride;
+    req_new = S.qreq + ((uint64_t)par * gridDim.x + blockIdx.x) * cap;
+    if (!om && lm && out.obs && obs_key_ok(c) && kObsMasks * L.lm_words <= L.scratch_dw * L.envs) om = om0;
+    blk = blk_nx;
+  }
+  STAMPR(3);
 }
 
 template <bool BIG>
@@ -4073,6 +4135,10 @@
   int q_block = -1;
   bool slot_plan = false;
   int tune_queue_mode = 0;
+  int tune_queue_grid = 0;
+  uint32_t step_ticks = kStepTicks;
+  uint64_t step_kernels = 0;
+  bool q_static = false;
   bool obs_current = false;
   FlatArgs flat{};
   const void* flat_fn = nullptr;
@@ -4088,8 +4154,8 @@
 };
 
 
-enum StepArgs { ARGS_ENV, ARGS_ENVB, ARGS_ENVQ };
-enum StepFamily { ENV_TR_SLOT, ENV_SLOT, ENV_TR, ENVB, ENVQ, ENV, kStepFamilies };
+enum StepArgs { ARGS_ENV, ARGS_ENVB, ARGS_ENVQ, ARGS_ENVQ_MANY };
+enum StepFamily { ENV_TR_SLOT, ENV_SLOT, ENV_TR, ENVB, ENVQ, ENV, ENVQ_MANY, kStepFamilies };
 struct StepKernel {
   const void* fn;
   StepArgs args;
@@ -4109,6 +4175,8 @@
     STEP_ROW((k_envq<false>), ARGS_ENVQ, "pgtg::k_envq<false>"),
     STEP_ROW((k_env<false, true>), ARGS_ENV, "pgtg::k_env<false, true>"),
     STEP_ROW((k_env<false, false>), ARGS_ENV, "pgtg::k_env<false, false>"),
+    STEP_ROW((k_envq<true, true>), ARGS_ENVQ_MANY, "pgtg::k_envq<true, true>"),
+    STEP_ROW((k_envq<false, true>), ARGS_ENVQ_MANY, "pgtg::k_envq<false, true>"),
 };
 #undef STEP_ROW
 
@@ -4567,6 +4635,7 @@
     const uint64_t blocks = (h->n + h->L.envs - 1) / h->L.envs;
     h->L.stagger = blocks >= (uint64_t)2 * h->L.stagger_wgs ? 1 : 0;
     h->q_grid = std::max<uint64_t>(1, std::min(std::min(blocks, (uint64_t)h->L.stagger_wgs), (uint64_t)kMaxQueueGrid));
+    if (h->tune_queue_grid > 0) h->q_grid = std::min(h->q_grid, (uint64_t)h->tune_queue_grid);
     if (h->q_block < 0 && h->L.queue)
       h->q_block = h->tune_queue_mode ? (h->tune_queue_mode == 2 ? 1 : 0)
                                       : (blocks <= (uint64_t)2 * h->L.stagger_wgs ? 1 : 0);
@@ -4584,6 +4653,11 @@
   h->tune_kt_cap = cfg->tune_kt_cap;
   h->tune_kt_wpc = cfg->tune_kt_wpc;
   h->tune_queue_mode = cfg->tune_queue_mode;
+  h->tune_queue_grid = cfg->tune_queue_grid;
+  if (cfg->tune_step_ticks > 0) h->step_ticks = (uint32_t)cfg->tune_step_ticks;
+#ifdef PGTG_TUNING
+  if (const char* e = getenv("PGTG_STEP_TICKS")) h->step_ticks = (uint32_t)std::max(1, atoi(e));
+#endif
   if (h->n == 0) return fail(h, PGTG_E_INVALID, "n_envs must be > 0");
   if (int rc = derive_cfg(h, *cfg, h->hcfg)) return rc;
   if (hipSetDevice(h->device) != hipSuccess) return fail(h, PGTG_E_DEVICE, "hipSetDevice failed");
@@ -4816,12 +4890,15 @@
     HIPCHK(h, hipEventRecord(h->evpool[h->ev_used], h->stream));
   }
   const StepKernel& k = step_fn(h, mode);
+  if (mode == MODE_STEP) h->step_kernels++;
   const bool full = !h->obs_current;
   h->obs_current = false;
   uint32_t qsel = (uint32_t)(h->q_launch % 3) | (uint32_t)(h->q_launch & 1) << 2 | (full ? kQselFull : 0u);
   void* args[] = {&h->dcfg, &h->dtab, &h->S, &actions, &mask, &h->out, &mode, &h->L, &h->tr_slot};
   void* bargs[] = {&h->dcfg, &h->dtab, &h->S, &actions, &h->out, &h->L};
-  void* qargs[] = {&h->dcfg, &h->dtab, &h->S, &actions, &h->out, &h->L, &qsel};
+  uint32_t one_tick = 1;
+  uint64_t no_stride = 0;
+  void* qargs[] = {&h->dcfg, &h->dtab, &h->S, &actions, &h->out, &h->L, &qsel, &one_tick, &no_stride};
   void** kargs = args;
   switch (k.args) {
     case ARGS_ENV: break;
@@ -4829,8 +4906,10 @@
     case ARGS_ENVQ:
       kargs = qargs;
       h->q_launch++;
+      h->q_static = false;
       blocks = std::min(blocks, h->q_grid);
       break;
+    case ARGS_ENVQ_MANY: return fail(h, PGTG_E_INVALID, "k_envq<BIG, true> is launched by pgtg_step_many");
   }
   HIPCHK(h, hipLaunchKernel(k.fn, dim3((unsigned)blocks), dim3(kBlock), kargs, h->lds, h->stream));
   HIPCHK(h, hipGetLastError());
@@ -4858,6 +4937,7 @@
 static int queue_fill(pgtg_handle* h) {
   if (!h->L.queue || !h->S.qbuf) return PGTG_OK;
   if (h->S.qctr) HIPCHK(h, hipMemsetAsync(h->S.qctr, 0, kQctrWords * sizeof(uint32_t), h->stream));
+  h->q_static = true;
 #ifdef PGTG_TUNING
   if (const char* e = getenv("PGTG_QFILL"))
     if (!atoi(e)) return PGTG_OK;
@@ -4909,10 +4989,42 @@
   return launch(h, actions_dev, nullptr, MODE_STEP);
 }
 
+static bool step_many_fused(const pgtg_handle* h) {
+  if (h->step_ticks < 2 || h->timing > 0 || h->flat_dst || h->final_flat_dst || h->ep.out_ret) return false;
+  if (step_fn(h, MODE_STEP).args != ARGS_ENVQ) return false;
+  return (h->n + h->L.envs - 1) / h->L.envs > h->q_grid;
+}
+
+static int launch_many(pgtg_handle* h, const uint8_t* actions, uint64_t row_stride, uint32_t ticks) {
+  if (!step_many_fused(h) || h->hcfg.need_car || h->hcfg.n_rules > 0)
+    return fail(h, PGTG_E_INVALID, "launch_many on a handle that needs a launch per tick");
+  HIPCHK(h, hipSetDevice(h->device));
+  const StepKernel& k = kStepKernels[2 * ENVQ_MANY + (h->hcfg.nt > kSmallTiles ? 0 : 1)];
+  const bool full = !h->obs_current;
+  h->obs_current = false;
+  uint32_t qsel = (uint32_t)(h->q_launch % 3) | (uint32_t)(h->q_launch & 1) << 2 | (full ? kQselFull : 0u);
+  void* args[] = {&h->dcfg, &h->dtab, &h->S, &actions, &h->out, &h->L, &qsel, &ticks, &row_stride};
+  h->q_launch += ticks;
+  h->step_kernels++;
+  h->q_static = true;
+  HIPCHK(h, hipLaunchKernel(k.fn, dim3((unsigned)h->q_grid), dim3(kBlock), args, h->lds, h->stream));
+  HIPCHK(h, hipGetLastError());
+  h->obs_current = h->out.obs != nullptr;
+  return PGTG_OK;
+}
+
 int pgtg_step_many(pgtg_handle* h, const uint8_t* actions_dev, uint64_t row_stride, uint64_t ticks) {
   if (!h || !actions_dev || row_stride < h->n) return PGTG_E_INVALID;
-  for (uint64_t k = 0; k < ticks; k++)
-    if (int rc = launch(h, actions_dev + k * row_stride, nullptr, MODE_STEP)) return rc;
+  if (ticks < 2 || !step_many_fused(h)) {
+    for (uint64_t k = 0; k < ticks; k++)
+      if (int rc = launch(h, actions_dev + k * row_stride, nullptr, MODE_STEP)) return rc;
+    return PGTG_OK;
+  }
+  for (uint64_t k = 0; k < ticks;) {
+    const uint32_t t = h->q_static ? (uint32_t)std::min<uint64_t>(ticks - k, h->step_ticks) : 1u;
+    if (int rc = launch_many(h, actions_dev + k * row_stride, row_stride, t)) return rc;
+    k += t;
+  }
   return PGTG_OK;
 }
 
@@ -5513,6 +5625,12 @@
   if (int rc = read_counters(h, c)) return rc;
   if (env_steps) *env_steps = c[0];
   if (episodes) *episodes = c[1];
+  return PGTG_OK;
+}
+
+int pgtg_get_step_launches(pgtg_handle* h, uint64_t* launches) {
+  if (!h || !launches) return PGTG_E_INVALID;
+  *launches = h->step_kernels;
   return PGTG_OK;
 }
 
diff --git a/pgtg_amd/vector.py b/pgtg_amd/vector.py
--- a/pgtg_amd/vector.py
+++ b/pgtg_amd/vector.py
@@ -571,6 +571,11 @@
         _check(self._lib.pgtg_get_queue_maps(self._h, C.byref(m)), self._h)
         return m.value
 
+    def step_launches(self) -> int:
+        m = C.c_uint64()
+        _check(self._lib.pgtg_get_step_launches(self._h, C.byref(m)), self._h)
+        return m.value
+
     def queue_overflow(self) -> int:
         m = C.c_uint64()
         if not hasattr(self._lib, "pgtg_get_queue_overflow"):
```
